# hucsmn/suffix_array

Measured on AMD Instinct MI355X. Metric: input MB/s indexed (SA build), higher is better.
Workload: dtype u8; 1 GPU; c3_english_256m: 268435456 bytes per GPU, seed base + rank, one independent text per GPU; n_bytes=268435456, sigma=57, symbols_per_key=13, refinement_rounds=9, text_rounds=0, radix_passes=25, unresolved_after_initial_sort=199000237

## Files before the change

### include/suffix_array_amd.h

```cpp
#ifndef SUFFIX_ARRAY_AMD_H
#define SUFFIX_ARRAY_AMD_H

#include <stdint.h>

#ifdef __cplusplus
extern "C" {
#endif

#define SA_AMD_OK          0
#define SA_AMD_EINVAL     (-1)
#define SA_AMD_ENOMEM     (-2)
#define SA_AMD_EHIP       (-3)
#define SA_AMD_ENODEVICE  (-4)
#define SA_AMD_EINTERNAL  (-5)
#define SA_AMD_ERANGE     (-6)

#define SA_AMD_MAX_LENGTH 2147483647

int32_t sa_amd_max_length(void);

int32_t sa_amd_divsufsort(const uint8_t *T, int32_t *SA, int32_t n);

int32_t sa_amd_saca_u8(const uint8_t *T, uint32_t *SA, int32_t n);

int32_t sa_amd_saca_batch(const uint8_t *const *T, uint32_t *const *SA, const int32_t *n,
                          const int32_t *device, int32_t count, int32_t *status);


typedef struct sa_amd_stats {
    int32_t sigma;
    int32_t bits_per_symbol;
    int32_t symbols_per_key;
    int32_t rounds;
    int32_t sort_passes;
    int32_t sparse_mode;
    int64_t sorted_elements;
    int64_t unresolved_after_initial;
    int32_t text_rounds;
    int32_t top32_first;
    int64_t locally_sorted;
    int32_t readbacks;
    int32_t reserved;
} sa_amd_stats;

int64_t sa_amd_workspace_bytes(int32_t n);

int32_t sa_amd_saca_device(const uint8_t *dT, uint32_t *dSA, int32_t n, void *dWork,
                           int64_t work_bytes, void *stream, sa_amd_stats *stats);

void sa_amd_release_cache(void);

int32_t sa_amd_last_host_timing(double *ms, int32_t capacity);

void sa_amd_last_stats(sa_amd_stats *out);

int32_t sa_amd_device_count(void);
int32_t sa_amd_device_pci_bus_id(int32_t device, char *buf, int32_t capacity);

const char *sa_amd_strerror(int32_t code);
const char *sa_amd_version(void);

#define SA_AMD_BUCKET_TABLE_LEN 65793
int32_t sa_amd_bucket_table(const uint8_t *T, int32_t n, const uint32_t *SA, uint32_t *bkt);
int32_t sa_amd_saca_u8_buckets(const uint8_t *T, uint32_t *SA, int32_t n, uint32_t *bkt);
int32_t sa_amd_bucket_table_device(const uint8_t *dT, const uint32_t *dSA, int32_t n, uint32_t *dBkt, void *stream);

int64_t sa_amd_check_integrity_work_bytes(int32_t n);
int32_t sa_amd_check_integrity(const uint8_t *T, int32_t n, const uint32_t *SA, int64_t sa_len);
int32_t sa_amd_check_integrity_device(const uint8_t *dT, int32_t n, const uint32_t *dSA, void *dWork,
                                      int64_t work_bytes, void *stream);

typedef struct sa_amd_index sa_amd_index;
int32_t sa_amd_index_create(const uint8_t *T, int32_t n, const uint32_t *SA, sa_amd_index **out);
void sa_amd_index_destroy(sa_amd_index *ix);
int32_t sa_amd_index_sa(const sa_amd_index *ix, uint32_t *SA_out);
int32_t sa_amd_index_buckets(sa_amd_index *ix, uint32_t *bkt);
int32_t sa_amd_index_check_integrity(const sa_amd_index *ix);
int32_t sa_amd_index_search(const sa_amd_index *ix, const uint8_t *pat_data, const int64_t *pat_off, int32_t count,
                            uint8_t *contains, uint32_t *range_lo, uint32_t *range_hi, uint32_t *lcp_start,
                            uint32_t *lcp_len);

int64_t sa_amd_pack_bound(int64_t length);
int32_t sa_amd_pack(const uint32_t *SA, int64_t length, uint8_t *out, int64_t capacity, int64_t *out_len);
int32_t sa_amd_unpack(const uint8_t *bytes, int64_t nbytes, uint32_t *SA, int64_t capacity, int64_t *length);

int64_t sa_amd_lcp_work_bytes(int32_t n);
int32_t sa_amd_lcp_device(const uint8_t *dT, const uint32_t *dSA, int32_t n, uint32_t *dLCP,
                          void *dWork, int64_t work_bytes, void *stream);
int32_t sa_amd_lcp(const uint8_t *T, int32_t n, const uint32_t *SA, uint32_t *LCP);
int32_t sa_amd_saca_u8_lcp(const uint8_t *T, uint32_t *SA, int32_t n, uint32_t *LCP);
int32_t sa_amd_index_lcp(const sa_amd_index *ix, uint32_t *LCP);

int32_t sa_amd_index_enable_lcp(sa_amd_index *ix);

typedef struct sa_amd_search_stats {
    int64_t patterns;
    int64_t compared_bytes;
    int64_t steps;
    int64_t table_steps;
    int32_t route;
    int32_t reserved;
} sa_amd_search_stats;
void sa_amd_last_search_stats(sa_amd_search_stats *out);

typedef struct sa_amd_lcp_stats {
    int64_t irreducible;
    int64_t compared_bytes;
    int64_t long_pairs;
    int32_t readbacks, reserved;
} sa_amd_lcp_stats;
void sa_amd_last_lcp_stats(sa_amd_lcp_stats *out);
int32_t sa_amd_lcp_set_compare_cap(int32_t bytes);

int64_t sa_amd_bwt_work_bytes(int32_t n);
int32_t sa_amd_bwt_device(const uint8_t *dT, const uint32_t *dSA, int32_t n, uint8_t *dBWT, int32_t *primary_out,
                          void *dWork, int64_t work_bytes, void *stream);
int32_t sa_amd_bwt(const uint8_t *T, int32_t n, const uint32_t *SA, uint8_t *BWT, int32_t *primary_out);
int32_t sa_amd_index_bwt(const sa_amd_index *ix, uint8_t *BWT, int32_t *primary_out);

int64_t sa_amd_unbwt_work_bytes(int32_t n);
int32_t sa_amd_unbwt_device(const uint8_t *dBWT, int32_t n, int32_t primary, uint8_t *dT_out, void *dWork,
                            int64_t work_bytes, void *stream);
int32_t sa_amd_unbwt(const uint8_t *BWT, int32_t n, int32_t primary, uint8_t *T_out);

typedef struct sa_amd_unbwt_stats {
    int64_t walkers;
    int64_t steps;
    int64_t longest_walk;
    int32_t splitter_spacing;
    int32_t walk_launches;
    int32_t restarts;
    int32_t readbacks;
} sa_amd_unbwt_stats;
void sa_amd_last_unbwt_stats(sa_amd_unbwt_stats *out);
void sa_amd_unbwt_set_walk_limits(int32_t cap_steps, int32_t max_launches);
int32_t sa_amd_unbwt_set_splitter_spacing(int32_t spacing);

#define SA_AMD_REPEATS_ALL        0
#define SA_AMD_REPEATS_KEEP_FIRST 1
int64_t sa_amd_repeats_work_bytes(int32_t n);
int64_t sa_amd_repeat_spans_bound(int32_t n, int32_t min_len);
int32_t sa_amd_repeat_lengths_device(const uint8_t *dT, const uint32_t *dSA, int32_t n, uint32_t *dLR, void *dWork,
                                     int64_t work_bytes, void *stream);
int32_t sa_amd_repeat_spans_device(const uint8_t *dT, const uint32_t *dSA, int32_t n, int32_t min_len, int32_t mode,
                                   uint32_t *dSpans, int64_t capacity, int64_t *count_out, void *dWork, int64_t work_bytes,
                                   void *stream);
int32_t sa_amd_repeat_lengths(const uint8_t *T, int32_t n, const uint32_t *SA, uint32_t *LR);
int32_t sa_amd_repeat_spans(const uint8_t *T, int32_t n, const uint32_t *SA, int32_t min_len, int32_t mode, uint32_t *spans,
                            int64_t capacity, int64_t *count_out);
int32_t sa_amd_index_repeat_lengths(const sa_amd_index *ix, uint32_t *LR);
int32_t sa_amd_index_repeat_spans(const sa_amd_index *ix, int32_t min_len, int32_t mode, uint32_t *spans, int64_t capacity,
                                  int64_t *count_out);

typedef struct sa_amd_repeat_stats {
    int64_t longest;
    int64_t longest_pos;
    int64_t lcp_sum;
    int64_t distinct_substrings;
    int64_t spans;
    int64_t covered_bytes;
    int64_t flagged;
    int32_t readbacks, reserved;
} sa_amd_repeat_stats;
void sa_amd_last_repeat_stats(sa_amd_repeat_stats *out);

#define SA_AMD_LZ_LITERAL 0xffffffffu
int64_t sa_amd_lz_work_bytes(int32_t n);
int32_t sa_amd_lpf_device(const uint8_t *dT, const uint32_t *dSA, int32_t n, uint32_t *dLPF, uint32_t *dSRC, void *dWork,
                          int64_t work_bytes, void *stream);
int32_t sa_amd_lz77_device(const uint8_t *dT, const uint32_t *dSA, int32_t n, uint32_t *dPhrases, int64_t capacity,
                           int64_t *count_out, void *dWork, int64_t work_bytes, void *stream);
int32_t sa_amd_lpf(const uint8_t *T, int32_t n, const uint32_t *SA, uint32_t *LPF, uint32_t *SRC);
int32_t sa_amd_lz77(const uint8_t *T, int32_t n, const uint32_t *SA, uint32_t *phrases, int64_t capacity, int64_t *count_out);
int32_t sa_amd_index_lpf(const sa_amd_index *ix, uint32_t *LPF, uint32_t *SRC);
int32_t sa_amd_index_lz77(const sa_amd_index *ix, uint32_t *phrases, int64_t capacity, int64_t *count_out);

typedef struct sa_amd_lz_stats {
    int64_t phrases;
    int64_t literals;
    int64_t longest;
    int64_t longest_pos;
    int64_t unresolved;
    int64_t hierarchy_steps;
    int64_t hierarchy_max;
    int64_t walkers;
    int64_t walk_steps;
    int32_t walk_launches;
    int32_t restarts;
    int32_t splitter_spacing;
    int32_t readbacks;
} sa_amd_lz_stats;
void sa_amd_last_lz_stats(sa_amd_lz_stats *out);

#define SA_AMD_MATCH_NONE 0xffffffffu
int64_t sa_amd_match_work_bytes(int32_t m);
int32_t sa_amd_index_match_stats(const sa_amd_index *ix, const uint8_t *Q, int32_t m, int32_t max_len, uint32_t *ML, uint32_t *POS);
int32_t sa_amd_index_match_stats_device(const sa_amd_index *ix, const uint8_t *dQ, int32_t m, int32_t max_len, uint32_t *dML,
                                        uint32_t *dPOS, void *dWork, int64_t work_bytes, void *stream);
int32_t sa_amd_index_match_spans(const sa_amd_index *ix, const uint8_t *Q, int32_t m, int32_t min_len, uint32_t *spans,
                                 int64_t capacity, int64_t *count_out);
int32_t sa_amd_index_match_spans_device(const sa_amd_index *ix, const uint8_t *dQ, int32_t m, int32_t min_len, uint32_t *dSpans,
// ... 35 lines not shown
```

### suffix_array_amd/__init__.py

```python
from __future__ import annotations

import ctypes
import os
from typing import Optional

import numpy as np

__all__ = ["MAX_LENGTH", "saca", "SuffixArray", "SuffixArrayError", "lib", "diag_lib", "library_path", "Stats", "last_host_timing",
           "saca_batch", "workspace_bytes", "device_pci_bus_id", "saca_device_ptr", "bucket_table", "check_integrity", "last_stats", "DeviceIndex", "pack", "unpack",
           "lcp", "saca_lcp", "last_lcp_stats", "lcp_work_bytes", "lcp_device_ptr", "LcpStats",
           "lcp_set_compare_cap", "last_search_stats", "SearchStats",
           "bwt", "unbwt", "bwt_device_ptr", "unbwt_device_ptr", "bwt_work_bytes", "unbwt_work_bytes", "last_unbwt_stats",
           "unbwt_set_walk_limits", "unbwt_set_splitter_spacing", "UnbwtStats",
           "repeat_lengths", "repeat_spans", "last_repeat_stats", "repeats_work_bytes", "repeat_spans_bound",
           "repeat_lengths_device_ptr", "repeat_spans_device_ptr", "RepeatStats", "REPEATS_ALL", "REPEATS_KEEP_FIRST",
           "lpf", "lz77", "lz77_decode", "lz77_literals", "last_lz_stats", "lz_work_bytes", "lpf_device_ptr", "lz77_device_ptr", "LzStats", "LZ_LITERAL",
           "MatchStats", "last_match_stats", "match_work_bytes", "match_set_group_cap", "match_set_group_lanes", "match_stats_device_ptr", "match_spans_device_ptr",
           "MATCH_NONE", "MATCH_TILE"]

MAX_LENGTH = 2**31 - 1

_HERE = os.path.dirname(os.path.abspath(__file__))
_LIB_NAME = "libsuffix_array_amd.so"
_lib: Optional[ctypes.CDLL] = None


class SuffixArrayError(RuntimeError):

    def __init__(self, code: int, what: str):
        super().__init__(f"suffix_array_amd: {what} (status {code})")
        self.code = code


class Stats(ctypes.Structure):
    _fields_ = [("sigma", ctypes.c_int32), ("bits_per_symbol", ctypes.c_int32),
                ("symbols_per_key", ctypes.c_int32), ("rounds", ctypes.c_int32),
                ("sort_passes", ctypes.c_int32), ("sparse_mode", ctypes.c_int32),
                ("sorted_elements", ctypes.c_int64), ("unresolved_after_initial", ctypes.c_int64),
                ("text_rounds", ctypes.c_int32), ("top32_first", ctypes.c_int32), ("locally_sorted", ctypes.c_int64),
                ("readbacks", ctypes.c_int32), ("reserved", ctypes.c_int32)]

    def as_dict(self):
        return {k: getattr(self, k) for k, _ in self._fields_}


class LcpStats(ctypes.Structure):
    _fields_ = [("irreducible", ctypes.c_int64), ("compared_bytes", ctypes.c_int64), ("long_pairs", ctypes.c_int64),
                ("readbacks", ctypes.c_int32), ("reserved", ctypes.c_int32)]

    def as_dict(self):
        return {k: getattr(self, k) for k, _ in self._fields_ if k != "reserved"}


class SearchStats(ctypes.Structure):
    _fields_ = [("patterns", ctypes.c_int64), ("compared_bytes", ctypes.c_int64), ("steps", ctypes.c_int64),
                ("table_steps", ctypes.c_int64), ("route", ctypes.c_int32), ("reserved", ctypes.c_int32)]

    def as_dict(self):
        return {name: getattr(self, name) for name, _ in self._fields_ if name != "reserved"}


class UnbwtStats(ctypes.Structure):
    _fields_ = [("walkers", ctypes.c_int64), ("steps", ctypes.c_int64), ("longest_walk", ctypes.c_int64),
                ("splitter_spacing", ctypes.c_int32), ("walk_launches", ctypes.c_int32), ("restarts", ctypes.c_int32),
                ("readbacks", ctypes.c_int32)]

    def as_dict(self):
        return {name: getattr(self, name) for name, _ in self._fields_}


class RepeatStats(ctypes.Structure):
    _fields_ = [("longest", ctypes.c_int64), ("longest_pos", ctypes.c_int64), ("lcp_sum", ctypes.c_int64),
                ("distinct_substrings", ctypes.c_int64), ("spans", ctypes.c_int64), ("covered_bytes", ctypes.c_int64),
                ("flagged", ctypes.c_int64), ("readbacks", ctypes.c_int32), ("reserved", ctypes.c_int32)]

    def as_dict(self):
        return {name: getattr(self, name) for name, _ in self._fields_ if name != "reserved"}


class LzStats(ctypes.Structure):
    _fields_ = [("phrases", ctypes.c_int64), ("literals", ctypes.c_int64), ("longest", ctypes.c_int64), ("longest_pos", ctypes.c_int64),
                ("unresolved", ctypes.c_int64), ("hierarchy_steps", ctypes.c_int64), ("hierarchy_max", ctypes.c_int64),
                ("walkers", ctypes.c_int64), ("walk_steps", ctypes.c_int64), ("walk_launches", ctypes.c_int32),
                ("restarts", ctypes.c_int32), ("splitter_spacing", ctypes.c_int32), ("readbacks", ctypes.c_int32)]

    def as_dict(self):
        return {name: getattr(self, name) for name, _ in self._fields_}


class MatchStats(ctypes.Structure):
    _fields_ = [("positions", ctypes.c_int64), ("matched", ctypes.c_int64), ("longest", ctypes.c_int64), ("longest_pos", ctypes.c_int64),
                ("ml_sum", ctypes.c_int64), ("long_positions", ctypes.c_int64), ("compared_bytes", ctypes.c_int64), ("steps", ctypes.c_int64),
                ("spans", ctypes.c_int64), ("covered_bytes", ctypes.c_int64), ("flagged", ctypes.c_int64), ("route_long", ctypes.c_int32),
                ("readbacks", ctypes.c_int32), ("group_lanes", ctypes.c_int32), ("group_cap", ctypes.c_int32), ("tile", ctypes.c_int32),
                ("reserved", ctypes.c_int32)]

    def as_dict(self):
        return {name: getattr(self, name) for name, _ in self._fields_ if name != "reserved"}


MATCH_NONE = 0xFFFFFFFF
MATCH_TILE = 256

LZ_LITERAL = 0xFFFFFFFF

REPEATS_ALL = 0
REPEATS_KEEP_FIRST = 1


def library_path() -> str:
    return os.path.join(_HERE, _LIB_NAME)


def lib() -> ctypes.CDLL:
    global _lib
    if _lib is None:
        path = library_path()
        if not os.path.exists(path):
            raise ImportError(f"{path} not found: run `python -c 'import __graft_entry__ as g; g.build()'` "
                              "(there is no CPU fallback)")
        L = ctypes.CDLL(path)
        c_u8p, c_vp = ctypes.c_void_p, ctypes.c_void_p
        L.sa_amd_max_length.restype = ctypes.c_int32
        L.sa_amd_divsufsort.argtypes = [c_u8p, c_vp, ctypes.c_int32]
        L.sa_amd_divsufsort.restype = ctypes.c_int32
        L.sa_amd_saca_u8.argtypes = [c_u8p, c_vp, ctypes.c_int32]
        L.sa_amd_saca_u8.restype = ctypes.c_int32
        L.sa_amd_saca_batch.argtypes = [c_vp, c_vp, c_vp, c_vp, ctypes.c_int32, c_vp]
        L.sa_amd_saca_batch.restype = ctypes.c_int32
        L.sa_amd_workspace_bytes.argtypes = [ctypes.c_int32]
        L.sa_amd_workspace_bytes.restype = ctypes.c_int64
        L.sa_amd_saca_device.argtypes = [c_vp, c_vp, ctypes.c_int32, c_vp, ctypes.c_int64, c_vp, c_vp]
        L.sa_amd_saca_device.restype = ctypes.c_int32
        L.sa_amd_device_count.restype = ctypes.c_int32
        L.sa_amd_device_pci_bus_id.argtypes = [ctypes.c_int32, ctypes.c_char_p, ctypes.c_int32]
        L.sa_amd_device_pci_bus_id.restype = ctypes.c_int32
        L.sa_amd_bucket_table_device.argtypes = [c_vp, c_vp, ctypes.c_int32, c_vp, c_vp]
        L.sa_amd_bucket_table_device.restype = ctypes.c_int32
        L.sa_amd_last_stats.argtypes = [c_vp]
        L.sa_amd_index_create.argtypes = [c_vp, ctypes.c_int32, c_vp, ctypes.POINTER(ctypes.c_void_p)]
        L.sa_amd_index_create.restype = ctypes.c_int32
        L.sa_amd_index_destroy.argtypes = [c_vp]
        L.sa_amd_index_destroy.restype = None
        for fn in ("sa_amd_index_sa", "sa_amd_index_buckets"):
            getattr(L, fn).argtypes = [c_vp, c_vp]
            getattr(L, fn).restype = ctypes.c_int32
        L.sa_amd_index_check_integrity.argtypes = [c_vp]
        L.sa_amd_index_check_integrity.restype = ctypes.c_int32
        L.sa_amd_index_search.argtypes = [c_vp, c_vp, c_vp, ctypes.c_int32, c_vp, c_vp, c_vp, c_vp, c_vp]
        L.sa_amd_index_search.restype = ctypes.c_int32
        L.sa_amd_pack_bound.argtypes = [ctypes.c_int64]
        L.sa_amd_pack_bound.restype = ctypes.c_int64
        L.sa_amd_pack.argtypes = [c_vp, ctypes.c_int64, c_vp, ctypes.c_int64, c_vp]
        L.sa_amd_pack.restype = ctypes.c_int32
        L.sa_amd_unpack.argtypes = [c_vp, ctypes.c_int64, c_vp, ctypes.c_int64, c_vp]
        L.sa_amd_unpack.restype = ctypes.c_int32
        L.sa_amd_bucket_table.argtypes = [c_vp, ctypes.c_int32, c_vp, c_vp]
        L.sa_amd_bucket_table.restype = ctypes.c_int32
        L.sa_amd_saca_u8_buckets.argtypes = [c_vp, c_vp, ctypes.c_int32, c_vp]
        L.sa_amd_saca_u8_buckets.restype = ctypes.c_int32
        L.sa_amd_check_integrity.argtypes = [c_vp, ctypes.c_int32, c_vp, ctypes.c_int64]
        L.sa_amd_check_integrity.restype = ctypes.c_int32
        L.sa_amd_last_stats.restype = None
        L.sa_amd_strerror.argtypes = [ctypes.c_int32]
        L.sa_amd_strerror.restype = ctypes.c_char_p
        L.sa_amd_version.restype = ctypes.c_char_p
        L.sa_amd_profile_begin.restype = None
        L.sa_amd_profile_end.argtypes = [c_vp, c_vp, c_vp, ctypes.c_int32]
        L.sa_amd_profile_end.restype = ctypes.c_int32
        L.sa_amd_profile_kernel_name.argtypes = [ctypes.c_int32]
        L.sa_amd_profile_kernel_name.restype = ctypes.c_char_p
        L.sa_amd_last_host_timing.argtypes = [c_vp, ctypes.c_int32]
        L.sa_amd_last_host_timing.restype = ctypes.c_int32
        L.sa_amd_profile_begin_classes.argtypes = [ctypes.c_uint64]
        L.sa_amd_profile_begin_classes.restype = None
        L.sa_amd_check_integrity_device.argtypes = [c_vp, ctypes.c_int32, c_vp, c_vp, ctypes.c_int64, c_vp]
        L.sa_amd_check_integrity_device.restype = ctypes.c_int32
        L.sa_amd_check_integrity_work_bytes.argtypes = [ctypes.c_int32]
        L.sa_amd_check_integrity_work_bytes.restype = ctypes.c_int64
        L.sa_amd_lcp_work_bytes.argtypes = [ctypes.c_int32]
        L.sa_amd_lcp_work_bytes.restype = ctypes.c_int64
        L.sa_amd_lcp_device.argtypes = [c_vp, c_vp, ctypes.c_int32, c_vp, c_vp, ctypes.c_int64, c_vp]
        L.sa_amd_lcp_device.restype = ctypes.c_int32
        L.sa_amd_lcp.argtypes = [c_vp, ctypes.c_int32, c_vp, c_vp]
        L.sa_amd_lcp.restype = ctypes.c_int32
        L.sa_amd_saca_u8_lcp.argtypes = [c_vp, c_vp, ctypes.c_int32, c_vp]
        L.sa_amd_saca_u8_lcp.restype = ctypes.c_int32
        L.sa_amd_index_lcp.argtypes = [c_vp, c_vp]
        L.sa_amd_index_lcp.restype = ctypes.c_int32
        L.sa_amd_last_lcp_stats.argtypes = [c_vp]
        L.sa_amd_last_lcp_stats.restype = None
        L.sa_amd_lcp_set_compare_cap.argtypes = [ctypes.c_int32]
        L.sa_amd_lcp_set_compare_cap.restype = ctypes.c_int32
        L.sa_amd_index_enable_lcp.argtypes = [c_vp]
        L.sa_amd_index_enable_lcp.restype = ctypes.c_int32
        L.sa_amd_last_search_stats.argtypes = [c_vp]
        L.sa_amd_last_search_stats.restype = None
        L.sa_amd_bwt_work_bytes.argtypes = [ctypes.c_int32]
        L.sa_amd_bwt_work_bytes.restype = ctypes.c_int64
        L.sa_amd_bwt_device.argtypes = [c_vp, c_vp, ctypes.c_int32, c_vp, c_vp, c_vp, ctypes.c_int64, c_vp]
        L.sa_amd_bwt_device.restype = ctypes.c_int32
        L.sa_amd_bwt.argtypes = [c_vp, ctypes.c_int32, c_vp, c_vp, c_vp]
        L.sa_amd_bwt.restype = ctypes.c_int32
        L.sa_amd_index_bwt.argtypes = [c_vp, c_vp, c_vp]
        L.sa_amd_index_bwt.restype = ctypes.c_int32
        L.sa_amd_unbwt_work_bytes.argtypes = [ctypes.c_int32]
        L.sa_amd_unbwt_work_bytes.restype = ctypes.c_int64
        L.sa_amd_unbwt_device.argtypes = [c_vp, ctypes.c_int32, ctypes.c_int32, c_vp, c_vp, ctypes.c_int64, c_vp]
        L.sa_amd_unbwt_device.restype = ctypes.c_int32
        L.sa_amd_unbwt.argtypes = [c_vp, ctypes.c_int32, ctypes.c_int32, c_vp]
        L.sa_amd_unbwt.restype = ctypes.c_int32
        L.sa_amd_last_unbwt_stats.argtypes = [c_vp]
        L.sa_amd_last_unbwt_stats.restype = None
        L.sa_amd_unbwt_set_walk_limits.argtypes = [ctypes.c_int32, ctypes.c_int32]
        L.sa_amd_unbwt_set_walk_limits.restype = None
        L.sa_amd_unbwt_set_splitter_spacing.argtypes = [ctypes.c_int32]
        L.sa_amd_unbwt_set_splitter_spacing.restype = ctypes.c_int32
        L.sa_amd_repeats_work_bytes.argtypes = [ctypes.c_int32]
        L.sa_amd_repeats_work_bytes.restype = ctypes.c_int64
        L.sa_amd_repeat_spans_bound.argtypes = [ctypes.c_int32, ctypes.c_int32]
        L.sa_amd_repeat_spans_bound.restype = ctypes.c_int64
        L.sa_amd_repeat_lengths_device.argtypes = [c_vp, c_vp, ctypes.c_int32, c_vp, c_vp, ctypes.c_int64, c_vp]
        L.sa_amd_repeat_lengths_device.restype = ctypes.c_int32
        L.sa_amd_repeat_spans_device.argtypes = [c_vp, c_vp, ctypes.c_int32, ctypes.c_int32, ctypes.c_int32, c_vp, ctypes.c_int64,
                                                 c_vp, c_vp, ctypes.c_int64, c_vp]
        L.sa_amd_repeat_spans_device.restype = ctypes.c_int32
        L.sa_amd_repeat_lengths.argtypes = [c_vp, ctypes.c_int32, c_vp, c_vp]
        L.sa_amd_repeat_lengths.restype = ctypes.c_int32
        L.sa_amd_repeat_spans.argtypes = [c_vp, ctypes.c_int32, c_vp, ctypes.c_int32, ctypes.c_int32, c_vp, ctypes.c_int64, c_vp]
        L.sa_amd_repeat_spans.restype = ctypes.c_int32
        L.sa_amd_index_repeat_lengths.argtypes = [c_vp, c_vp]
        L.sa_amd_index_repeat_lengths.restype = ctypes.c_int32
        L.sa_amd_index_repeat_spans.argtypes = [c_vp, ctypes.c_int32, ctypes.c_int32, c_vp, ctypes.c_int64, c_vp]
        L.sa_amd_index_repeat_spans.restype = ctypes.c_int32
        L.sa_amd_last_repeat_stats.argtypes = [c_vp]
        L.sa_amd_last_repeat_stats.restype = None
        L.sa_amd_lz_work_bytes.argtypes = [ctypes.c_int32]
        L.sa_amd_lz_work_bytes.restype = ctypes.c_int64
        L.sa_amd_lpf_device.argtypes = [c_vp, c_vp, ctypes.c_int32, c_vp, c_vp, c_vp, ctypes.c_int64, c_vp]
        L.sa_amd_lpf_device.restype = ctypes.c_int32
        L.sa_amd_lz77_device.argtypes = [c_vp, c_vp, ctypes.c_int32, c_vp, ctypes.c_int64, c_vp, c_vp, ctypes.c_int64, c_vp]
        L.sa_amd_lz77_device.restype = ctypes.c_int32
        L.sa_amd_lpf.argtypes = [c_vp, ctypes.c_int32, c_vp, c_vp, c_vp]
        L.sa_amd_lpf.restype = ctypes.c_int32
        L.sa_amd_lz77.argtypes = [c_vp, ctypes.c_int32, c_vp, c_vp, ctypes.c_int64, c_vp]
        L.sa_amd_lz77.restype = ctypes.c_int32
        L.sa_amd_index_lpf.argtypes = [c_vp, c_vp, c_vp]
        L.sa_amd_index_lpf.restype = ctypes.c_int32
        L.sa_amd_index_lz77.argtypes = [c_vp, c_vp, ctypes.c_int64, c_vp]
        L.sa_amd_index_lz77.restype = ctypes.c_int32
        L.sa_amd_last_lz_stats.argtypes = [c_vp]
        L.sa_amd_last_lz_stats.restype = None
        L.sa_amd_match_work_bytes.argtypes = [ctypes.c_int32]
        L.sa_amd_match_work_bytes.restype = ctypes.c_int64
        L.sa_amd_index_match_stats.argtypes = [c_vp, c_vp, ctypes.c_int32, ctypes.c_int32, c_vp, c_vp]
        L.sa_amd_index_match_stats.restype = ctypes.c_int32
        L.sa_amd_index_match_stats_device.argtypes = [c_vp, c_vp, ctypes.c_int32, ctypes.c_int32, c_vp, c_vp, c_vp, ctypes.c_int64, c_vp]
        L.sa_amd_index_match_stats_device.restype = ctypes.c_int32
        L.sa_amd_index_match_spans.argtypes = [c_vp, c_vp, ctypes.c_int32, ctypes.c_int32, c_vp, ctypes.c_int64, c_vp]
        L.sa_amd_index_match_spans.restype = ctypes.c_int32
        L.sa_amd_index_match_spans_device.argtypes = [c_vp, c_vp, ctypes.c_int32, ctypes.c_int32, c_vp, ctypes.c_int64, c_vp, c_vp,
                                                      ctypes.c_int64, c_vp]
        L.sa_amd_index_match_spans_device.restype = ctypes.c_int32
        L.sa_amd_last_match_stats.argtypes = [c_vp]
        L.sa_amd_last_match_stats.restype = None
        L.sa_amd_match_set_group_cap.argtypes = [ctypes.c_int32]
        L.sa_amd_match_set_group_cap.restype = ctypes.c_int32
        L.sa_amd_match_set_group_lanes.argtypes = [ctypes.c_int32]
        L.sa_amd_match_set_group_lanes.restype = ctypes.c_int32
        _lib = L
    return _lib


_diag: Optional[ctypes.CDLL] = None


def diag_lib() -> ctypes.CDLL:
    global _diag
    if _diag is None:
        path = os.path.join(_HERE, "libsuffix_array_amd_diag.so")
        if not os.path.exists(path):
            raise ImportError(f"{path} not found: run __graft_entry__.build()")
        L = ctypes.CDLL(path)
        c_vp = ctypes.c_void_p
        L.sa_amd_test_sort_pairs.argtypes = [c_vp, c_vp, ctypes.c_int64, ctypes.c_int32, ctypes.c_int32]
        L.sa_amd_test_sort_pairs.restype = ctypes.c_int32
        L.sa_amd_test_sort_pairs32.argtypes = [c_vp, c_vp, ctypes.c_int64, ctypes.c_int32, ctypes.c_int32]
        L.sa_amd_test_sort_pairs32.restype = ctypes.c_int32
        L.sa_amd_test_sample_sort64.argtypes = [c_vp, c_vp, ctypes.c_int64, ctypes.c_int32, c_vp]
        L.sa_amd_test_sample_sort64.restype = ctypes.c_int32
        L.sa_amd_test_bucket_sort32.argtypes = [c_vp, c_vp, ctypes.c_int64, ctypes.c_int32, c_vp]
        L.sa_amd_test_bucket_sort32.restype = ctypes.c_int32
        L.sa_amd_test_lz_nsv.argtypes = [c_vp, ctypes.c_int64, c_vp, c_vp, c_vp]
        L.sa_amd_test_lz_nsv.restype = ctypes.c_int32
        L.sa_amd_test_build_keys.argtypes = [c_vp, ctypes.c_int32, c_vp, c_vp, c_vp]
        L.sa_amd_test_build_keys.restype = ctypes.c_int32
        L.sa_amd_debug_phase_cycles.argtypes = [c_vp, ctypes.c_int32]
        L.sa_amd_debug_phase_cycles.restype = ctypes.c_int32
        L.sa_amd_debug_group_sort_stamps.argtypes = [ctypes.c_int32]
        L.sa_amd_debug_group_sort_stamps.restype = ctypes.c_int32
        L.sa_amd_debug_sort_variant_count.restype = ctypes.c_int32
        L.sa_amd_debug_sort_variant_name.argtypes = [ctypes.c_int32]
        L.sa_amd_debug_sort_variant_name.restype = ctypes.c_char_p
        L.sa_amd_saca_u8.argtypes = [c_vp, c_vp, ctypes.c_int32]
        L.sa_amd_saca_u8.restype = ctypes.c_int32
        L.sa_amd_saca_device.argtypes = [c_vp, c_vp, ctypes.c_int32, c_vp, ctypes.c_int64, c_vp, c_vp]
        L.sa_amd_saca_device.restype = ctypes.c_int32
        L.sa_amd_workspace_bytes.argtypes = [ctypes.c_int32]
        L.sa_amd_workspace_bytes.restype = ctypes.c_int64
        L.sa_amd_version.restype = ctypes.c_char_p
        _diag = L
    return _diag


def device_pci_bus_id(device: int = 0) -> str:
    buf = ctypes.create_string_buffer(64)
    _check(lib().sa_amd_device_pci_bus_id(int(device), buf, 64))
    return buf.value.decode()


def _check(code: int) -> None:
    if code != 0:
        raise SuffixArrayError(code, lib().sa_amd_strerror(code).decode())


def _as_u8(s) -> np.ndarray:
    if isinstance(s, np.ndarray):
        if s.dtype != np.uint8 or not s.flags.c_contiguous:
            raise TypeError("text must be a contiguous uint8 array")
        return s
    return np.frombuffer(bytes(s), dtype=np.uint8) if len(s) else np.zeros(0, dtype=np.uint8)


def saca(s, sa: np.ndarray) -> None:
    t = _as_u8(s)
    assert t.size <= MAX_LENGTH
    assert t.size + 1 == sa.size
    if sa.dtype != np.uint32 or not sa.flags.c_contiguous or not sa.flags.writeable:
        raise TypeError("sa must be a writable contiguous uint32 array")
    _check(lib().sa_amd_saca_u8(t.ctypes.data, sa.ctypes.data, t.size))


def divsufsort(s, sa: np.ndarray) -> None:
    t = _as_u8(s)
    assert t.size == sa.size and sa.dtype == np.int32
    _check(lib().sa_amd_divsufsort(t.ctypes.data, sa.ctypes.data, t.size))


def saca_batch(texts, devices=None):
    ts = [_as_u8(t) for t in texts]
    cnt = len(ts)
    if cnt >= 64:
        sizes = np.fromiter((t.size for t in ts), dtype=np.int64, count=cnt)
        offs = np.zeros(cnt + 1, dtype=np.int64)
        np.cumsum(sizes + 1, out=offs[1:])
        buf = np.empty(int(offs[-1]), dtype=np.uint32)
        outs = [buf[a:b] for a, b in zip(offs[:-1].tolist(), offs[1:].tolist())]
        tp = np.fromiter((t.__array_interface__["data"][0] for t in ts), dtype=np.uint64, count=cnt)
        sp = (np.uint64(buf.ctypes.data) + (offs[:-1] * 4).astype(np.uint64)).astype(np.uint64)
        nn = sizes.astype(np.int32)
        dd = np.asarray(devices, dtype=np.int32) if devices is not None else None
        st = np.zeros(cnt, dtype=np.int32)
        rc = lib().sa_amd_saca_batch(tp.ctypes.data, sp.ctypes.data, nn.ctypes.data, dd.ctypes.data if dd is not None else None, cnt,
                                     st.ctypes.data)
        _check(rc)
        return outs
    outs = [np.empty(t.size + 1, dtype=np.uint32) for t in ts]
    T = (ctypes.c_void_p * cnt)(*[t.ctypes.data for t in ts])
    S = (ctypes.c_void_p * cnt)(*[o.ctypes.data for o in outs])
    N = (ctypes.c_int32 * cnt)(*[t.size for t in ts])
    D = (ctypes.c_int32 * cnt)(*devices) if devices is not None else None
    st = (ctypes.c_int32 * cnt)()
    rc = lib().sa_amd_saca_batch(T, S, N, D, cnt, st)
    _check(rc)
    return outs


def last_host_timing() -> dict:
    v = (ctypes.c_double * 9)()
    lib().sa_amd_last_host_timing(v, 9)
    return {"acquire": v[0], "h2d": v[1], "build": v[2], "d2h": v[3], "release": v[4], "total": v[5], "staged_threads": int(v[6]),
            "early_fraction": v[7], "workspace_bytes_in_host_memory": int(v[8])}


def last_stats() -> dict:
    st = Stats()
    lib().sa_amd_last_stats(ctypes.byref(st))
    return st.as_dict()


BUCKET_TABLE_LEN = 256 * 257 + 1


def bucket_table(s, sa: np.ndarray | None = None) -> np.ndarray:
    t = _as_u8(s)
    if sa is not None:
        assert np.asarray(sa).size == t.size + 1
    bkt = np.empty(BUCKET_TABLE_LEN, dtype=np.uint32)
    _check(lib().sa_amd_bucket_table(t.ctypes.data, t.size, None, bkt.ctypes.data))
    return bkt


def check_integrity(s, sa: np.ndarray) -> bool:
    t = _as_u8(s)
    a = np.ascontiguousarray(sa, dtype=np.uint32)
    rc = lib().sa_amd_check_integrity(t.ctypes.data, t.size, a.ctypes.data, a.size)
    if rc == -6:
        raise IndexError("suffix offset out of range (the reference panics here, src/sa.rs:77-78)")
    if rc < 0:
        _check(rc)
    return rc == 1


def pack(sa: np.ndarray) -> bytes:
    a = np.ascontiguousarray(sa, dtype=np.uint32)
    cap = int(lib().sa_amd_pack_bound(a.size))
    out = np.empty(cap, dtype=np.uint8)
    n_out = ctypes.c_int64()
    _check(lib().sa_amd_pack(a.ctypes.data, a.size, out.ctypes.data, cap, ctypes.byref(n_out)))
    return out[:n_out.value].tobytes()


def unpack(blob: bytes) -> np.ndarray:
    b = np.frombuffer(blob, dtype=np.uint8)
    if b.size < 16:
        raise ValueError("packed suffix array: truncated header")
    length = int(np.frombuffer(blob[4:8], dtype="<u4")[0])
    out = np.empty(max(length, 1), dtype=np.uint32)
    got = ctypes.c_int64()
    rc = lib().sa_amd_unpack(b.ctypes.data, b.size, out.ctypes.data, out.size, ctypes.byref(got))
    if rc == -1:
        raise ValueError("packed suffix array: invalid data")
    _check(rc)
    return out[:got.value]


def _lcp_rc(rc: int) -> None:
    if rc == -6:
        raise IndexError("suffix offset out of range")
    _check(rc)


def lcp(s, sa: np.ndarray) -> np.ndarray:
    t = _as_u8(s)
    a = np.ascontiguousarray(sa, dtype=np.uint32)
    assert a.size == t.size + 1
    out = np.empty(t.size + 1, dtype=np.uint32)
    _lcp_rc(lib().sa_amd_lcp(t.ctypes.data, t.size, a.ctypes.data, out.ctypes.data))
    return out


def saca_lcp(s):
    t = _as_u8(s)
    assert t.size <= MAX_LENGTH
    a = np.empty(t.size + 1, dtype=np.uint32)
    out = np.empty(t.size + 1, dtype=np.uint32)
    _check(lib().sa_amd_saca_u8_lcp(t.ctypes.data, a.ctypes.data, t.size, out.ctypes.data))
    return a, out


def last_lcp_stats() -> dict:
    st = LcpStats()
    lib().sa_amd_last_lcp_stats(ctypes.byref(st))
# ... 211 lines not shown
def lz77_device_ptr(text_ptr: int, sa_ptr: int, n: int, phrases_ptr: int, capacity: int, work_ptr: int, work_bytes: int,
                    stream: int = 0) -> int:
    count = ctypes.c_int64(0)
    _bwt_rc(lib().sa_amd_lz77_device(text_ptr, sa_ptr, n, phrases_ptr or None, int(capacity), ctypes.byref(count), work_ptr, work_bytes,
                                     stream))
    return int(count.value)


def last_match_stats() -> dict:
    st = MatchStats()
    lib().sa_amd_last_match_stats(ctypes.byref(st))
    return st.as_dict()


def match_work_bytes(m: int) -> int:
    return int(lib().sa_amd_match_work_bytes(m))


def match_set_group_cap(nbytes: int) -> int:
    return int(lib().sa_amd_match_set_group_cap(int(nbytes)))


def match_set_group_lanes(lanes: int) -> int:
    return int(lib().sa_amd_match_set_group_lanes(int(lanes)))


def _index_handle(index):
    return index._h if isinstance(index, DeviceIndex) else index


def match_stats_device_ptr(index, query_ptr: int, m: int, max_len: int, ml_ptr: int, pos_ptr: int, work_ptr: int, work_bytes: int,
                           stream: int = 0) -> None:
    _check(lib().sa_amd_index_match_stats_device(_index_handle(index), query_ptr or None, int(m), int(max_len), ml_ptr or None,
                                                 pos_ptr or None, work_ptr, work_bytes, stream))


def match_spans_device_ptr(index, query_ptr: int, m: int, min_len: int, spans_ptr: int, capacity: int, work_ptr: int, work_bytes: int,
                           stream: int = 0) -> int:
    count = ctypes.c_int64(0)
    _check(lib().sa_amd_index_match_spans_device(_index_handle(index), query_ptr or None, int(m), int(min_len), spans_ptr or None,
                                                 int(capacity), ctypes.byref(count), work_ptr, work_bytes, stream))
    return int(count.value)


class DeviceIndex:

    def __init__(self, s, sa: Optional[np.ndarray] = None):
        self._s = _as_u8(s)
        h = ctypes.c_void_p()
        a = None if sa is None else np.ascontiguousarray(sa, dtype=np.uint32)
        if a is not None:
            assert a.size == self._s.size + 1
        _check(lib().sa_amd_index_create(self._s.ctypes.data, self._s.size, None if a is None else a.ctypes.data,
                                         ctypes.byref(h)))
        self._h = h

    def close(self):
        if getattr(self, "_h", None):
            lib().sa_amd_index_destroy(self._h)
            self._h = None

    __del__ = close

    def suffix_array(self) -> np.ndarray:
        out = np.empty(self._s.size + 1, dtype=np.uint32)
        _check(lib().sa_amd_index_sa(self._h, out.ctypes.data))
        return out

    def buckets(self) -> np.ndarray:
        bkt = np.empty(BUCKET_TABLE_LEN, dtype=np.uint32)
        _check(lib().sa_amd_index_buckets(self._h, bkt.ctypes.data))
        return bkt

    def check_integrity(self) -> bool:
        rc = lib().sa_amd_index_check_integrity(self._h)
        if rc < 0 and rc != -6:
            _check(rc)
        return rc == 1

    def lcp(self) -> np.ndarray:
        out = np.empty(self._s.size + 1, dtype=np.uint32)
        _lcp_rc(lib().sa_amd_index_lcp(self._h, out.ctypes.data))
        return out

    def bwt(self):
        out = np.empty(self._s.size, dtype=np.uint8)
        primary = ctypes.c_int32(0)
        _bwt_rc(lib().sa_amd_index_bwt(self._h, out.ctypes.data, ctypes.byref(primary)))
        return out, int(primary.value)

    def repeat_lengths(self) -> np.ndarray:
        out = np.empty(self._s.size, dtype=np.uint32)
        _bwt_rc(lib().sa_amd_index_repeat_lengths(self._h, out.ctypes.data))
        return out

    def repeat_spans(self, min_len: int, keep_first: bool = False) -> np.ndarray:
        k = _repeat_min_len(min_len)
        cap = (self._s.size + 1) // (k + 1)
        out = np.empty((cap, 2), dtype=np.uint32)
        count = ctypes.c_int64(0)
        _bwt_rc(lib().sa_amd_index_repeat_spans(self._h, k, REPEATS_KEEP_FIRST if keep_first else REPEATS_ALL, out.ctypes.data, cap,
                                                ctypes.byref(count)))
        return out[:min(int(count.value), cap)].copy()

    def lpf(self):
        out = np.empty((2, self._s.size), dtype=np.uint32)
        _bwt_rc(lib().sa_amd_index_lpf(self._h, out[0].ctypes.data, out[1].ctypes.data))
        return out[0], out[1]

    def lz77(self) -> np.ndarray:
        cap = min(self._s.size, max(1 << 16, self._s.size // 8))
        while True:
            out = np.empty((cap, 2), dtype=np.uint32)
            count = ctypes.c_int64(0)
            _bwt_rc(lib().sa_amd_index_lz77(self._h, out.ctypes.data, cap, ctypes.byref(count)))
            if count.value <= cap:
                return out[:int(count.value)].copy()
            cap = int(count.value)

    def match_stats(self, query, max_len: int):
        q = _as_u8(query)
        assert q.size <= MAX_LENGTH
        cap = min(_repeat_min_len(max_len), 2**31 - 1)
        out = np.empty((2, q.size), dtype=np.uint32)
        _check(lib().sa_amd_index_match_stats(self._h, q.ctypes.data, q.size, cap, out[0].ctypes.data, out[1].ctypes.data))
        return out[0], out[1]

    def match_spans(self, query, min_len: int) -> np.ndarray:
        q = _as_u8(query)
        assert q.size <= MAX_LENGTH
        k = _repeat_min_len(min_len)
        cap = (q.size + 1) // (k + 1)
        out = np.empty((cap, 2), dtype=np.uint32)
        count = ctypes.c_int64(0)
        _check(lib().sa_amd_index_match_spans(self._h, q.ctypes.data, q.size, k, out.ctypes.data, cap, ctypes.byref(count)))
        return out[:min(int(count.value), cap)].copy()

    def enable_lcp(self) -> None:
        _lcp_rc(lib().sa_amd_index_enable_lcp(self._h))

    def search(self, patterns):
        pats = [bytes(p) for p in patterns]
        cnt = len(pats)
        off = np.zeros(cnt + 1, dtype=np.int64)
        off[1:] = np.cumsum([len(p) for p in pats])
        data = np.frombuffer(b"".join(pats), dtype=np.uint8) if off[-1] else np.zeros(1, dtype=np.uint8)
        c = np.zeros(cnt, dtype=np.uint8)
        lo, hi, ls, ll = (np.zeros(cnt, dtype=np.uint32) for _ in range(4))
        _check(lib().sa_amd_index_search(self._h, data.ctypes.data, off.ctypes.data, cnt, c.ctypes.data, lo.ctypes.data,
                                         hi.ctypes.data, ls.ctypes.data, ll.ctypes.data))
        return {"contains": c.astype(bool), "lo": lo, "hi": hi, "lcp_start": ls, "lcp_len": ll}


def workspace_bytes(n: int) -> int:
    return int(lib().sa_amd_workspace_bytes(n))


def saca_device_ptr(text_ptr: int, sa_ptr: int, n: int, work_ptr: int, work_bytes: int, stream: int = 0,
                    stats: Optional[Stats] = None) -> None:
    _check(lib().sa_amd_saca_device(text_ptr, sa_ptr, n, work_ptr, work_bytes, stream,
                                    ctypes.byref(stats) if stats is not None else None))


def _check_integrity(s: np.ndarray, sa: np.ndarray) -> bool:
    n = s.size
    if n + 1 != sa.size:
        return False
    if sa.max() > n:
        raise IndexError("suffix offset out of range (the reference panics here, src/sa.rs:77-78)")
    if n <= 64:
        return _check_integrity_literal(s, sa)
    return _check_integrity_linear(s, sa)


def _check_integrity_literal(s: np.ndarray, sa: np.ndarray) -> bool:
    b = s.tobytes()
    return all(b[int(sa[i - 1]):] < b[int(sa[i]):] for i in range(1, s.size + 1))


def _check_integrity_linear(s: np.ndarray, sa: np.ndarray) -> bool:
    n = s.size
    if int(sa[0]) != n:
        return False
    rank = np.full(n + 1, -1, dtype=np.int64)
    rank[sa] = np.arange(n + 1)
    if (rank < 0).any():
        return False
    a, b = sa[1:-1].astype(np.int64), sa[2:].astype(np.int64)
    ca, cb = s[a], s[b]
    ok = (ca < cb) | ((ca == cb) & (rank[a + 1] < rank[b + 1]))
    return bool(ok.all())


class SuffixArray:

    def __init__(self, s):
        self._s = _as_u8(s)
        self._sa = np.zeros(self._s.size + 1, dtype=np.uint32)
        saca(self._s, self._sa)
        self._bkt = None
        self._esa = False
        self._ix = None

    @classmethod
    def new(cls, s) -> "SuffixArray":
        return cls(s)

    def set(self, s) -> None:
        t = _as_u8(s)
        self._sa = np.resize(self._sa, t.size + 1)
        saca(t, self._sa)
        self._ix = None

    def fit(self) -> None:
        self._sa = np.ascontiguousarray(self._sa)

    def as_ref(self) -> np.ndarray:
        return self._s

    def len(self) -> int:
        return int(self._s.size)

    def is_empty(self) -> bool:
        return self.len() == 0

    def into_parts(self):
        return self._s, self._sa

    @classmethod
    def from_parts(cls, s, sa) -> Optional["SuffixArray"]:
        obj = cls.unchecked_from_parts(s, sa)
        if lib().sa_amd_device_count() > 0:
            ok = check_integrity(obj._s, obj._sa)
        else:
            ok = _check_integrity(obj._s, obj._sa)
        return obj if ok else None

    @classmethod
    def unchecked_from_parts(cls, s, sa) -> "SuffixArray":
        obj = cls.__new__(cls)
        obj._s = _as_u8(s)
        obj._sa = np.ascontiguousarray(sa, dtype=np.uint32)
        obj._bkt = None
        obj._esa = False
        obj._ix = None
        return obj

    def dump_bytes(self) -> bytes:
        return pack(self._sa)

    def dump(self, file) -> None:
        file.write(self.dump_bytes())

    @classmethod
    def load_bytes(cls, s, blob: bytes) -> "SuffixArray":
        obj = cls.from_parts(s, unpack(blob))
        if obj is None:
            raise ValueError("inconsistent suffix array")
        return obj

    @classmethod
    def load(cls, s, file) -> "SuffixArray":
        return cls.load_bytes(s, file.read())

    def enable_buckets(self) -> None:
        if self._bkt is None:
            self._bkt = bucket_table(self._s, self._sa)
            if getattr(self, "_ix", None) is not None:
                self._ix.buckets()

    def buckets(self) -> Optional[np.ndarray]:
        return self._bkt

    def _index(self) -> "DeviceIndex":
        if getattr(self, "_ix", None) is None:
            self._ix = DeviceIndex(self._s, self._sa)
            if self._bkt is not None:
                self._ix.buckets()
            if getattr(self, "_esa", False):
                self._ix.enable_lcp()
        return self._ix

    def contains(self, pat) -> bool:
        return bool(self._index().search([pat])["contains"][0])

    def search_all(self, pat) -> np.ndarray:
        r = self._index().search([pat])
        return self._sa[int(r["lo"][0]):int(r["hi"][0])]

    def search_lcp(self, pat) -> range:
        r = self._index().search([pat])
        return range(int(r["lcp_start"][0]), int(r["lcp_start"][0]) + int(r["lcp_len"][0]))

    def lcp_array(self) -> np.ndarray:
        return lcp(self._s, self._sa)

    def bwt(self):
        return bwt(self._s, self._sa)

    def repeat_lengths(self) -> np.ndarray:
        return repeat_lengths(self._s, self._sa)

    def repeat_spans(self, min_len: int, keep_first: bool = False) -> np.ndarray:
        return repeat_spans(self._s, min_len, keep_first, self._sa)

    def lpf(self):
# ... 18 lines not shown
```

### suffix_array_amd/csrc/host/pipeline.hpp

```cpp
#pragma once
#include "support.hpp"
#include "tuning.hpp"
#include "pool.hpp"

#include <functional>

namespace sa {

constexpr int SORT_MAX_WG = 1024;
constexpr int BK_TOP_BITS_MAX = 18;
constexpr uint32_t BK_BUCKETS_MAX = 1u << BK_TOP_BITS_MAX;
static_assert(32 - 16 <= BK_MAX_LBITS, "two 8-bit passes inside a bucket");
constexpr size_t GRAM_MAX_ENTRIES = (size_t)1 << 24;
static_assert(GROUP_CAP_MAX == GS_CAP, "Tuning clamps SA_AMD_GROUP_CAP to the kernel's cap");

#ifdef SA_AMD_DIAG
typedef void (*DownsweepFn)(const uint64_t *, const uint32_t *, uint64_t *, uint32_t *, uint32_t *,
                            const uint32_t *, int64_t, int, uint32_t, int64_t, int);
struct SortVariant { int threads, items, wg_per_cu; DownsweepFn fn; const char *name; };
static const SortVariant sort_variants[] = {
    { 1024, 8, 2, k_radix_downsweep_wcl<1024, 8, 16, 1, false, uint64_t, 4>, "carry-completed lines 1024x8 + LDS prefetch of half of the next tile's keys (default)" },
    { 1024, 8, 2, k_radix_downsweep_wcl<1024, 8>, "carry-completed lines 1024x8" },
    { 512, 16, 1, k_radix_downsweep_wcl<512, 16>, "carry-completed lines 512x16" },
    { 1024, 8, 2, k_radix_downsweep_wcl<1024, 8, 8>, "carry 1024x8, granule 8" },
#ifdef SA_AMD_DIAG
    { 1024, 8, 2, k_radix_downsweep<1024, 8, 4>, "plain tile scatter 1024x8 (first generation)" },
    { 1024, 8, 2, k_radix_downsweep<1024, 8, 4, 1>, "plain 1024x8 ABLATION sequential stores (wrong results)" },
    { 1024, 8, 2, k_radix_downsweep<1024, 8, 4, 33>, "plain 1024x8 ABLATION no ranking + sequential stores (wrong results)" },
    { 1024, 8, 2, k_radix_downsweep<1024, 8, 4, 16>, "plain 1024x8 ABLATION no stores (wrong results)" },
    { 1024, 8, 2, k_radix_downsweep<1024, 8, 4, 49>, "plain 1024x8 ABLATION no ranking, no stores (wrong results)" },
    { 1024, 8, 2, k_radix_downsweep_wcl<1024, 8, 16, 1, true>, "carry 1024x8 DIAGNOSTIC phase stamps (tools/phase_stamps.py)" },
#endif
};
constexpr int N_SORT_VARIANTS = (int)(sizeof(sort_variants) / sizeof(sort_variants[0]));

struct SortGrid { int G; int64_t tiles_per_wg; int tile; };
static SortGrid sort_grid(int64_t count, const SortVariant &sv)
{
    SortGrid g;
    g.tile = sv.threads * sv.items;
    const int64_t tiles = ceil_div(count, g.tile);
    int max_wg = 256 * sv.wg_per_cu;
    if (max_wg > SORT_MAX_WG) max_wg = SORT_MAX_WG;
    g.tiles_per_wg = ceil_div(tiles, max_wg);
    if (g.tiles_per_wg < 1) g.tiles_per_wg = 1;
    g.G = (int)ceil_div(tiles, g.tiles_per_wg);
    if (g.G < 1) g.G = 1;
    return g;
}

#else
constexpr int N_SORT_VARIANTS = 1;
#endif

struct SortScratch {
    uint32_t *spine;
    uint32_t *digit_tot;
    unsigned long long *status;
    uint32_t *err;
};

struct Workspace {
    uint64_t *keysA, *keysB, *keysC;
    uint32_t *valsA, *valsB, *isa, *U0, *U1, *G0, *G1;
    uint32_t *spine, *digit_tot, *tcnt, *thead, *tnext, *hist, *total, *chg, *has_isa;
    uint8_t *packed;
    uint8_t *gram_flags;
    uint4 *gram_table;
    uint32_t *surv_bits, *surv_cnt, *todo_bits, *ft_cnt, *ft_head;
    unsigned long long *os_status;
    uint32_t *os_err;
    uint32_t *bk_start;
    uint32_t *early_bits, *early_cnt;
    SortScratch ss;
    size_t bytes, bytes2;
};

static Workspace carve(void *base, int64_t n, size_t cap = ~(size_t)0, void *base2 = nullptr)
{
    Workspace w;
    const size_t N = (size_t)(n > 0 ? n : 1);
    size_t off = 0, off2 = 0;
    auto take = [&](size_t b) {
        if (off + b <= cap) { size_t o = off; off = align_up(off + b, 256); return (char *)base + o; }
        size_t o = off2; off2 = align_up(off2 + b, 256); return (char *)base2 + o;
    };
    const size_t rr_tiles = (size_t)ceil_div((int64_t)N, RR_TILE);
    const size_t ft_tiles = (size_t)ceil_div((int64_t)N, FT_TILE) + 1;
    const size_t gram_entries = N < GRAM_MAX_ENTRIES ? N : GRAM_MAX_ENTRIES;
    w.spine = (uint32_t *)take((size_t)RADIX * SORT_MAX_WG * 4);
    w.digit_tot = (uint32_t *)take(RADIX * 4);
    w.os_status = (unsigned long long *)take(((size_t)ceil_div((int64_t)N, OS_MIN_TILE) + 1) * RADIX * 8);
    w.os_err = (uint32_t *)take(256);
    w.hist = (uint32_t *)take(256 * 4);
    w.total = (uint32_t *)take(256);
    w.chg = (uint32_t *)take((size_t)RR_CHG_COUNTERS * 32 * 4);
    w.tcnt = (uint32_t *)take(rr_tiles * 4);
    w.thead = (uint32_t *)take(rr_tiles * 4);
    w.tnext = (uint32_t *)take(rr_tiles * 4);
    w.surv_cnt = (uint32_t *)take(rr_tiles * 4);
    w.ft_cnt = (uint32_t *)take(ft_tiles * 4);
    w.ft_head = (uint32_t *)take(ft_tiles * 4);
    w.bk_start = (uint32_t *)take(((size_t)BK_BUCKETS_MAX + 1) * 4);
    w.early_cnt = (uint32_t *)take(((N + 1 + EARLY_TILE - 1) / EARLY_TILE + 8) * 4);
    w.gram_table = (uint4 *)take((gram_entries / 64 + 1) * 16);
    w.has_isa = (uint32_t *)take((N + 31) / 32 * 4);
    w.surv_bits = (uint32_t *)take((N + 31) / 32 * 4);
    w.todo_bits = (uint32_t *)take((N + 31) / 32 * 4);
    w.early_bits = (uint32_t *)take(((N + 1 + 31) / 32 + EARLY_THREADS) * 4);
    w.gram_flags = (uint8_t *)take(gram_entries + 64);
    w.packed = (uint8_t *)take(N / 2 + 64);
    w.keysA = (uint64_t *)take((N + 64) * 8);
    w.keysB = (uint64_t *)take((N + 64) * 8);
    w.valsA = (uint32_t *)take(N * 4);
    w.valsB = (uint32_t *)take(N * 4);
    w.isa = (uint32_t *)take(N * 4);
    w.U0 = (uint32_t *)take(N * 4);
    w.G0 = (uint32_t *)take(N * 4);
    w.U1 = (uint32_t *)take(N * 4);
    w.G1 = (uint32_t *)take(N * 4);
    w.keysC = (uint64_t *)take((N + 64) * 8);
    w.ss.spine = w.spine; w.ss.digit_tot = w.digit_tot; w.ss.status = w.os_status; w.ss.err = w.os_err;
    w.bytes = off;
    w.bytes2 = off2;
    return w;
}


struct OsShape { int threads, items; bool seq; int wg_per_cu; };
static const OsShape os_shapes64[] = { { 1024, 8, false, 1 }, { 512, 16, true, 2 }, { 512, 8, false, 2 } };
static const OsShape os_shapes32[] = { { 1024, 12, false, 1 }, { 512, 16, true, 2 }, { 512, 12, false, 2 }, { 1024, 8, false, 1 } };
constexpr int N_OS_SHAPES64 = (int)(sizeof(os_shapes64) / sizeof(os_shapes64[0]));
constexpr int N_OS_SHAPES32 = (int)(sizeof(os_shapes32) / sizeof(os_shapes32[0]));
constexpr int OS_TICKETS = 64;
constexpr int OS_MAX_RADIX = 512;
constexpr int OS_ZONE = OS_TICKETS + OS_MAX_RADIX * OS_NSEG;
static_assert(OS_NSEG <= OS_TICKETS, "one ticket word per segment");
constexpr int OS_MAX_ZONES = 2 * 8 + 2;
static_assert(OS_MAX_ZONES * OS_ZONE <= RADIX * SORT_MAX_WG, "the zones live in the spine slab");

#ifdef SA_AMD_DIAG
static bool onesweep_on(const SortScratch &ss, const Tuning &tn) { return ss.status != nullptr && !tn.no_onesweep; }
#else
static bool onesweep_on(const SortScratch &ss, const Tuning &) { return ss.status != nullptr; }
#endif

struct OnesweepGeom { int tiles, nseg, tiles_per_seg; int64_t seg_elems; };
static OnesweepGeom onesweep_geom(int64_t count, int tile)
{
    OnesweepGeom g;
    g.tiles = (int)ceil_div(count, tile);
    if (g.tiles < 1) g.tiles = 1;
    int nseg = g.tiles < OS_NSEG ? g.tiles : OS_NSEG;
    g.tiles_per_seg = (int)ceil_div(g.tiles, nseg);
    g.nseg = (int)ceil_div(g.tiles, g.tiles_per_seg);
    g.seg_elems = (int64_t)g.tiles_per_seg * tile;
    return g;
}

struct FirstCounts { uint32_t *counts; int64_t chunk_elems; int G; void *zero_ptr; size_t zero_bytes; };
static FirstCounts sort_first_counts(const SortScratch &ss, const Tuning &tn, int64_t count, bool keys32);

static int cu_count()
{
    static int cus = 0;
    if (cus > 0) return cus;
    int dev = 0;
    hipDeviceProp_t prop;
    if (hipGetDevice(&dev) == hipSuccess && hipGetDeviceProperties(&prop, dev) == hipSuccess && prop.multiProcessorCount > 0) cus = prop.multiProcessorCount;
    else { (void)hipGetLastError(); cus = 256; }
    return cus;
}

static int read_words(void *dst, const void *dsrc, size_t bytes, hipStream_t st);

__global__ __launch_bounds__(RADIX) void k_os_digit_totals(const uint32_t *__restrict__ hist, int nseg, uint32_t *__restrict__ digit_tot)
{
    uint32_t s = 0;
    for (int q = 0; q < nseg; ++q) s += hist[threadIdx.x * nseg + q];
    digit_tot[threadIdx.x] = s;
}

constexpr int HA_THREADS = 256;
template <typename KeyT>
__global__ __launch_bounds__(HA_THREADS) void k_radix_hist_all(const KeyT *__restrict__ keys, int64_t count, int begin_bit, int end_bit,
                                                               uint32_t *__restrict__ zone0, int zone_words, int ticket_words)
{
    __shared__ uint32_t h[8][RADIX];
    for (int i = threadIdx.x; i < 8 * RADIX; i += HA_THREADS) (&h[0][0])[i] = 0;
    __syncthreads();
    const int np = (end_bit - begin_bit + RADIX_BITS - 1) / RADIX_BITS;
    for (int64_t i = (int64_t)blockIdx.x * HA_THREADS + threadIdx.x; i < count; i += (int64_t)gridDim.x * HA_THREADS) {
        const uint64_t k = (uint64_t)keys[i];
        for (int p = 0; p < np; ++p) {
            const int sh = begin_bit + p * RADIX_BITS, nb = end_bit - sh < RADIX_BITS ? end_bit - sh : RADIX_BITS;
            atomicAdd(&h[p][(k >> sh) & ((1u << nb) - 1u)], 1u);
        }
    }
    __syncthreads();
    for (int i = threadIdx.x; i < np * RADIX; i += HA_THREADS) {
        const uint32_t c = (&h[0][0])[i];
        if (c) atomicAdd(&zone0[(size_t)(i / RADIX) * zone_words + ticket_words + (i % RADIX)], c);
    }
}

template <typename KeyT, int THREADS, int ITEMS, bool SEQ, int RBITS = RADIX_BITS>
static int sort_pairs_onesweep(KeyT *keys_in, uint32_t *vals_in, KeyT *keys_alt, uint32_t *vals_alt, int64_t count, int begin_bit, int end_bit,
                               const SortScratch &ss, uint32_t *final_vals, hipStream_t st, KeyT **keys_res, uint32_t **vals_res, int *passes,
                               int *skipped, const Tuning &tn, bool iota, bool may_skip, bool first_counted,
                               const uint8_t *text = nullptr, int64_t text_n = 0,
                               int text_bits = 8,
                               int val_extra = 0,
                               KeyT *keys_out2 = nullptr)
{
    constexpr int TILE = THREADS * ITEMS;
    constexpr int R = 1 << RBITS;
    static_assert(R <= OS_MAX_RADIX && (RBITS == RADIX_BITS || TILE >= 2 * OS_MIN_TILE), "zones and granule slab are sized for 8-bit digits of 4 Ki-element tiles");
    static_assert(TILE >= OS_MIN_TILE, "the granule slab is sized for tiles of at least OS_MIN_TILE elements");
    constexpr bool K64 = sizeof(KeyT) == 8;
    OnesweepGeom g = onesweep_geom(count, TILE);
    auto zone = [&](int i) { return ss.spine + (size_t)i * OS_ZONE; };
    int z = 0;
    bool have_counts = first_counted;
    const int npass = (int)ceil_div(end_bit - begin_bit, RBITS);
    const bool upfront = RBITS == RADIX_BITS && !tn.no_upfront_counts && count < tn.count_next_min_n && !may_skip && !text && npass <= 8 && npass >= 2;
    if (upfront) { g.nseg = 1; g.tiles_per_seg = g.tiles; g.seg_elems = (int64_t)g.tiles * TILE; }
    HIP_TRY(hipMemsetAsync(ss.status, 0, (size_t)g.tiles * R * 8, st));
    {
        int zones = (may_skip ? 2 * npass : npass) + 1;
        if (zones > OS_MAX_ZONES) return SA_AMD_EINTERNAL;
        const int z0 = (first_counted && !upfront) ? 1 : 0;
        HIP_TRY(hipMemsetAsync(zone(z0), 0, (size_t)(zones - z0) * OS_ZONE * 4, st));
    }
    if (upfront) {
        int blocks = (int)ceil_div(count, (int64_t)HA_THREADS * 16);
        if (blocks > 512) blocks = 512;
        if (blocks < 1) blocks = 1;
        PROF(K64 ? KC_UPSWEEP : KC_UPSWEEP32, count, st, hipLaunchKernelGGL((k_radix_hist_all<KeyT>), dim3((unsigned)blocks), dim3(HA_THREADS), 0, st, (const KeyT *)keys_in, count,
                                                                        begin_bit, end_bit, zone(0), (int)OS_ZONE, (int)OS_TICKETS));
        have_counts = true;
    }
    KeyT *kin = keys_in, *kout = keys_alt;
    uint32_t *vin = vals_in, *vout = vals_alt;
    constexpr int WG_PER_CU = THREADS <= 512 ? 2 : 1;
    int grid = cu_count() * WG_PER_CU;
    if (grid > g.tiles) grid = g.tiles;
    uint32_t epoch = 0;
    for (int shift = begin_bit; shift < end_bit; shift += RBITS) {
        const int nb = (end_bit - shift) < RBITS ? (end_bit - shift) : RBITS;
        const uint32_t dmask = (1u << nb) - 1u;
        const bool last = shift + RBITS >= end_bit;
        uint32_t *vdst = (last && final_vals) ? final_vals : vout;
        if (!have_counts) {
            if (RBITS != RADIX_BITS) return SA_AMD_EINTERNAL;
            int split = 2048 / g.nseg;
            while (split > 1 && g.seg_elems / split < 8192) split /= 2;
            const int64_t sub = K64 ? ((ceil_div(g.seg_elems, split) + 1) & ~(int64_t)1) : ((ceil_div(g.seg_elems, split) + 3) & ~(int64_t)3);
            if (K64)
// ... 239 lines not shown
        f.counts = ss.spine + OS_TICKETS; f.chunk_elems = g.seg_elems; f.G = g.nseg;
        f.zero_ptr = ss.spine; f.zero_bytes = (size_t)OS_ZONE * 4;
        return f;
    }
#ifdef SA_AMD_DIAG
    f.counts = ss.spine; f.zero_ptr = ss.spine;
    if (keys32) {
        const SortGrid32 g32 = sort_grid32(count, sort32_variants[tn.sort32_variant]);
        f.chunk_elems = g32.tiles_per_wg * g32.tile; f.G = g32.G;
    } else {
        const SortGrid g64 = sort_grid(count, sort_variants[tn.sort_variant]);
        f.chunk_elems = g64.tiles_per_wg * g64.tile; f.G = g64.G;
    }
    f.zero_bytes = (size_t)RADIX * f.G * 4;
    return f;
#else
    f.counts = ss.spine; f.zero_ptr = ss.spine; f.chunk_elems = count; f.G = 1; f.zero_bytes = (size_t)RADIX * 4;
    return f;
#endif
}

struct BkShape { int threads, items, minw; };
static const BkShape bk_shapes[] = { { 256, 10, 6 }, { 512, 10, 8 }, { 1024, 10, 8 }, { 1024, 20, 1 }, { 256, 20, 1 } };
constexpr int N_BK_SHAPES = (int)(sizeof(bk_shapes) / sizeof(bk_shapes[0]));
constexpr int N_BK_DEFAULT = 4;
static int64_t bucket_cap(int shape) { return (int64_t)bk_shapes[shape].threads * bk_shapes[shape].items; }
static int64_t bucket_cap_max() { return bucket_cap(N_BK_DEFAULT - 1); }

static int bucket_sort32(const uint32_t *keys_in, const uint32_t *vals_in, uint32_t *keys_out, uint32_t *vals_out, int64_t count, int top_bits,
                         uint32_t *start, uint32_t *words, hipStream_t st, const Tuning &tn, bool *done, uint32_t *largest,
                         const BucketFinish *fin = nullptr, const KeyParams *P = nullptr, const KeySrc *K = nullptr, bool *fused = nullptr,
                         int val_extra = 0)
{
    *done = false; *largest = 0;
    if (fused) *fused = false;
    if (top_bits < 32 - BK_MAX_LBITS || top_bits > BK_TOP_BITS_MAX) return SA_AMD_EINTERNAL;
    const int lbits = 32 - top_bits;
    if (val_extra < 0 || lbits + val_extra > BK_MAX_LBITS) return SA_AMD_EINTERNAL;
    const uint32_t nb = 1u << top_bits;
    HIP_TRY(hipMemsetAsync(words, 0, 8, st));
    PROF(KC_MISC, nb, st, hipLaunchKernelGGL((k_bucket_starts), dim3((unsigned)ceil_div((int64_t)nb + 1, BK_STARTS_THREADS)), dim3(BK_STARTS_THREADS),
                                              0, st, keys_in, count, lbits, nb, start));
    PROF(KC_MISC, nb, st, hipLaunchKernelGGL((k_bucket_max), dim3((unsigned)ceil_div((int64_t)nb, BK_STARTS_THREADS)), dim3(BK_STARTS_THREADS), 0, st,
                                              (const uint32_t *)start, nb, words));
    uint32_t maxb = 0;
    { const int rcw = read_words(&maxb, words, 4, st); if (rcw) return rcw; }
    *largest = maxb;
    int shape = -1;
    if (tn.bucket_shape >= 0 && tn.bucket_shape < N_BK_SHAPES && bucket_cap(tn.bucket_shape) >= (int64_t)maxb) shape = tn.bucket_shape;
    for (int c = 0; shape < 0 && c < N_BK_DEFAULT; ++c)
        if (bucket_cap(c) >= (int64_t)maxb) shape = c;
    if (shape < 0) return SA_AMD_OK;
    const bool fuse = fin != nullptr && (bk_shapes[shape].items <= 10 || tn.bucket_finish_always);
    const BucketFinish F0 = BucketFinish();
    const KeyParams P0 = KeyParams();
    const KeySrc K0 = KeySrc();
#define BK_LAUNCH(T, I, W)                                                                                                               \
    do {                                                                                                                                 \
        if (fuse) PROF(KC_BUCKET, count, st, hipLaunchKernelGGL((k_bucket_sort<T, I, W, true>), dim3(nb), dim3(T), 0, st, keys_in, vals_in,         \
                                                                (const uint32_t *)start, lbits, keys_out, vals_out, words + 1, *fin, *P, *K, val_extra)); \
        else PROF(KC_BUCKET, count, st, hipLaunchKernelGGL((k_bucket_sort<T, I, W, false>), dim3(nb), dim3(T), 0, st, keys_in, vals_in,             \
                                                            (const uint32_t *)start, lbits, keys_out, vals_out, words + 1, F0, P0, K0, val_extra)); \
    } while (0)
    switch (shape) {
    case 0: BK_LAUNCH(256, 10, 6); break;
    case 1: BK_LAUNCH(512, 10, 8); break;
    case 2: BK_LAUNCH(1024, 10, 8); break;
    case 3: BK_LAUNCH(1024, 20, 1); break;
    default: BK_LAUNCH(256, 20, 1); break;
    }
#undef BK_LAUNCH
    *done = true;
    if (fused) *fused = fuse;
    return SA_AMD_OK;
}

#ifdef SA_AMD_DIAG
static int64_t sample_count(int64_t n, const Tuning &tn)
{
    int lg = tn.sample_log ? tn.sample_log : (n >= ((int64_t)1 << 28) ? 22 : (n >= ((int64_t)1 << 27) ? 21 : 20));
    while (lg > 16 && ((int64_t)1 << lg) * 4 > n) --lg;
    return (int64_t)1 << lg;
}

static int sample_sort64(uint64_t *keys_a, uint64_t *keys_b, uint64_t *keys_c, uint32_t *vals_a, uint32_t *vals_b, uint32_t *u0, uint32_t *u1,
                         uint32_t *big, uint32_t *small, uint32_t *words, uint32_t *final_vals, int64_t n, int key_bits, const SortScratch &ss,
                         hipStream_t st, sa_amd_stats *local, const Tuning &tn, bool *done, bool trace)
{
    *done = false;
    const int64_t S = sample_count(n, tn);
    if (S < 65536 || n < 4 * S || n >= ((int64_t)1 << 32)) return SA_AMD_OK;
    uint64_t *samp = keys_c, *samp_alt = keys_c + S;
    PROF(KC_MISC, S, st, hipLaunchKernelGGL((k_ss_sample), dim3((unsigned)ceil_div(S, 256)), dim3(256), 0, st, (const uint64_t *)keys_a, n, S, samp));
    SortResult sr;
    int rc = sort_pairs(samp, u0, samp_alt, u1, S, 0, key_bits, ss, nullptr, st, &sr, tn, true);
    if (rc) return rc;
    local->sort_passes += sr.passes; local->sorted_elements += (int64_t)sr.passes * S;
    const uint64_t *sample = sr.keys;
    const int64_t tiles1 = ceil_div(n, SS_TILE), max_tiles2 = tiles1 + SS_WAYS;
    const int64_t per = ceil_div(tiles1, SS_CHUNKS);
    const int chunks = (int)ceil_div(tiles1, per);
    uint32_t *counts = big;
    uint32_t *tot1 = small, *base1 = tot1 + SS_CHUNKS * SS_WAYS, *seg_start = base1 + SS_CHUNKS * SS_WAYS, *seg_first = seg_start + 320;
    uint32_t *tot2 = seg_first + 320, *bstart = tot2 + SS_WAYS * SS_IDS2;
    uint32_t *tile_seg = bstart + SS_BUCKETS + 64, *tile_base = tile_seg + ((max_tiles2 + 63) & ~(int64_t)63);
    PROF(KC_SS_COUNT, n, st, hipLaunchKernelGGL((k_ss_count<1>), dim3((unsigned)tiles1), dim3(SS_THREADS), 0, st, (const uint64_t *)keys_a, n, sample, S,
                                                (const uint32_t *)nullptr, (const uint32_t *)nullptr, (const uint32_t *)nullptr, counts));
    PROF(KC_RR_SCAN, tiles1, st, hipLaunchKernelGGL((k_ss_scan_tiles<SS_WAYS>), dim3((unsigned)chunks), dim3(SS_WAYS), 0, st, counts, tiles1, per,
                                                    (const uint32_t *)nullptr, tot1));
    PROF(KC_RR_SCAN, chunks, st, hipLaunchKernelGGL((k_ss_bases1), dim3(1), dim3(SS_WAYS), 0, st, (const uint32_t *)tot1, chunks, base1, seg_start, seg_first));
    PROF(KC_RR_SCAN, max_tiles2, st, hipLaunchKernelGGL((k_ss_tiles), dim3(SS_WAYS + 1), dim3(256), 0, st, (const uint32_t *)seg_start, (const uint32_t *)seg_first,
                                                        max_tiles2, tile_seg, tile_base));
    PROF(KC_SS_SCATTER, n, st, hipLaunchKernelGGL((k_ss_scatter<1>), dim3((unsigned)tiles1), dim3(SS_THREADS), 0, st, (const uint64_t *)keys_a, (const uint32_t *)nullptr, n,
                                                  sample, S, (const uint32_t *)nullptr, (const uint32_t *)nullptr, (const uint32_t *)nullptr,
                                                  (const uint32_t *)counts, (const uint32_t *)base1, per, keys_b, vals_a));
    PROF(KC_SS_COUNT, n, st, hipLaunchKernelGGL((k_ss_count<2>), dim3((unsigned)max_tiles2), dim3(SS_THREADS), 0, st, (const uint64_t *)keys_b, n, sample, S,
                                                (const uint32_t *)tile_seg, (const uint32_t *)tile_base, (const uint32_t *)seg_start, counts));
    PROF(KC_RR_SCAN, max_tiles2, st, hipLaunchKernelGGL((k_ss_scan_tiles<SS_IDS2>), dim3(SS_WAYS), dim3(SS_IDS2), 0, st, counts, max_tiles2, (int64_t)0,
                                                        (const uint32_t *)seg_first, tot2));
    PROF(KC_RR_SCAN, SS_WAYS, st, hipLaunchKernelGGL((k_ss_bases2), dim3(SS_WAYS), dim3(SS_IDS2), 0, st, (const uint32_t *)tot2, (const uint32_t *)seg_start, bstart, (uint32_t)n));
    PROF(KC_SS_SCATTER, n, st, hipLaunchKernelGGL((k_ss_scatter<2>), dim3((unsigned)max_tiles2), dim3(SS_THREADS), 0, st, (const uint64_t *)keys_b, (const uint32_t *)vals_a, n,
                                                  sample, S, (const uint32_t *)tile_seg, (const uint32_t *)tile_base, (const uint32_t *)seg_start,
                                                  (const uint32_t *)counts, (const uint32_t *)bstart, (int64_t)1, keys_a, vals_b));
    HIP_TRY(hipMemsetAsync(words, 0, 16, st));
    if (!tn.sample_merge)
    PROF(KC_SS_BUCKET, n, st, hipLaunchKernelGGL((k_ss_bucket_sort<SB_SMALL_THREADS, SB_SMALL_ITEMS, 9, 0, false>), dim3((unsigned)SS_BUCKETS), dim3(SB_SMALL_THREADS), 0, st,
                                                 (const uint64_t *)keys_a, (const uint32_t *)vals_b, (const uint32_t *)bstart, keys_b, final_vals, words, words + 4));
    else
    PROF(KC_SS_BUCKET, n, st, hipLaunchKernelGGL((k_ss_bucket_merge<SB_SMALL_THREADS, SB_SMALL_ITEMS>), dim3((unsigned)SS_BUCKETS), dim3(SB_SMALL_THREADS), 0, st,
                                                 (const uint64_t *)keys_a, (const uint32_t *)vals_b, (const uint32_t *)bstart, keys_b, final_vals, words));
    PROF(KC_SS_BUCKET, 0, st, hipLaunchKernelGGL((k_ss_bucket_sort<SB_THREADS, SB_ITEMS, 10, SB_SMALL_CAP, true>), dim3((unsigned)SS_BUCKETS), dim3(SB_THREADS), 0, st,
                                                 (const uint64_t *)keys_a, (const uint32_t *)vals_b, (const uint32_t *)bstart, keys_b, final_vals, words, words + 4));
    uint32_t res[2] = { 0, 0 };
    { const int rcw = read_words(res, words, 8, st); if (rcw) return rcw; }
    local->sort_passes += 3; local->sorted_elements += 3 * n;
    if (trace) fprintf(stderr, "suffix_array_amd: sample sort: %lld samples, largest bucket %u (a workgroup holds %d), %u oversize buckets that are no equality buckets\n",
                       (long long)S, res[1], SB_CAP, res[0]);
    *done = res[0] == 0;
    return SA_AMD_OK;
}

#endif

static int make_key_params(const uint32_t *hist, KeyParams *P, int *sigma_out, int kb_max = 64)
{
    int sigma = 0;
    for (int c = 0; c < 256; ++c) {
        if (hist[c]) P->code[c] = (uint8_t)sigma++;
        else P->code[c] = 0;
    }
    *sigma_out = sigma;
    P->packed = nullptr;
    P->gram = 0; P->gram_m = 0; P->gram_tail = 0; P->gram_top = 0; P->gram_D = 0; P->gram_table = nullptr;
    const uint64_t se = sigma > 2 ? (uint64_t)sigma : 2u;
    P->sigma = se;
    if ((se & (se - 1)) == 0) {
        const int bits = bit_length(se - 1);
        P->bits = bits;
        P->k = kb_max / bits;
        const int used = P->k * bits;
        P->mask = used >= 64 ? ~0ull : ((1ull << used) - 1ull);
        P->top = 0;
        return used;
    }
    unsigned __int128 pw = 1;
    int k = 0;
    while (pw * se <= ((unsigned __int128)1 << kb_max)) { pw *= se; ++k; }
    P->bits = 0;
    P->k = k;
    P->mask = ~0ull;
    uint64_t top = 1;
    for (int i = 0; i + 1 < k; ++i) top *= se;
    P->top = top;
    const unsigned __int128 maxkey = pw - 1;
    return bit_length((uint64_t)maxkey);
}

struct PinnedWords {
    PinBlock b;
    bool failed = false;
    ~PinnedWords() { if (b.p) pool().release_pinned(b); }
};
static thread_local PinnedWords g_pinned;
static thread_local int g_readbacks = 0;
static thread_local bool g_posted_off = false;
static std::atomic<uint32_t> g_post_seq{0};

constexpr int POST_LINE = 16;
__global__ __launch_bounds__(256) void k_post_words(const uint32_t *__restrict__ src, uint32_t *__restrict__ dst, int words, uint32_t seq)
{
    const int lines = (words + POST_LINE - 2) / (POST_LINE - 1);
    for (int i = threadIdx.x; i < lines * POST_LINE; i += 256) {
        const int q = i / POST_LINE, j = i % POST_LINE;
        if (j) { const int k = q * (POST_LINE - 1) + j - 1; dst[i] = k < words ? src[k] : 0u; }
    }
    __threadfence_system();
    __syncthreads();
    for (int q = threadIdx.x; q < lines; q += 256) __hip_atomic_store(dst + q * POST_LINE, seq, __ATOMIC_RELEASE, __HIP_MEMORY_SCOPE_SYSTEM);
}

static int read_words(void *dst, const void *dsrc, size_t bytes, hipStream_t st)
{
    ++g_readbacks;
    if (!g_pinned.b.p && !g_pinned.failed) {
        if (pool().pinned(8192, -1, -1, &g_pinned.b) == SA_AMD_OK) memset(g_pinned.b.p, 0, 8192);
        else g_pinned.failed = true;
    }
    if (!g_pinned.b.p) {
        HIP_TRY(hipMemcpyAsync(dst, dsrc, bytes, hipMemcpyDeviceToHost, st));
        HIP_TRY(hipStreamSynchronize(st));
        return SA_AMD_OK;
    }
    const int words = (int)(bytes / 4);
    const int lines = (words + POST_LINE - 2) / (POST_LINE - 1);
    if (!g_posted_off && (bytes & 3) == 0 && words > 0 && (size_t)lines * POST_LINE * 4 <= 4096) {
        uint32_t *host = (uint32_t *)g_pinned.b.p;
        uint32_t seq = g_post_seq.fetch_add(1, std::memory_order_relaxed) + 1;
        if (seq == 0) seq = g_post_seq.fetch_add(1, std::memory_order_relaxed) + 1;
        hipLaunchKernelGGL(k_post_words, dim3(1), dim3(256), 0, st, (const uint32_t *)dsrc, host, words, seq);
        if (hipGetLastError() == hipSuccess) {
            const auto t0 = std::chrono::steady_clock::now();
            bool done = false, finished = false;
            for (unsigned spin = 0; !done; ++spin) {
                done = true;
                for (int q = lines - 1; q >= 0 && done; --q)
                    done = __atomic_load_n((volatile uint32_t *)(host + q * POST_LINE), __ATOMIC_ACQUIRE) == seq;
                if (done) break;
                if ((spin & 1023u) == 1023u) {
                    const double us = std::chrono::duration<double, std::micro>(std::chrono::steady_clock::now() - t0).count();
                    if (us > 200.0) {
                        if (finished) break;
                        const hipError_t q = hipStreamQuery(st);
                        if (q == hipSuccess) finished = true;
                        else if (q != hipErrorNotReady) { (void)hipGetLastError(); break; }
                    }
                }
            }
            if (done) {
                uint32_t *out = (uint32_t *)dst;
                for (int k = 0; k < words; ++k) out[k] = host[(k / (POST_LINE - 1)) * POST_LINE + 1 + k % (POST_LINE - 1)];
                return SA_AMD_OK;
            }
        }
    }
    char *copy = (char *)g_pinned.b.p + 4096;
    HIP_TRY(hipMemcpyAsync(copy, dsrc, bytes, hipMemcpyDeviceToHost, st));
    HIP_TRY(hipStreamSynchronize(st));
    memcpy(dst, copy, bytes);
    return SA_AMD_OK;
}

static bool binned(int64_t n, int64_t count, const Tuning &tn)
{
    if (tn.no_binned_isa) return false;
    if (tn.binned_isa_always) return count > 0;
    return n >= ((int64_t)1 << 25) && (count >= n || count >= tn.binned_min);
}

static int scatter_binned(uint32_t *pk, uint32_t *pv, uint32_t *altk, uint32_t *altv, int64_t count, int64_t n,
                          const Workspace &w, hipStream_t st, sa_amd_stats *local, const Tuning &tn, bool iota = false,
                          uint32_t *altk2 = nullptr, uint32_t *altv2 = nullptr)
{
    const int nb = bit_length((uint64_t)(n > 1 ? n : 1));
    int wlog = nb - 16;
    if (wlog < 10) wlog = 10;
    if (wlog > 15) wlog = 15;
    const bool two = nb > wlog && (tn.scatter_levels == 2 || (tn.scatter_levels == 0 && count >= ((int64_t)1 << 25)));
    SortResult32 pr;
    if (two) {
        int rc;
        if (iota) {
            const int mid = wlog + RADIX_BITS < nb ? wlog + RADIX_BITS : nb;
            rc = sort_pairs32(pk, nullptr, altk, altv, count, wlog, mid, w.ss, nullptr, st, &pr, tn, true);
            if (rc) return rc;
            if (pr.passes != 1) return SA_AMD_EINTERNAL;
            local->sort_passes += 1; local->sorted_elements += count;
            if (mid < nb) {
                rc = sort_pairs32(altk, altv, altk2, altv2, count, mid, nb, w.ss, nullptr, st, &pr, tn);
                if (rc) return rc;
                local->sort_passes += pr.passes; local->sorted_elements += (int64_t)pr.passes * count;
            }
        } else {
            rc = sort_pairs32(pk, pv, altk, altv, count, wlog, nb, w.ss, nullptr, st, &pr, tn, false, false, RADIX_BITS, nullptr, 0, 8, 0, altk2);
            if (rc) return rc;
            local->sort_passes += pr.passes; local->sorted_elements += (int64_t)pr.passes * count;
        }
        const unsigned grid = (unsigned)ceil_div(count, SW_CHUNK);
        if (wlog <= 13)
            PROF(KC_SCATTER, count, st, hipLaunchKernelGGL((k_scatter_windows<13>), dim3(grid), dim3(SW_THREADS), 0, st, (const uint32_t *)pr.keys,
                                                           (const uint32_t *)pr.vals, w.isa, count, (uint32_t)n, wlog));
        else
            PROF(KC_SCATTER, count, st, hipLaunchKernelGGL((k_scatter_windows<15>), dim3(grid), dim3(SW_THREADS), 0, st, (const uint32_t *)pr.keys,
                                                           (const uint32_t *)pr.vals, w.isa, count, (uint32_t)n, wlog));
        return SA_AMD_OK;
    }
    const int shift = nb > RADIX_BITS ? nb - RADIX_BITS : 0;
    int rc = sort_pairs32(pk, pv, altk, altv, count, shift, shift + RADIX_BITS, w.ss, nullptr, st, &pr, tn, iota);
    if (rc) return rc;
    local->sort_passes += pr.passes; local->sorted_elements += (int64_t)pr.passes * count;
    PROF(KC_SCATTER, count, st, hipLaunchKernelGGL((k_scatter_pairs<uint32_t>), dim3((unsigned)ceil_div(count, 1024)), dim3(256), 0, st,
                                                   (const uint32_t *)pr.keys, (const uint32_t *)pr.vals, w.isa, count, (uint32_t)n));
    return SA_AMD_OK;
}

struct Refined { const uint64_t *keys; const uint32_t *vals; uint32_t *vnext; int64_t m_global; };

// ... 78 lines not shown
    const int64_t tiles = ceil_div(m, RR_TILE);
    const int kb = K.kb;
    SortResult sr;
    int rc;
    bool counted = false;
    uint32_t groups = 0;
    if (!*local_ok && retry_local && !tn.no_local_sort && m < tn.dense_rekey_min) *local_ok = true;
    if (!*local_ok && retry_local && !tn.no_local_sort && m >= tn.dense_rekey_min) {
        PROF(KC_RR_COUNT, m, st, hipLaunchKernelGGL((k_flag_count), dim3((unsigned)tiles), dim3(RR_THREADS), 0, st,
                                                    (const uint8_t *)nullptr, Ucur, Gcur, m, w.tcnt, w.ft_cnt));
        PROF(KC_RR_SCAN, tiles, st, hipLaunchKernelGGL((k_rr_scan), dim3(1), dim3(SPINE_THREADS), 0, st, w.ft_cnt, w.thead, tiles, w.total + 8));
        { const int rcw = read_words(&groups, w.total + 8, 4, st); if (rcw) return rcw; }
        counted = true;
        if ((int64_t)groups * 2 * tn.group_cap >= m) *local_ok = true;
    }
    const bool had_local_pass = *local_ok;
    if (*local_ok) {
        uint8_t *flags = (uint8_t *)scratchG;
        const unsigned gs_blocks = (unsigned)ceil_div(m, GS_TILE);
        const int cap = tn.group_cap;
        const bool big_local = !tn.no_big_group_sort && kb <= 32 && m > GS_CAP && !(ctl && ctl->skip_big);
        uint32_t *bheads = big_local ? scratchU : (uint32_t *)nullptr, *bcount = big_local ? w.total + RC_BIG_LISTED : (uint32_t *)nullptr;
        if (!resume) {
        if (!(ctl && ctl->counters_clear))
            HIP_TRY(hipMemsetAsync(w.total + RC_BIG_LISTED, 0, 8, st));
        if (K.mode == KS_TEXT)
            PROF(KC_LOCAL, m, st, hipLaunchKernelGGL((k_group_sort<KS_TEXT>), dim3(gs_blocks), dim3(GS_THREADS), 0, st, (const uint32_t *)Vcur,
                                                     Gcur, Ucur, dT, P, m, n, K, rkA, Vcur, flags, cap, bheads, bcount));
        else if (K.mode == KS_LOWKEY)
            PROF(KC_LOCAL, m, st, hipLaunchKernelGGL((k_group_sort<KS_LOWKEY>), dim3(gs_blocks), dim3(GS_THREADS), 0, st, (const uint32_t *)Vcur,
                                                     Gcur, Ucur, dT, P, m, n, K, rkA, Vcur, flags, cap, bheads, bcount));
        else if (K.mode == KS_RANK)
            PROF(KC_LOCAL, m, st, hipLaunchKernelGGL((k_group_sort<KS_RANK>), dim3(gs_blocks), dim3(GS_THREADS), 0, st, (const uint32_t *)Vcur,
                                                     Gcur, Ucur, dT, P, m, n, K, rkA, Vcur, flags, cap, bheads, bcount));
        else if (K.mode == KS_CHASE)
            PROF(KC_LOCAL, m, st, hipLaunchKernelGGL((k_group_sort<KS_CHASE>), dim3(gs_blocks), dim3(GS_THREADS), 0, st, (const uint32_t *)Vcur,
                                                     Gcur, Ucur, dT, P, m, n, K, rkA, Vcur, flags, cap, bheads, bcount));
        else {
            int64_t gblocks = ceil_div(m, GK_THREADS);
            if (gblocks > 8192) gblocks = 8192;
            PROF(KC_GATHER, m, st, hipLaunchKernelGGL((k_gather_textkey<KS_SPARSE>), dim3((unsigned)gblocks), dim3(GK_THREADS), 0, st,
                                                      (const uint32_t *)Vcur, Gcur, dT, P, m, n, K, rkA));
            PROF(KC_LOCAL, m, st, hipLaunchKernelGGL((k_group_sort<KS_PRE>), dim3(gs_blocks), dim3(GS_THREADS), 0, st, (const uint32_t *)Vcur,
                                                     Gcur, Ucur, dT, P, m, n, K, rkA, Vcur, flags, cap, bheads, bcount));
        }
        if (gs_blocks > 1)
            PROF(KC_LOCAL, 0, st, hipLaunchKernelGGL((k_group_sort_straddle), dim3(gs_blocks - 1), dim3(GX_THREADS), 0, st, rkA, Vcur, Gcur,
                                                     Ucur, m, flags, cap, K, n));
        if (big_local) {
            const int lo = cap > GS_CAP ? cap : GS_CAP;
            PROF(KC_LOCAL, 0, st, hipLaunchKernelGGL((k_group_sort_big<256>), dim3((unsigned)(8 * cu_count())), dim3(256), 0, st, rkA, Vcur, Gcur, m, kb, lo,
                                                     (const uint32_t *)bheads, (const uint32_t *)bcount, flags, w.total + 13));
            PROF(KC_LOCAL, 0, st, hipLaunchKernelGGL((k_group_sort_big<512>), dim3((unsigned)(4 * cu_count())), dim3(512), 0, st, rkA, Vcur, Gcur, m, kb,
                                                     lo > GB_CAP_SMALL ? lo : GB_CAP_SMALL, (const uint32_t *)bheads, (const uint32_t *)bcount, flags, w.total + 13));
        }
        PROF(KC_RR_COUNT, m, st, hipLaunchKernelGGL((k_flag_count), dim3((unsigned)tiles), dim3(RR_THREADS), 0, st,
                                                    (const uint8_t *)flags, Ucur, Gcur, m, w.tcnt, w.ft_cnt));
        PROF(KC_RR_SCAN, tiles, st, hipLaunchKernelGGL((k_rr_scan_pair), dim3(2), dim3(SPINE_THREADS), 0, st, w.tcnt, w.thead, w.total + RC_FLAGGED,
                                                       w.ft_cnt, (uint32_t *)nullptr, w.total + RC_GROUPS, tiles));
        }
        if (ctl && ctl->defer && !resume) {
            ctl->deferred = true;
            out->keys = rkA; out->vals = Vcur; out->vnext = Valt; out->m_global = 0;
            return SA_AMD_OK;
        }
        uint32_t tot9[RC_WORDS] = { 0 };
        if (resume) memcpy(tot9, ctl->resume_tot, sizeof(tot9));
        else {
            const int rcw = read_words(tot9, w.total, sizeof(tot9), st); if (rcw) return rcw;
            }
        const int64_t m_big = tot9[RC_FLAGGED], m_big_local = tot9[RC_BIG_ORDERED];
        if (ctl) { ctl->m_flagged = m_big; ctl->big_listed = big_local ? (int64_t)tot9[RC_BIG_LISTED] : -1; }
        const size_t half = ((size_t)n / 2) & ~(size_t)1;
        if ((size_t)m_big <= half && half + (size_t)m_big <= (size_t)n) {
            if (m_big > 0) {
                const int idx_bits = bit_length((uint64_t)(tot9[RC_GROUPS] > 0 ? tot9[RC_GROUPS] - 1 : 0));
                PROF(KC_RR_APPLY, m, st, hipLaunchKernelGGL((k_flag_gather), dim3((unsigned)tiles), dim3(RR_THREADS), 0, st,
                                                            (const uint8_t *)flags, (const uint64_t *)rkA, (const uint32_t *)Vcur, Ucur, Gcur, m,
                                                            (const uint32_t *)w.tcnt, (const uint32_t *)w.ft_cnt, kb, rkB, Valt, scratchU));
                rc = sort_pairs(rkB, Valt, rkB + half, Valt + half, m_big, 0, kb + idx_bits, w.ss, nullptr, st, &sr, tn, false, true);
                if (rc) return rc;
                local->sort_passes += sr.passes; local->sorted_elements += (int64_t)sr.passes * m_big;
                PROF(KC_SCATTER, m_big, st, hipLaunchKernelGGL((k_scatter_back), dim3((unsigned)ceil_div(m_big, 256)), dim3(256), 0, st,
                                                               (const uint64_t *)sr.keys, (const uint32_t *)sr.vals,
                                                               (const uint32_t *)scratchU, Gcur, kb, m_big, rkA, Vcur));
            }
            out->keys = rkA; out->vals = Vcur; out->vnext = Valt; out->m_global = m_big + m_big_local;
            local->locally_sorted += m - m_big;
            if (m_big * 2 > m) *local_ok = false;
            return SA_AMD_OK;
        }
        if (m_big * 10 >= m * 9) *local_ok = false;
    }
    int sort_bits = kb + g_bits;
    bool rekeyed = false;
    if (m >= tn.dense_rekey_min) {
        if (!counted || had_local_pass) {
            PROF(KC_RR_COUNT, m, st, hipLaunchKernelGGL((k_flag_count), dim3((unsigned)tiles), dim3(RR_THREADS), 0, st,
                                                        (const uint8_t *)nullptr, Ucur, Gcur, m, w.tcnt, w.ft_cnt));
            PROF(KC_RR_SCAN, tiles, st, hipLaunchKernelGGL((k_rr_scan), dim3(1), dim3(SPINE_THREADS), 0, st, w.ft_cnt, w.thead, tiles, w.total + 8));
            { const int rcw = read_words(&groups, w.total + 8, 4, st); if (rcw) return rcw; }
            }
        const int idx_bits = bit_length((uint64_t)(groups > 0 ? groups - 1 : 0));
        if (ceil_div(kb + idx_bits, RADIX_BITS) < ceil_div(kb + g_bits, RADIX_BITS)) {
            sort_bits = kb + idx_bits;
            rekeyed = true;
        }
    }
    const bool split_wanted = rekeyed && !tn.no_split && m >= tn.split_min && groups > 0 && (int64_t)groups * tn.split_group_min <= m &&
                              !(split_rest && *split_rest > 0);
    bool starts_ready = false;
    if (had_local_pass) {
        if (rekeyed)
            PROF(KC_RR_APPLY, m, st, hipLaunchKernelGGL((k_rekey_dense), dim3((unsigned)tiles), dim3(RR_THREADS), 0, st, rkA, Ucur, Gcur, m,
                                                        (const uint32_t *)w.ft_cnt, kb));
    } else if (K.mode == KS_SPARSE) {
        int64_t gblocks = ceil_div(m, GK_THREADS);
        if (gblocks > 8192) gblocks = 8192;
        PROF(KC_GATHER, m, st, hipLaunchKernelGGL((k_gather_textkey<KS_SPARSE>), dim3((unsigned)gblocks), dim3(GK_THREADS), 0, st,
                                                  (const uint32_t *)Vcur, Gcur, dT, P, m, n, K, rkA));
        if (rekeyed)
            PROF(KC_RR_APPLY, m, st, hipLaunchKernelGGL((k_rekey_dense), dim3((unsigned)tiles), dim3(RR_THREADS), 0, st, rkA, Ucur, Gcur, m,
                                                        (const uint32_t *)w.ft_cnt, kb));
    } else {
        const uint32_t *th = rekeyed ? (const uint32_t *)w.ft_cnt : (const uint32_t *)nullptr;
        uint32_t *gs = split_wanted ? scratchG : (uint32_t *)nullptr;
        starts_ready = gs != nullptr;
        if (K.mode == KS_TEXT)
            PROF(KC_GATHER, m, st, hipLaunchKernelGGL((k_gather_keyed<KS_TEXT>), dim3((unsigned)tiles), dim3(RR_THREADS), 0, st,
                                                      (const uint32_t *)Vcur, Ucur, Gcur, dT, P, m, n, K, th, rkA, gs, groups));
        else if (K.mode == KS_LOWKEY)
            PROF(KC_GATHER, m, st, hipLaunchKernelGGL((k_gather_keyed<KS_LOWKEY>), dim3((unsigned)tiles), dim3(RR_THREADS), 0, st,
                                                      (const uint32_t *)Vcur, Ucur, Gcur, dT, P, m, n, K, th, rkA, gs, groups));
        else
            PROF(KC_GATHER, m, st, hipLaunchKernelGGL((k_gather_keyed<KS_RANK>), dim3((unsigned)tiles), dim3(RR_THREADS), 0, st,
                                                      (const uint32_t *)Vcur, Ucur, Gcur, dT, P, m, n, K, th, rkA, gs, groups));
    }
    if (split_rest && *split_rest > 0) --*split_rest;
    else if (split_wanted) {
        bool taken = false;
        rc = split_giant_groups(rkA, rkB, Vcur, Valt, Ucur, Gcur, scratchU, scratchG, m, n, groups, kb, sort_bits, w, st, local, out, tn, &taken,
                                starts_ready);
        if (rc || taken) return rc;
        if (split_rest) *split_rest = 3;
    }
    rc = sort_pairs(rkA, Vcur, rkB, Valt, m, 0, sort_bits, w.ss, nullptr, st, &sr, tn, false, true);
    if (rc) return rc;
    local->sort_passes += sr.passes; local->sorted_elements += (int64_t)sr.passes * m;
    out->keys = sr.keys; out->vals = sr.vals; out->m_global = m;
    out->vnext = (sr.vals == Vcur) ? Valt : Vcur;
    return SA_AMD_OK;
}

static int choose_gram_keys(const uint8_t *dT, int64_t n, KeyParams *Pp, int *key_bits, const Workspace &w, hipStream_t st,
                            const Tuning &tn, bool trace)
{
    KeyParams &P = *Pp;
    const uint64_t se = P.sigma;
    const uint64_t cap = (uint64_t)((size_t)n < GRAM_MAX_ENTRIES ? (size_t)n : GRAM_MAX_ENTRIES);
    int g = 0;
    uint64_t S = 1;
    for (int t = 1; t <= 8; ++t) {
        if (S * se > cap) break;
        S *= se; g = t;
        if (tn.gram_g >= 2 && g == tn.gram_g) break;
    }
    if (g < 2) return SA_AMD_OK;
    uint64_t top = 1;
    for (int t = 0; t + 1 < g; ++t) top *= se;
    const int64_t gtiles = ceil_div((int64_t)S, GT_TILE);
    HIP_TRY(hipMemsetAsync(w.gram_flags, 0, (size_t)S, st));
    PROF(KC_MISC, n, st, hipLaunchKernelGGL((k_gram_mark), dim3((unsigned)ceil_div(ceil_div(n, KB_TILE), GM_TPW)), dim3(KB_THREADS), 0, st, dT, n, P, g,
                                            (uint32_t)top, w.gram_flags));
    PROF(KC_MISC, (int64_t)S, st, hipLaunchKernelGGL((k_gram_count), dim3((unsigned)gtiles), dim3(GT_THREADS), 0, st,
                                            (const uint8_t *)w.gram_flags, (int64_t)S, w.tcnt));
    PROF(KC_RR_SCAN, gtiles, st, hipLaunchKernelGGL((k_rr_scan), dim3(1), dim3(SPINE_THREADS), 0, st, w.tcnt, w.thead, gtiles, w.total));
    uint32_t D = 0;
    { const int rcw = read_words(&D, w.total, 4, st); if (rcw) return rcw; }
    int m = 0;
    unsigned __int128 pw = 1;
    while (D >= 2 && (m + 1) * g <= 64 && pw * D <= ((unsigned __int128)1 << 64)) { pw *= D; ++m; }
    int tail = 0;
    while (m > 0 && tail < tn.gram_tail_max && m * g + tail + 1 <= 64 && pw * se <= ((unsigned __int128)1 << 64)) { pw *= se; ++tail; }
    const int gram_bits = m > 0 ? bit_length((uint64_t)(pw - 1)) : 0;
    const int plain_passes = (int)ceil_div(*key_bits, RADIX_BITS), gram_passes = (int)ceil_div(gram_bits, RADIX_BITS);
    const int syms = m * g + tail;
    const bool better = m > 0 && (syms > P.k || (syms == P.k && gram_passes < plain_passes));
    if (trace) fprintf(stderr, "suffix_array_amd: gram keys: %u of %llu %d-grams occur -> %d symbols (%d grams + %d plain) in %d bits (plain: %d in %d) -> %s\n",
                       D, (unsigned long long)S, g, syms, m, tail, gram_bits, P.k, *key_bits, better ? "gram keys" : "plain keys");
    if (!better) return SA_AMD_OK;
    PROF(KC_MISC, (int64_t)S, st, hipLaunchKernelGGL((k_gram_table), dim3((unsigned)gtiles), dim3(GT_THREADS), 0, st,
                                            (const uint8_t *)w.gram_flags, (int64_t)S, (const uint32_t *)w.tcnt, w.gram_table));
    P.gram = g; P.gram_m = m; P.gram_tail = tail; P.gram_top = (uint32_t)top; P.gram_D = D; P.gram_table = w.gram_table;
    P.bits = 0; P.k = syms; P.mask = ~0ull;
    *key_bits = gram_bits;
    return SA_AMD_OK;
}

struct EarlyDownload {
    int off = 0;
    int64_t threshold = 0;
    std::function<void(hipEvent_t)> start;
    std::function<int64_t()> stop;
    bool started = false;
    int64_t m_snap = 0;
    int64_t covered = 0;
    int64_t holes = 0;
    const uint32_t *d_bits = nullptr, *d_tile_off = nullptr, *d_holes = nullptr;
    hipEvent_t ev = nullptr;
};

struct DeviceBuild {
    const uint8_t *dT;
    uint32_t *dSA, *SA;
    int64_t n;
    hipStream_t st;
    Tuning tn;
    Workspace w;
    sa_amd_stats local;
    EarlyDownload *early = nullptr;
    bool trace = false;
    double trace_t = 0;
    double lap() { const double t = now_ms(), d = t - trace_t; trace_t = t; return d; }
    bool timing_only() const
    {
#ifdef SA_AMD_DIAG
        return tn.timing_only_initial_sort;
#else
        return false;
#endif
    }
    KeyParams P, Ptext;
    int sigma = 0, key_bits = 0, g_bits = 0, top_shift = 0;
    bool force_dense = false, text_ok = false, local_ok = false, probe_dense = false;
    SortResult sr;
    const uint32_t *sorted32 = nullptr;
    int bucket_top_bits = 0;
    bool flat_text = false;
    bool bucket_finished = false;
    uint64_t *sorted0 = nullptr;
    uint32_t *Ucur = nullptr, *Unext = nullptr, *Gcur = nullptr, *Gnext = nullptr, *Vcur = nullptr;
    uint64_t *rkA = nullptr, *rkB = nullptr;
    int64_t tiles = 0, m = 0, depth = 0;
    uint32_t m32 = 0;
    bool lists_ready = false, finished32 = false, fused64 = false, sparse = false;
    bool isa_tail_ranks = false;
    int s_sym = 0, tkb = 0, key2_bits = 0;
    bool unary_done = false;
    bool prev_clean = true;
    int deferred_misses = 0;


    int early_maybe_start()
    {
        if (!early || early->started || m <= 0 || m > early->threshold || !early->start) return SA_AMD_OK;
        if (!early->ev && hipEventCreateWithFlags(&early->ev, hipEventDisableTiming) != hipSuccess) { (void)hipGetLastError(); return SA_AMD_OK; }
        hipLaunchKernelGGL(k_set_u32, dim3(1), dim3(1), 0, st, dSA, (uint32_t)n);
        LAUNCH_CHECK(st);
        HIP_TRY(hipMemsetAsync(w.early_bits, 0, (((size_t)n + 1 + 31) / 32 + EARLY_THREADS) * 4, st));
        int64_t blocks = ceil_div(m, 256 * 8);
        if (blocks > 65536) blocks = 65536;
        if ((((uintptr_t)Ucur) & 15) != 0) return SA_AMD_OK;
        PROF(KC_MISC, m, st, hipLaunchKernelGGL((k_early_mark), dim3((unsigned)blocks), dim3(256), 0, st, (const uint32_t *)Ucur, m, (uint32_t)early->off, w.early_bits));
        HIP_TRY(hipEventRecord(early->ev, st));
        early->started = true;
        early->m_snap = m;
        if (trace) fprintf(stderr, "suffix_array_amd: early download starts with %lld suffixes still tied\n", (long long)m);
        early->start(early->ev);
        return SA_AMD_OK;
    }
    int early_finish()
    {
        if (!early || !early->started) return SA_AMD_OK;
        early->covered = early->stop ? early->stop() : 0;
        if (early->covered > n + early->off) early->covered = n + early->off;
        early->holes = 0;
        if (early->covered <= 0) return SA_AMD_OK;
        const int64_t tiles_e = ceil_div(early->covered, EARLY_TILE);
        const int64_t words = ceil_div(early->covered, 32);
        PROF(KC_MISC, early->covered, st, hipLaunchKernelGGL((k_early_count), dim3((unsigned)tiles_e), dim3(EARLY_THREADS), 0, st,
                                                             (const uint32_t *)w.early_bits, words, w.early_cnt));
        PROF(KC_RR_SCAN, tiles_e, st, hipLaunchKernelGGL((k_rr_scan), dim3(1), dim3(SPINE_THREADS), 0, st, w.early_cnt, (uint32_t *)nullptr, tiles_e, w.early_cnt + tiles_e));
        uint32_t *holes = (uint32_t *)w.keysC;
        PROF(KC_MISC, early->covered, st, hipLaunchKernelGGL((k_early_gather), dim3((unsigned)tiles_e), dim3(EARLY_THREADS), 0, st,
                                                             (const uint32_t *)w.early_bits, words, (const uint32_t *)w.early_cnt,
                                                             (const uint32_t *)(dSA + 1 - early->off), holes));
        uint32_t total = 0;
        { const int rcw = read_words(&total, w.early_cnt + tiles_e, 4, st); if (rcw) return rcw; }
        early->holes = total;
        early->d_bits = w.early_bits; early->d_tile_off = w.early_cnt; early->d_holes = holes;
        return SA_AMD_OK;
    }

    int choose_bucket_bits() const
    {
        if (tn.no_bucket_sort || n < tn.bucket_min_n || n <= 1) return 0;
        const bool wide_ok = onesweep_on(w.ss, tn) && tn.onesweep32_shape == 0;
        if (tn.bucket_bits == 18 && wide_ok) return 18;
        if (tn.bucket_bits == 16) return 16;
        const bool value_bits = wide_ok && !tn.no_value_bits && !tn.no_text_keys && g_bits <= 30 &&
                                ((sigma == 256 && P.bits == 8) || (sigma == 4 && P.bits == 2 && !tn.no_packed_text));
        if (value_bits && (n >> 16) > 7500 && (n >> 18) * 10 <= bucket_cap_max() * 9) return 18;
        if ((n >> 16) * 10 <= bucket_cap(2) * 9) return 16;
        if (wide_ok && (n >> 18) * 10 <= bucket_cap_max() * 9) return 18;
        if ((n >> 16) * 10 <= bucket_cap_max() * 9) return 16;
        return 0;
    }

    bool flat_rule_applies() const { return n >= 2 && n < tn.top32_probe_min_n && n < ((int64_t)1 << 24) && !tn.no_flat_rule; }

    int geometry_and_probes()
    {
        int rc = SA_AMD_OK; (void)rc;
        HIP_TRY(hipMemsetAsync(w.hist, 0, 256 * 4, st));
        {
            int64_t blocks = ceil_div(ceil_div(n, 16), BH_THREADS);
            if (blocks > 2048) blocks = 2048;
            if (blocks < 1) blocks = 1;
            const bool counts = flat_rule_applies();
            if (counts) PROF(KC_BYTE_HIST, n, st, hipLaunchKernelGGL((k_byte_hist_counts), dim3((unsigned)(blocks > 256 ? 256 : blocks)), dim3(BH_THREADS), 0, st, dT, n, w.hist));
            else PROF(KC_BYTE_HIST, n, st, hipLaunchKernelGGL((k_byte_hist), dim3((unsigned)blocks), dim3(BH_THREADS), 0, st, dT, n, w.hist));
        }
        uint32_t hist[256];
        { const int rcw = read_words(hist, w.hist, sizeof(hist), st); if (rcw) return rcw; }
        int kb_max = tn.key_bits_max;
        if (flat_rule_applies()) {
            double h0 = 0.0; int used = 0;
            for (int c = 0; c < 256; ++c)
                if (hist[c]) { const double pc = (double)hist[c] / (double)n; h0 -= pc * std::log2(pc); ++used; }
            if (used >= 2 && h0 > std::log2((double)used) - 0.01) {
                int kb = (bit_length((uint64_t)(n - 1)) + 20 + 7) / 8 * 8;
                if (kb < 32) kb = 32;
                if (kb < kb_max) kb_max = kb;
                flat_text = true;
            }
        }
        key_bits = make_key_params(hist, &P, &sigma, kb_max);
        local.sigma = sigma; local.bits_per_symbol = P.bits; local.symbols_per_key = P.k;
        if (sigma == 1 && !tn.no_unary_shortcut) {
            int64_t blocks = ceil_div(n, 256 * 16);
            if (blocks > 16384) blocks = 16384;
            PROF(KC_MISC, n, st, hipLaunchKernelGGL((k_fill_descending), dim3((unsigned)blocks), dim3(256), 0, st, SA, n));
            unary_done = true;
            return SA_AMD_OK;
        }

        g_bits = bit_length((uint64_t)(n - 1 > 0 ? n - 1 : 1));
        bucket_top_bits = choose_bucket_bits();
        force_dense = tn.force_dense;
        text_ok = !force_dense && !tn.no_text_rounds;
        local_ok = !tn.no_local_sort;

        top_shift = 0;
        if (text_ok && local_ok && key_bits > 32 && !tn.no_top32) {
            bool use = tn.force_top32;
            if (!use && n >= tn.top32_probe_min_n) {
                int64_t S = (int64_t)1 << 20;
                while (S > 1024 && S * 8 > n) S >>= 1;
                PROF(KC_MISC, S, st, hipLaunchKernelGGL((k_sample_keys), dim3((unsigned)ceil_div(S, GK_THREADS)), dim3(GK_THREADS), 0, st, dT, P, n, S,
                                                        key_bits - 32, w.keysA));
                const uint32_t H = (uint32_t)S * 4u;
                HIP_TRY(hipMemsetAsync(w.keysB, 0xff, (size_t)H * 8, st));
                HIP_TRY(hipMemsetAsync(w.total, 0, 8, st));
                PROF(KC_MISC, S, st, hipLaunchKernelGGL((k_count_sample_dups), dim3((unsigned)(ceil_div(S, 256) < 4096 ? ceil_div(S, 256) : 4096)), dim3(256), 0, st, (const uint64_t *)w.keysA, S,
                                                        (unsigned long long *)w.keysB, H - 1u, w.total));
                const int tb = choose_bucket_bits();
                if (tb) {
                    HIP_TRY(hipMemsetAsync(w.keysC, 0, ((size_t)1 << tb) * 4, st));
                    PROF(KC_MISC, S / 4, st, hipLaunchKernelGGL((k_sample_bucket_hist), dim3((unsigned)ceil_div(S / 4, BK_STARTS_THREADS)), dim3(BK_STARTS_THREADS), 0, st,
                                                            (const uint64_t *)w.keysA, S / 4, tb, (uint32_t *)w.keysC));
                    PROF(KC_MISC, S, st, hipLaunchKernelGGL((k_u32_max), dim3((unsigned)(((size_t)1 << tb) / BK_STARTS_THREADS)), dim3(BK_STARTS_THREADS), 0, st,
                                                            (const uint32_t *)w.keysC, 1u << tb, w.total + 1));
                }
                uint32_t dups = 0;
                {
                    uint32_t two[2] = { 0, 0 };
                    const int rcw = read_words(two, w.total, 8, st); if (rcw) return rcw;
                    dups = two[0];
                    const double est = (double)two[1] * (double)n / (double)(S / 4);
                    if (tb && est > 3.0 * (double)bucket_cap_max()) {
                        bucket_top_bits = 0;
                        if (trace) fprintf(stderr, "suffix_array_amd: bucket sort of the 32-bit first stage: largest bucket estimated at %.0f suffixes -> four global passes\n", est);
                    }
                }
                const double p32 = (double)n * 2.0 * (double)dups / ((double)S * (double)S);
                use = p32 < (double)tn.top32_partners_x100 / 100.0;
                double p64 = -1.0;
                if (!use && p32 < 4.0 * (double)tn.top32_collisions_x100 / 100.0) {
                    PROF(KC_MISC, S, st, hipLaunchKernelGGL((k_sample_keys), dim3((unsigned)ceil_div(S, GK_THREADS)), dim3(GK_THREADS), 0, st, dT, P, n, S,
                                                            -1, w.keysA));
                    HIP_TRY(hipMemsetAsync(w.keysB, 0xff, (size_t)H * 8, st));
                    HIP_TRY(hipMemsetAsync(w.total, 0, 4, st));
                    PROF(KC_MISC, S, st, hipLaunchKernelGGL((k_count_sample_dups), dim3((unsigned)(ceil_div(S, 256) < 4096 ? ceil_div(S, 256) : 4096)), dim3(256), 0, st, (const uint64_t *)w.keysA, S,
                                                            (unsigned long long *)w.keysB, H - 1u, w.total));
                    uint32_t dups64 = 0;
                    { const int rcw = read_words(&dups64, w.total, 4, st); if (rcw) return rcw; }
                    const double chance = (double)S * (double)S / 8589934592.0;
                    const double d64 = (double)dups64 > chance ? (double)dups64 - chance : 0.0;
                    p64 = (double)n * 2.0 * d64 / ((double)S * (double)S);
                    use = p64 < 0.8 * (double)tn.top32_partners_x100 / 100.0 && p32 - p64 < (double)tn.top32_collisions_x100 / 100.0;
                }
                if (trace) fprintf(stderr, "suffix_array_amd: entropy probe: %u duplicates of the top 32 key bits among %lld samples -> %.3f expected partners per suffix "
                                           "(on all key bits: %.3f) -> %s\n", dups, (long long)S, p32, p64, use ? "32-bit first stage" : "full keys");
            }
            if (use) top_shift = key_bits - 32;
        }
        local.top32_first = top_shift ? 1 : 0;
        probe_dense = false;
        if (text_ok && local_ok && !top_shift && !force_dense && !tn.no_repeat_probe && n >= ((int64_t)1 << 24)) {
            const int64_t S = (int64_t)1 << 20;
            PROF(KC_MISC, S, st, hipLaunchKernelGGL((k_sample_repeat_keys), dim3((unsigned)ceil_div(S, GK_THREADS)), dim3(GK_THREADS), 0, st, dT, P, n, S,
                                                    w.keysA));
            const uint32_t H = (uint32_t)S * 4u;
            HIP_TRY(hipMemsetAsync(w.keysB, 0xff, (size_t)H * 8, st));
            HIP_TRY(hipMemsetAsync(w.total, 0, 4, st));
            PROF(KC_MISC, S, st, hipLaunchKernelGGL((k_count_sample_dups), dim3((unsigned)(ceil_div(S, 256) < 4096 ? ceil_div(S, 256) : 4096)), dim3(256), 0, st, (const uint64_t *)w.keysA, S,
                                                    (unsigned long long *)w.keysB, H - 1u, w.total));
            uint32_t dups = 0;
            { const int rcw = read_words(&dups, w.total, 4, st); if (rcw) return rcw; }
            const double chance = (double)S * (double)S / 8589934592.0;
            const double frac = ((double)dups - chance) * (double)n / ((double)S * (double)S);
            probe_dense = frac > 0.04;
            if (trace) fprintf(stderr, "suffix_array_amd: repeat probe: %u duplicates among %lld samples (repeat index %.3f, threshold 0.04) -> %s\n",
                               dups, (long long)S, frac, probe_dense ? "rank doubling from the start" : "text-keyed rounds");
        }

        if (!top_shift && !tn.no_gram_keys && n >= tn.gram_min_n && n >= 2 && sigma >= 2 && tn.key_bits_max == 64) {
            const int rcg = choose_gram_keys(dT, n, &P, &key_bits, w, st, tn, trace);
            if (rcg) return rcg;
            local.bits_per_symbol = P.bits; local.symbols_per_key = P.k;
        }

        return SA_AMD_OK;
    }

    int initial_sort_top32(uint32_t *vals0, uint8_t *packed_out, bool iota)
    {
        int rc = SA_AMD_OK; (void)rc;
        uint32_t *k32a = (uint32_t *)w.keysA, *k32b = (uint32_t *)w.keysB;
        int top_bits = bucket_top_bits;
        for (;;) {
            const FirstCounts fc = sort_first_counts(w.ss, tn, n, true);
            const bool counted = n > 1;
            const int rbits = top_bits == 18 ? 9 : RADIX_BITS;
            const bool text_route = top_bits != 0 && counted && iota && top_shift == 32 && onesweep_on(w.ss, tn) && tn.onesweep32_shape == 0 && !tn.no_text_keys;
            const bool text_keys = text_route && sigma == 256 && P.bits == 8 && packed_out == nullptr;
            const bool packed_keys = text_route && sigma == 4 && P.bits == 2 && packed_out != nullptr;
            int val_extra = 0;
            if ((text_keys || packed_keys) && !tn.no_value_bits) {
                val_extra = 32 - g_bits;
                if (val_extra > BK_MAX_LBITS - (32 - top_bits)) val_extra = BK_MAX_LBITS - (32 - top_bits);
                if (val_extra > 2) val_extra = 2;
                if (val_extra < 0) val_extra = 0;
            }
            if (counted) HIP_TRY(hipMemsetAsync(fc.zero_ptr, 0, fc.zero_bytes, st));
            if (text_keys || packed_keys) {
                int split = 2048 / fc.G;
                while (split > 1 && fc.chunk_elems / split < 16384) split /= 2;
                const int64_t sub = (ceil_div(fc.chunk_elems, split) + 15) & ~(int64_t)15;
                if (packed_keys) {
                    int64_t pblocks = ceil_div(ceil_div(n, 16), 256);
                    if (pblocks > 16384) pblocks = 16384;
                    PROF(KC_BUILD_KEYS, n, st, hipLaunchKernelGGL((k_pack_text2), dim3((unsigned)pblocks), dim3(256), 0, st, dT, n, P, packed_out));
                    PROF(KC_BUILD_KEYS, n, st, hipLaunchKernelGGL((k_packed2_upsweep32), dim3((unsigned)(fc.G * split)), dim3(SORT_THREADS), 0, st, (const uint8_t *)packed_out, n,
                                                                  fc.counts, 32 - top_bits, (1u << rbits) - 1u, fc.chunk_elems, fc.G, split, sub));
                } else
                PROF(KC_BUILD_KEYS, n, st, hipLaunchKernelGGL((k_text_upsweep32), dim3((unsigned)(fc.G * split)), dim3(SORT_THREADS), 0, st, dT, n, fc.counts,
                                                              32 - top_bits, (1u << rbits) - 1u, fc.chunk_elems, fc.G, split, sub));
            } else
            PROF(KC_BUILD_KEYS, n, st, hipLaunchKernelGGL((k_build_keys<true>), dim3((unsigned)ceil_div(ceil_div(n, KB_TILE), KB_TPW)), dim3(KB_THREADS), 0, st, dT, n, P,
                                                          (uint64_t *)nullptr, vals0, k32a, top_shift, packed_out,
                                                          counted ? fc.counts : (uint32_t *)nullptr, fc.chunk_elems, fc.G, (1u << rbits) - 1u, top_bits ? 32 - top_bits : 0));
            SortResult32 s32;
            if (top_bits) {
                rc = sort_pairs32(k32a, w.valsA, k32b, w.valsB, n, 32 - top_bits, 32, w.ss, nullptr, st, &s32, tn, iota, counted, rbits,
                                  text_keys ? dT : (packed_keys ? (const uint8_t *)packed_out : (const uint8_t *)nullptr), n, packed_keys ? 2 : 8, val_extra);
                if (rc) return rc;
                local.sort_passes += s32.passes; local.sorted_elements += (int64_t)s32.passes * n;
                uint32_t *kout = (s32.keys == k32a) ? k32b : k32a;
                bool done = false, fused = false;
                uint32_t largest = 0;
                const bool fuse = local_ok && !tn.no_fused_finish && !tn.no_bucket_finish && !timing_only();
                BucketFinish F = BucketFinish();
                KeySrc K = KeySrc();
                if (fuse) {
                    const int64_t rr_tiles = ceil_div(n, RR_TILE);
                    HIP_TRY(hipMemsetAsync(w.surv_bits, 0, ((size_t)n + 31) / 32 * 4, st));
                    HIP_TRY(hipMemsetAsync(w.tcnt, 0, (size_t)rr_tiles * 4, st));
                    HIP_TRY(hipMemsetAsync(w.thead, 0, (size_t)rr_tiles * 4, st));
                    HIP_TRY(hipMemsetAsync(w.total, 0, 16, st));
                    HIP_TRY(hipMemsetAsync(w.chg, 0, (size_t)RR_CHG_COUNTERS * 32 * 4, st));
                    F.T = dT; F.n = n; F.cap = tn.group_cap; F.surv_bits = w.surv_bits; F.surv_head = w.isa; F.tile_cnt = w.tcnt; F.counters = w.total;
                    K.mode = KS_LOWKEY; K.kb = top_shift;
                }
                KeyParams Pf = P;
                Pf.packed = packed_out;
                rc = bucket_sort32(s32.keys, s32.vals, kout, SA, n, top_bits, w.bk_start, w.os_err + 2, st, tn, &done, &largest,
                                   fuse ? &F : nullptr, &Pf, &K, &fused, val_extra);
                if (rc) return rc;
                bucket_finished = done && fused;
                if (trace) fprintf(stderr, "suffix_array_amd: 32-bit first stage: %d global passes over the top %d key bits, largest bucket %u -> %s\n", s32.passes, top_bits, largest,
                                   done ? (fused ? "low bits and ties on all 32 ordered bucket by bucket in LDS" : "low bits ordered bucket by bucket in LDS")
                                        : "too large: keys rebuilt, four global passes");
                if (!done) { top_bits = 0; continue; }
                local.sort_passes += 1; local.sorted_elements += n;
                sorted32 = kout;
                sr.vals = SA; sr.passes = s32.passes + 1;
                sr.keys = (kout == k32a) ? w.keysA : w.keysB;
                break;
            }
            rc = sort_pairs32(k32a, w.valsA, k32b, w.valsB, n, 0, 32, w.ss, SA, st, &s32, tn, iota, counted);
            if (rc) return rc;
            local.sort_passes += s32.passes; local.sorted_elements += (int64_t)s32.passes * n;
            sorted32 = s32.keys;
            sr.vals = s32.vals; sr.passes = s32.passes;
            sr.keys = (s32.keys == k32a) ? w.keysA : w.keysB;
            break;
        }
        return SA_AMD_OK;
    }

    int initial_sort()
    {
        int rc = SA_AMD_OK; (void)rc;
        sr.keys = w.keysA; sr.vals = w.valsA; sr.passes = 0;
        sorted32 = nullptr;
        bucket_finished = false;
        const bool iota = n >= 2 && key_bits > 0;
        uint32_t *vals0 = iota ? (uint32_t *)nullptr : w.valsA;
        uint8_t *packed_out = nullptr;
        if ((P.bits == 1 || P.bits == 2 || P.bits == 4) && n >= 64 && !tn.no_packed_text) {
            packed_out = w.packed;
            HIP_TRY(hipMemsetAsync(packed_out + (size_t)(n >> 3) * P.bits, 0, 64, st));
        }
        if (top_shift) {
            rc = initial_sort_top32(vals0, packed_out, iota);
            if (rc) return rc;
        } else {
            const FirstCounts fc = sort_first_counts(w.ss, tn, n, false);
            const bool counted = n > 1 && key_bits > 0;
            const int nb0 = key_bits < RADIX_BITS ? key_bits : RADIX_BITS;
            if (counted) HIP_TRY(hipMemsetAsync(fc.zero_ptr, 0, fc.zero_bytes, st));
            if (P.gram > 0)
                PROF(KC_BUILD_KEYS, n, st, hipLaunchKernelGGL((k_build_keys<false, true>), dim3((unsigned)ceil_div(ceil_div(n, KB_TILE), KB_TPW)), dim3(KB_THREADS), 0, st, dT, n, P,
                                                              w.keysA, vals0, (uint32_t *)nullptr, 0, packed_out,
                                                              counted ? fc.counts : (uint32_t *)nullptr, fc.chunk_elems, fc.G, (1u << nb0) - 1u));
            else
                PROF(KC_BUILD_KEYS, n, st, hipLaunchKernelGGL((k_build_keys<false>), dim3((unsigned)ceil_div(ceil_div(n, KB_TILE), KB_TPW)), dim3(KB_THREADS), 0, st, dT, n, P,
                                                              w.keysA, vals0, (uint32_t *)nullptr, 0, packed_out,
                                                              counted ? fc.counts : (uint32_t *)nullptr, fc.chunk_elems, fc.G, (1u << nb0) - 1u));
            bool ss_done = false;
#ifdef SA_AMD_DIAG
            if (iota && counted && tn.sample_sort && n >= tn.sample_sort_min_n && key_bits > 32 && onesweep_on(w.ss, tn) && !timing_only()) {
                const size_t need_big = ((size_t)ceil_div(n, SS_TILE) + SS_WAYS) * SS_IDS2 * 4;
                if (need_big <= (size_t)n * 4 && (size_t)n * 4 >= ((size_t)4 << 20)) {
                    rc = sample_sort64(w.keysA, w.keysB, w.keysC, w.valsA, w.valsB, w.U0, w.U1, w.isa, w.G0, w.bk_start, SA, n, key_bits, w.ss, st, &local, tn,
                                       &ss_done, trace);
                    if (rc) return rc;
                    if (ss_done) { sr.keys = w.keysB; sr.vals = SA; sr.passes = 3; sr.skipped = 0; }
                    else {
                        HIP_TRY(hipMemsetAsync(fc.zero_ptr, 0, fc.zero_bytes, st));
                        if (P.gram > 0)
                            PROF(KC_BUILD_KEYS, n, st, hipLaunchKernelGGL((k_build_keys<false, true>), dim3((unsigned)ceil_div(ceil_div(n, KB_TILE), KB_TPW)), dim3(KB_THREADS), 0, st, dT, n, P,
                                                                          w.keysA, vals0, (uint32_t *)nullptr, 0, packed_out, fc.counts, fc.chunk_elems, fc.G, (1u << nb0) - 1u));
                        else
                            PROF(KC_BUILD_KEYS, n, st, hipLaunchKernelGGL((k_build_keys<false>), dim3((unsigned)ceil_div(ceil_div(n, KB_TILE), KB_TPW)), dim3(KB_THREADS), 0, st, dT, n, P,
                                                                          w.keysA, vals0, (uint32_t *)nullptr, 0, packed_out, fc.counts, fc.chunk_elems, fc.G, (1u << nb0) - 1u));
                    }
                }
            }
#endif
            if (!ss_done) {
            rc = sort_pairs(w.keysA, w.valsA, w.keysB, w.valsB, n, 0, key_bits, w.ss, SA, st, &sr, tn, iota, sigma == 1, counted);
            if (rc) return rc;
            local.sort_passes += sr.passes; local.sorted_elements += (int64_t)sr.passes * n;
            }
        }
        P.packed = packed_out;
        if (sr.vals != SA) {
            PROF(KC_MISC, n, st, hipLaunchKernelGGL((k_copy_u32), dim3(1), dim3(256), 0, st, sr.vals, SA, n));
        }

        return SA_AMD_OK;
    }

    int first_round_from_sorted_keys()
    {
        int rc = SA_AMD_OK; (void)rc;
        Ucur = w.U0; Unext = w.U1; Gcur = w.G0; Gnext = w.G1;
        Vcur = w.valsA;
        tiles = ceil_div(n, RR_TILE);
        m32 = 0;
        m = 0;
        rkA = w.keysA; rkB = w.keysB;
        sorted0 = sr.keys;
        lists_ready = false;
        depth = P.k;
        Ptext = P;
        if (P.bits == 0) Ptext.bits = bit_length(P.sigma - 1);
        Ptext.gram = 0;
        s_sym = 0; tkb = 0;
        {
            const int room = 64 - g_bits;
            s_sym = room / Ptext.bits;
            if (s_sym > 64) s_sym = 64;
            tkb = s_sym * Ptext.bits;
        }
        finished32 = false; fused64 = false;
        if (top_shift && local_ok && !tn.no_fused_finish && !timing_only()) {
            const int cap = tn.group_cap;
            uint32_t *surv_bits = w.surv_bits, *surv_head = w.isa;
            if (!bucket_finished) {
            HIP_TRY(hipMemsetAsync(surv_bits, 0, ((size_t)n + 31) / 32 * 4, st));
            HIP_TRY(hipMemsetAsync(w.tcnt, 0, (size_t)tiles * 4, st));
            HIP_TRY(hipMemsetAsync(w.thead, 0, (size_t)tiles * 4, st));
            HIP_TRY(hipMemsetAsync(w.total, 0, 16, st));
            HIP_TRY(hipMemsetAsync(w.chg, 0, (size_t)RR_CHG_COUNTERS * 32 * 4, st));
            KeySrc K = KeySrc(); K.mode = KS_LOWKEY; K.kb = top_shift;
            PROF(KC_FINISH, n, st, hipLaunchKernelGGL((k_finish_sorted<uint32_t, KS_LOWKEY, false>), dim3((unsigned)ceil_div(n, FT_TILE)), dim3(FT_THREADS),
                                                     0, st, sorted32, SA, dT, P, n, K, cap, surv_bits, surv_head, w.tcnt, w.total, (uint32_t *)nullptr,
                                                     (uint32_t *)nullptr, (uint32_t *)nullptr));
            }
            if (!bucket_finished) PROF(KC_RR_SCAN, tiles, st, hipLaunchKernelGGL((k_rr_scan), dim3(1), dim3(SPINE_THREADS), 0, st, w.tcnt, w.thead, tiles, w.total));
            uint32_t cnt3[3] = { 0, 0, 0 };
            {
                uint32_t words[64 + RR_CHG_COUNTERS * 32];
                const int rcw = read_words(words, w.total, sizeof(words), st); if (rcw) return rcw;
                cnt3[0] = words[0]; cnt3[1] = words[1];
                for (int c = 0; c < RR_CHG_COUNTERS; ++c) cnt3[2] += words[64 + c * 32];
                if (bucket_finished) {
                    cnt3[0] = 0;
                    for (int c = 0; c < RR_CHG_COUNTERS; ++c) cnt3[0] += words[64 + c * 32 + 1];
                    if (cnt3[0] != 0 && cnt3[1] == 0)
                        PROF(KC_RR_SCAN, tiles, st, hipLaunchKernelGGL((k_rr_scan), dim3(1), dim3(SPINE_THREADS), 0, st, w.tcnt, w.thead, tiles, w.total));
                }
            }
            if (cnt3[1] == 0) {
                finished32 = true;
                m = cnt3[0];
                local.locally_sorted += cnt3[2];
                local.unresolved_after_initial = m;
                if (m > 0) {
                    PROF(KC_RR_APPLY, n, st, hipLaunchKernelGGL((k_surv_compact), dim3((unsigned)tiles), dim3(256), 0, st, (const uint32_t *)surv_bits,
                                                                (const uint32_t *)surv_head, (const uint32_t *)SA, n, (const uint32_t *)w.tcnt,
                                                                (const uint32_t *)w.total, Ucur, Gcur, Vcur));
                    rkA = (sr.keys == w.keysA) ? w.keysB : w.keysA;
                    rkB = w.keysC;
                    lists_ready = true;
                }
            }
        }
        if (!top_shift && text_ok && local_ok && s_sym > 0 && tn.fused64 && !tn.no_fused_finish && !tn.sparse_div_set && !timing_only()) {
            const int cap = tn.group_cap;
            const int64_t ft_tiles = ceil_div(n, FT_TILE);
            uint32_t *surv_head = w.isa;
            HIP_TRY(hipMemsetAsync(w.surv_bits, 0, ((size_t)n + 31) / 32 * 4, st));
            HIP_TRY(hipMemsetAsync(w.todo_bits, 0, ((size_t)n + 31) / 32 * 4, st));
            HIP_TRY(hipMemsetAsync(w.ft_cnt, 0, (size_t)(ft_tiles + 1) * 4, st));
            HIP_TRY(hipMemsetAsync(w.ft_head, 0, (size_t)(ft_tiles + 1) * 4, st));
            HIP_TRY(hipMemsetAsync(w.surv_cnt, 0, (size_t)tiles * 4, st));
            HIP_TRY(hipMemsetAsync(w.thead, 0, (size_t)tiles * 4, st));
            HIP_TRY(hipMemsetAsync(w.total, 0, 32, st));
            HIP_TRY(hipMemsetAsync(w.chg, 0, (size_t)RR_CHG_COUNTERS * 32 * 4, st));
            KeySrc K = KeySrc(); K.mode = KS_TEXT; K.h = depth; K.s = s_sym; K.kb = tkb;
            PROF(KC_FINISH, n, st, hipLaunchKernelGGL((k_finish_sorted<uint64_t, KS_TEXT, true>), dim3((unsigned)ft_tiles), dim3(FT_THREADS), 0, st,
                                                     (const uint64_t *)sorted0, SA, dT, Ptext, n, K, cap, w.surv_bits, surv_head, w.surv_cnt, w.total,
                                                     w.todo_bits, w.ft_cnt, w.ft_head));
            PROF(KC_RR_SCAN, ft_tiles, st, hipLaunchKernelGGL((k_rr_scan), dim3(1), dim3(SPINE_THREADS), 0, st, w.ft_cnt, w.ft_head, ft_tiles, w.total + 3));
            uint32_t cnt4[4] = { 0, 0, 0, 0 };
            {
                uint32_t words[64 + RR_CHG_COUNTERS * 32];
                const int rcw = read_words(words, w.total, sizeof(words), st); if (rcw) return rcw;
                cnt4[0] = words[0]; cnt4[1] = words[1]; cnt4[3] = words[3];
                for (int c = 0; c < RR_CHG_COUNTERS; ++c) cnt4[2] += words[64 + c * 32];
            }
            local.unresolved_after_initial = cnt4[2];
            const int64_t m_todo = cnt4[3];
            local.locally_sorted += (int64_t)cnt4[2] - m_todo;
            rkA = (sr.keys == w.keysA) ? w.keysB : w.keysA;
            rkB = w.keysC;
            if (m_todo > 0) {
                PROF(KC_RR_APPLY, n, st, hipLaunchKernelGGL((k_todo_compact<uint64_t>), dim3((unsigned)ft_tiles), dim3(FT_THREADS), 0, st,
                                                            (const uint64_t *)sorted0, (const uint32_t *)SA, n, (const uint32_t *)w.todo_bits,
                                                            (const uint32_t *)w.ft_cnt, (const uint32_t *)w.ft_head, (const uint32_t *)(w.total + 3),
                                                            Ucur, Gcur, Vcur));
                uint32_t *Valt = (Vcur == w.valsA) ? w.valsB : w.valsA;
                Refined rf;
                bool big_local = true;
                rc = refine_list(rkA, rkB, Vcur, Valt, Ucur, Gcur, Unext, Gnext, m_todo, n, dT, Ptext, K, g_bits, &big_local, w, st, &local, &rf, tn);
                if (rc) return rc;
                const int64_t tt = ceil_div(m_todo, RR_TILE);
                PROF(KC_RR_COUNT, m_todo, st, hipLaunchKernelGGL((k_rr_count<false>), dim3((unsigned)tt), dim3(RR_THREADS), 0, st, rf.keys,
                                                            (const uint32_t *)Ucur, m_todo, w.ft_cnt, w.ft_head, 0, (uint32_t *)nullptr, 0));
                PROF(KC_RR_SCAN, tt, st, hipLaunchKernelGGL((k_rr_scan), dim3(1), dim3(SPINE_THREADS), 0, st, w.ft_cnt, w.ft_head, tt, w.total + 4));
                PROF(KC_RR_APPLY, m_todo, st, hipLaunchKernelGGL((k_rr_apply<false, true, 4>), dim3((unsigned)tt), dim3(RR_THREADS), 0, st,
                                                            rf.keys, rf.vals, (const uint32_t *)Ucur, m_todo, (const uint32_t *)w.ft_cnt,
                                                            (const uint32_t *)w.ft_head, SA, surv_head, Unext, Gnext, rf.vnext, (uint32_t)n,
                                                            w.surv_bits, 0, (uint64_t *)nullptr, w.surv_cnt, (const uint32_t *)(w.total + 4), 0, (const uint32_t *)nullptr, 0, (uint32_t *)nullptr));
            }
            PROF(KC_RR_SCAN, tiles, st, hipLaunchKernelGGL((k_rr_scan), dim3(1), dim3(SPINE_THREADS), 0, st, w.surv_cnt, w.thead, tiles, w.total));
            { const int rcw = read_words(&m32, w.total, 4, st); if (rcw) return rcw; }
            m = m32;
            Ucur = w.U0; Gcur = w.G0; Vcur = w.valsA; Unext = w.U1; Gnext = w.G1;
            if (m > 0)
                PROF(KC_RR_APPLY, n, st, hipLaunchKernelGGL((k_surv_compact), dim3((unsigned)tiles), dim3(256), 0, st, (const uint32_t *)w.surv_bits,
                                                            (const uint32_t *)surv_head, (const uint32_t *)SA, n, (const uint32_t *)w.surv_cnt,
                                                            (const uint32_t *)w.total, Ucur, Gcur, Vcur));
            fused64 = true;
            lists_ready = true;
            depth += s_sym;
            local.text_rounds++;
            local.rounds++;
        }
        return SA_AMD_OK;
    }

// ... 376 lines not shown
```

### suffix_array_amd/csrc/host/tuning.hpp

```cpp
#pragma once
#include <cstdlib>
#include <cstdint>
#include <atomic>

namespace sa {

constexpr int64_t SPARSE_DIV_DEFAULT = 64;
constexpr int GROUP_CAP_MAX = 1024;

constexpr int UNBWT_SPACING_DEFAULT = 256;
constexpr int UNBWT_SPACING_MAX = 65536;
constexpr int UNBWT_SPACING_MIN = 4;
constexpr int UNBWT_CAP_DEFAULT = 4096;
constexpr int UNBWT_CAP_MAX = 1 << 24;
constexpr int UNBWT_RESTART_WALKS = 64;

inline bool env_flag(const char *name)
{
    const char *e = getenv(name);
    return e && *e && !(e[0] == '0' && e[1] == 0);
}

inline int64_t env_int(const char *name, int64_t def, int64_t lo, int64_t hi)
{
    const char *e = getenv(name);
    if (!e || !*e) return def;
    char *end = nullptr;
    const long long v = strtoll(e, &end, 10);
    if (end == e) return def;
    return v < lo ? lo : (v > hi ? hi : (int64_t)v);
}

inline int env_small_max() { return (int)env_int("SA_AMD_SMALL_MAX", 8192, 0, 8192); }

#ifdef SA_AMD_DIAG
inline std::atomic<int> g_rerank_routes{0};
#endif

struct Tuning {
    int sort_variant = 0;
    int sort32_variant = 0;
    int key_bits_max = 64;
    int group_cap = GROUP_CAP_MAX;
    int64_t sparse_div = SPARSE_DIV_DEFAULT;
    bool sparse_div_set = false;
    bool force_dense = false;
    bool no_text_rounds = false;
    bool no_local_sort = false;
    bool no_top32 = false;
    bool force_top32 = false;
    bool no_fused_finish = false;
    bool fused64 = false;
    bool no_packed_text = false;
    bool no_binned_isa = false;
    bool binned_isa_always = false;
    bool no_run_skip = false;
    int64_t run_skip_min = (int64_t)1 << 25;
    int64_t dense_rekey_min = (int64_t)1 << 22;
    bool no_first_tail = false;
    bool sa_every_round = false;
    bool setup_key_copy = false;
    bool no_repeat_probe = false;
    int64_t binned_min = (int64_t)1 << 26;
    int chase = 7;
    int chase_big = 3;
    int64_t chase_big_min = (int64_t)1 << 23;
    int scatter_levels = 0;
    int max_text_rounds = 4;
    bool no_split = false;
    int64_t split_min = (int64_t)1 << 22;
    int64_t split_group_min = (int64_t)1 << 15;
    bool no_gram_keys = false;
    int64_t gram_min_n = (int64_t)1 << 22;
    int gram_g = 0;
    int gram_tail_max = 8;
    int top32_partners_x100 = 50;
    int top32_collisions_x100 = 400;
    int64_t top32_probe_min_n = (int64_t)1 << 21;
    int small_max = 8192;
    bool no_onesweep = false;
    int onesweep_flags = 0;
    int onesweep64_shape = 0;
    int onesweep32_shape = 0;
    bool no_unary_shortcut = false;
    int64_t count_next_min_n = 20000000;
    int64_t count_next_below_n = 393216;
    int network_min = 256;
    bool no_upfront_counts = false;
    bool no_flat_rule = false;
    bool no_posted_readback = false;
    bool no_defer = false;
    bool no_big_group_sort = false;
    bool no_text_keys = false;
    bool no_value_bits = false;
    bool no_bucket_sort = false;
    int64_t bucket_min_n = (int64_t)1 << 25;
    bool no_bucket_finish = false;
    bool bucket_finish_always = false;
    int bucket_bits = 0;
    int bucket_shape = -1;
#ifdef SA_AMD_DIAG
    bool sample_sort = false;
    int64_t sample_sort_min_n = (int64_t)1 << 26;
    bool sample_merge = false;
    int sample_log = 0;
    bool timing_only_initial_sort = false;
#endif

    static Tuning from_env(int n_sort_variants, int n_sort32_variants, int n_os64 = 1, int n_os32 = 1)
    {
        Tuning t;
        t.sort_variant = (int)env_int("SA_AMD_SORT_VARIANT", 0, 0, 1 << 20);
        if (t.sort_variant >= n_sort_variants) t.sort_variant = 0;
        t.sort32_variant = (int)env_int("SA_AMD_SORT32_VARIANT", 0, 0, 1 << 20);
        if (t.sort32_variant >= n_sort32_variants) t.sort32_variant = 0;
        t.key_bits_max = (int)env_int("SA_AMD_KEY_BITS", 64, 16, 64);
        t.group_cap = (int)env_int("SA_AMD_GROUP_CAP", GROUP_CAP_MAX, 2, GROUP_CAP_MAX);
        t.sparse_div_set = getenv("SA_AMD_SPARSE_DIV") != nullptr;
        t.sparse_div = env_int("SA_AMD_SPARSE_DIV", SPARSE_DIV_DEFAULT, 1, (int64_t)1 << 40);
        t.force_dense = env_flag("SA_AMD_FORCE_DENSE");
        t.no_text_rounds = env_flag("SA_AMD_NO_TEXT_ROUNDS");
        t.no_local_sort = env_flag("SA_AMD_NO_LOCAL_SORT");
        t.no_top32 = env_flag("SA_AMD_NO_TOP32");
        t.force_top32 = env_flag("SA_AMD_FORCE_TOP32");
        t.no_fused_finish = env_flag("SA_AMD_NO_FUSED_FINISH");
        t.fused64 = env_flag("SA_AMD_FUSED64");
        t.no_packed_text = env_flag("SA_AMD_NO_PACKED_TEXT");
        t.no_binned_isa = env_flag("SA_AMD_NO_BINNED_ISA");
        t.binned_isa_always = env_flag("SA_AMD_BINNED_ISA_ALWAYS");
        t.no_run_skip = env_flag("SA_AMD_NO_RUN_SKIP");
        t.run_skip_min = env_int("SA_AMD_RUN_SKIP_MIN", (int64_t)1 << 25, 1, (int64_t)1 << 40);
        t.no_first_tail = env_flag("SA_AMD_NO_FIRST_TAIL");
        t.no_repeat_probe = env_flag("SA_AMD_NO_REPEAT_PROBE");
        t.dense_rekey_min = env_int("SA_AMD_DENSE_REKEY_MIN", (int64_t)1 << 22, 1, (int64_t)1 << 40);
        t.max_text_rounds = (int)env_int("SA_AMD_MAX_TEXT_ROUNDS", 4, 0, 8);
        t.chase = (int)env_int("SA_AMD_CHASE", 7, 1, 15);
        t.chase_big = (int)env_int("SA_AMD_CHASE_BIG", 3, 1, 15);
        t.chase_big_min = env_int("SA_AMD_CHASE_BIG_MIN", (int64_t)1 << 23, 1, (int64_t)1 << 40);
        t.scatter_levels = (int)env_int("SA_AMD_SCATTER_LEVELS", 0, 0, 2);
        t.binned_min = env_int("SA_AMD_BINNED_MIN", (int64_t)1 << 26, 1, (int64_t)1 << 40);
        t.no_split = env_flag("SA_AMD_NO_SPLIT");
        t.split_min = env_int("SA_AMD_SPLIT_MIN", (int64_t)1 << 22, 1, (int64_t)1 << 40);
        t.split_group_min = env_int("SA_AMD_SPLIT_GROUP_MIN", (int64_t)1 << 15, 1, (int64_t)1 << 40);
        t.no_gram_keys = env_flag("SA_AMD_NO_GRAM_KEYS");
        t.gram_min_n = env_int("SA_AMD_GRAM_MIN_N", (int64_t)1 << 22, 1, (int64_t)1 << 40);
        t.gram_g = (int)env_int("SA_AMD_GRAM_G", 0, 0, 8);
        t.gram_tail_max = (int)env_int("SA_AMD_GRAM_TAIL", 8, 0, 8);
        t.top32_partners_x100 = (int)env_int("SA_AMD_TOP32_PARTNERS_X100", 50, 0, 1000000);
        t.top32_collisions_x100 = (int)env_int("SA_AMD_TOP32_COLLISIONS_X100", 400, 0, 1000000);
        t.top32_probe_min_n = env_int("SA_AMD_TOP32_PROBE_MIN_N", (int64_t)1 << 21, 8192, (int64_t)1 << 40);
        t.small_max = env_small_max();
        t.no_onesweep = env_flag("SA_AMD_NO_ONESWEEP");
        t.onesweep_flags = (int)env_int("SA_AMD_ONESWEEP_FLAGS", 0, 0, 255);
        t.onesweep64_shape = (int)env_int("SA_AMD_ONESWEEP64_SHAPE", 0, 0, 1 << 20);
        if (t.onesweep64_shape >= n_os64) t.onesweep64_shape = 0;
        t.onesweep32_shape = (int)env_int("SA_AMD_ONESWEEP32_SHAPE", 0, 0, 1 << 20);
        if (t.onesweep32_shape >= n_os32) t.onesweep32_shape = 0;
        t.no_big_group_sort = env_flag("SA_AMD_NO_BIG_GROUP_SORT");
        t.no_defer = env_flag("SA_AMD_NO_DEFER");
        t.no_posted_readback = env_flag("SA_AMD_NO_POSTED_READBACK");
        t.no_flat_rule = env_flag("SA_AMD_NO_FLAT_RULE");
        t.no_upfront_counts = env_flag("SA_AMD_NO_UPFRONT_COUNTS");
        t.network_min = (int)env_int("SA_AMD_NETWORK_MIN", 256, 0, 1 << 20);
        t.count_next_min_n = env_int("SA_AMD_COUNT_NEXT_MIN_N", 20000000, 0, (int64_t)1 << 40);
        t.count_next_below_n = env_int("SA_AMD_COUNT_NEXT_BELOW_N", 393216, 0, (int64_t)1 << 40);
        t.no_unary_shortcut = env_flag("SA_AMD_NO_UNARY_SHORTCUT");

        t.no_text_keys = env_flag("SA_AMD_NO_TEXT_KEYS");
        t.no_value_bits = env_flag("SA_AMD_NO_VALUE_BITS");
        t.no_bucket_sort = env_flag("SA_AMD_NO_BUCKET_SORT");
        t.bucket_min_n = env_int("SA_AMD_BUCKET_MIN_N", (int64_t)1 << 25, 1, (int64_t)1 << 40);
        t.no_bucket_finish = env_flag("SA_AMD_NO_BUCKET_FINISH");
        t.bucket_finish_always = env_flag("SA_AMD_BUCKET_FINISH_ALWAYS");
        t.bucket_bits = (int)env_int("SA_AMD_BUCKET_BITS", 0, 0, 18);
        if (t.bucket_bits != 16 && t.bucket_bits != 18) t.bucket_bits = 0;
        t.bucket_shape = (int)env_int("SA_AMD_BUCKET_SHAPE", -1, -1, 64);
#ifdef SA_AMD_DIAG
        t.sample_sort = env_flag("SA_AMD_SAMPLE_SORT");
        t.sample_merge = env_flag("SA_AMD_SAMPLE_MERGE");
        t.sample_sort_min_n = env_int("SA_AMD_SAMPLE_SORT_MIN_N", (int64_t)1 << 26, (int64_t)1 << 17, (int64_t)1 << 40);
        t.sample_log = (int)env_int("SA_AMD_SAMPLE_LOG", 0, 0, 24);
        if (t.sample_log != 0 && t.sample_log < 16) t.sample_log = 16;
        t.timing_only_initial_sort = env_flag("SA_AMD_TIMING_ONLY_INITIAL_SORT");
        {
            const int r = g_rerank_routes.load(std::memory_order_relaxed);
            t.sa_every_round = (r & 1) != 0;
            t.setup_key_copy = (r & 2) != 0;
        }
#endif
        return t;
    }
};

constexpr size_t STAGE_BYTES = (size_t)16 << 20;

struct HostTuning {
    int small_max;
    int copy_threads;
    size_t staged_min;
    bool prefault;
    int prefault_keep;
    bool prefault_wait;
    int64_t early_div;
    size_t early_min;
    size_t early_chunk;
    int64_t early_wait;
    bool reduced;
    bool lanes;
    int64_t lanes_min_n;
    bool kernel_d2h;
    bool kernel_d2h_always;
    int verbose;

    static HostTuning from_env()
    {
        HostTuning h;
        h.small_max = env_small_max();
        h.copy_threads = (int)env_int("SA_AMD_COPY_THREADS", 12, 0, 32);
        h.staged_min = (size_t)env_int("SA_AMD_STAGED_MIN_BYTES", (int64_t)64 << 20, 0, (int64_t)1 << 40);
        h.prefault = env_int("SA_AMD_NO_PREFAULT", 0, 0, 1) == 0;
        h.prefault_keep = (int)env_int("SA_AMD_PREFAULT_KEEP", 3, 0, 32);
        h.prefault_wait = env_int("SA_AMD_PREFAULT_WAIT", 0, 0, 1) != 0;
        h.early_div = env_int("SA_AMD_EARLY_DIV", 4, 0, 1 << 20);
        h.early_min = (size_t)env_int("SA_AMD_EARLY_MIN_BYTES", (int64_t)128 << 20, 0, (int64_t)1 << 40);
        h.early_chunk = (size_t)env_int("SA_AMD_EARLY_CHUNK_BYTES", (int64_t)STAGE_BYTES, 65536, (int64_t)STAGE_BYTES) & ~(size_t)4095;
        h.early_wait = env_int("SA_AMD_EARLY_WAIT_CHUNKS", 0, 0, 1 << 20);
        h.reduced = env_int("SA_AMD_NO_REDUCED", 0, 0, 1) == 0;
        h.lanes = env_int("SA_AMD_NO_LANES", 0, 0, 1) == 0;
        h.lanes_min_n = env_int("SA_AMD_LANES_MIN_N", (int64_t)32 << 20, 0, (int64_t)1 << 40);
        h.kernel_d2h = env_int("SA_AMD_NO_KERNEL_D2H", 0, 0, 1) == 0;
        h.kernel_d2h_always = env_int("SA_AMD_KERNEL_D2H_ALWAYS", 0, 0, 1) != 0;
        h.verbose = (int)env_int("SA_AMD_VERBOSE", 0, 0, 9);
        return h;
    }
};

}
```

### suffix_array_amd/csrc/kernels/keys.hpp

```cpp
#pragma once
#include "common.hpp"

namespace sa {

constexpr int BH_THREADS = 256;

__global__ __launch_bounds__(BH_THREADS) void k_byte_hist(const uint8_t *__restrict__ T, int64_t n,
                                                           uint32_t *__restrict__ hist)
{
    __shared__ uint32_t h[256];
    h[threadIdx.x] = 0;
    __syncthreads();
    const uintptr_t addr = (uintptr_t)T;
    int64_t head = (int64_t)((16 - (addr & 15)) & 15);
    if (head > n) head = n;
    const int64_t nvec = (n - head) / 16;
    const uint4 *V = (const uint4 *)(T + head);
    const int64_t gtid = (int64_t)blockIdx.x * BH_THREADS + threadIdx.x;
    const int64_t gstride = (int64_t)gridDim.x * BH_THREADS;
    for (int64_t i = gtid; i < nvec; i += gstride) {
        uint4 q = V[i];
        uint32_t w4[4] = { q.x, q.y, q.z, q.w };
#pragma unroll
        for (int a = 0; a < 4; ++a) {
#pragma unroll
            for (int b = 0; b < 4; ++b) h[(w4[a] >> (8 * b)) & 255u] = 1u;
        }
    }
    if (blockIdx.x == 0) {
        for (int64_t i = threadIdx.x; i < head; i += BH_THREADS) h[T[i]] = 1u;
        for (int64_t i = head + nvec * 16 + threadIdx.x; i < n; i += BH_THREADS) h[T[i]] = 1u;
    }
    __syncthreads();
    if (h[threadIdx.x]) hist[threadIdx.x] = 1u;
}

__global__ __launch_bounds__(BH_THREADS) void k_byte_hist_counts(const uint8_t *__restrict__ T, int64_t n, uint32_t *__restrict__ hist)
{
    __shared__ uint32_t h[BH_THREADS / WAVE][256];
    for (int i = threadIdx.x; i < (BH_THREADS / WAVE) * 256; i += BH_THREADS) (&h[0][0])[i] = 0;
    __syncthreads();
    uint32_t *mine = h[wave_id()];
    const uintptr_t addr = (uintptr_t)T;
    int64_t head = (int64_t)((16 - (addr & 15)) & 15);
    if (head > n) head = n;
    const int64_t nvec = (n - head) / 16;
    const uint4 *V = (const uint4 *)(T + head);
    const int64_t gtid = (int64_t)blockIdx.x * BH_THREADS + threadIdx.x;
    const int64_t gstride = (int64_t)gridDim.x * BH_THREADS;
    for (int64_t i = gtid; i < nvec; i += gstride) {
        const uint4 q = V[i];
        const uint32_t w4[4] = { q.x, q.y, q.z, q.w };
#pragma unroll
        for (int a = 0; a < 4; ++a) {
#pragma unroll
            for (int b = 0; b < 4; ++b) atomicAdd(&mine[(w4[a] >> (8 * b)) & 255u], 1u);
        }
    }
    if (blockIdx.x == 0) {
        for (int64_t i = threadIdx.x; i < head; i += BH_THREADS) atomicAdd(&mine[T[i]], 1u);
        for (int64_t i = head + nvec * 16 + threadIdx.x; i < n; i += BH_THREADS) atomicAdd(&mine[T[i]], 1u);
    }
    __syncthreads();
    uint32_t c = 0;
#pragma unroll
    for (int w = 0; w < BH_THREADS / WAVE; ++w) c += h[w][threadIdx.x];
    if (c) atomicAdd(&hist[threadIdx.x], c);
}

constexpr int KB_THREADS = 256;
constexpr int KB_ITEMS = 8;
constexpr int KB_TILE = KB_THREADS * KB_ITEMS;
constexpr int KB_HALO = 64 + 8;

struct KeyParams {
    uint8_t code[256];
    int32_t bits;
    int32_t k;
    uint64_t mask;
    uint64_t sigma;
    uint64_t top;
    const uint8_t *packed;
    int32_t gram, gram_m, gram_tail;
    uint32_t gram_top;
    uint64_t gram_D;
    const uint4 *gram_table;
};

__device__ __forceinline__ uint32_t gram_rank(const uint4 *__restrict__ table, uint32_t idx)
{
    const uint4 rec = table[idx >> 6];
    const uint64_t bits = ((uint64_t)rec.y << 32) | rec.x;
    return rec.z + (uint32_t)__popcll(bits & ((1ull << (idx & 63u)) - 1ull));
}

__device__ __forceinline__ void kb_stage_codes(const uint8_t *__restrict__ T, int64_t n, int64_t base, const uint8_t *lcode, uint8_t *c, int tid);

constexpr int KB_TPW = 8;
constexpr int GM_LOG = 13;
constexpr int GRAM_CACHE = 1 << GM_LOG;
constexpr int GM_TPW = 64;
__device__ __forceinline__ uint32_t gram_slot(uint32_t idx) { return (idx * 2654435761u) >> (32 - GM_LOG); }

template <bool TOP32, bool GRAM = false>
__global__ __launch_bounds__(KB_THREADS) void k_build_keys(const uint8_t *__restrict__ T, int64_t n,
                                                            KeyParams P, uint64_t *__restrict__ keys,
                                                            uint32_t *__restrict__ vals, uint32_t *__restrict__ keys32,
                                                            int top_shift, uint8_t *__restrict__ packed_out,
                                                            uint32_t *__restrict__ counts, int64_t chunk_elems, int G, uint32_t dmask, int dshift = 0)
{
    __shared__ uint8_t lcode[256];
    __shared__ __attribute__((aligned(16))) uint8_t c[KB_TILE + KB_HALO];
    __shared__ uint32_t dhist[512];
    __shared__ uint32_t gc[GRAM ? KB_TILE + KB_HALO : 1];
    const int tid = threadIdx.x;
    lcode[tid] = P.code[tid];
    for (int d = tid; d < 512; d += KB_THREADS) dhist[d] = 0;

    __syncthreads();
    const int64_t tiles = (n + KB_TILE - 1) / KB_TILE;
    const int64_t tile0 = (int64_t)blockIdx.x * KB_TPW;
    const int64_t tile1 = tile0 + KB_TPW < tiles ? tile0 + KB_TPW : tiles;
  for (int64_t tile = tile0; tile < tile1; ++tile) {
    const int64_t base = tile * KB_TILE;
    kb_stage_codes(T, n, base, lcode, c, tid);
    __syncthreads();
    const int p0 = tid * KB_ITEMS;
    const int k = P.k, bits = P.bits;
    uint64_t kk[KB_ITEMS];
    if (GRAM) {
        const int g = P.gram, m = P.gram_m;
        const uint32_t sg = (uint32_t)P.sigma;
        for (int o = tid; o + g <= KB_TILE + KB_HALO; o += KB_THREADS) {
            uint32_t idx = 0;
            for (int t = 0; t < g; ++t) idx = idx * sg + (uint32_t)c[o + t];
            gc[o] = gram_rank(P.gram_table, idx);
        }
        __syncthreads();
        const uint64_t D = P.gram_D;
        const int tail = P.gram_tail;
#pragma unroll
        for (int r = 0; r < KB_ITEMS; ++r) {
            uint64_t key = 0;
            for (int j = 0; j < m; ++j) key = key * D + (uint64_t)gc[p0 + r + g * j];
            for (int t = 0; t < tail; ++t) key = key * (uint64_t)sg + (uint64_t)c[p0 + r + g * m + t];
            kk[r] = key;
        }
    } else if (bits > 0) {
        const uint64_t mask = P.mask;
        uint64_t key = 0;
        for (int j = 0; j < k; ++j) key = (key << bits) | (uint64_t)c[p0 + j];
        kk[0] = key;
#pragma unroll
        for (int r = 1; r < KB_ITEMS; ++r) {
            key = ((key << bits) | (uint64_t)c[p0 + k - 1 + r]) & mask;
            kk[r] = key;
        }
    } else {
        const uint64_t sigma = P.sigma, top = P.top;
        uint64_t key = 0;
        for (int j = 0; j < k; ++j) key = key * sigma + (uint64_t)c[p0 + j];
        kk[0] = key;
#pragma unroll
        for (int r = 1; r < KB_ITEMS; ++r) {
            key = (key - (uint64_t)c[p0 + r - 1] * top) * sigma + (uint64_t)c[p0 + k - 1 + r];
            kk[r] = key;
        }
    }
    const int64_t g0 = base + p0;
    if (packed_out && g0 < n) {
        uint32_t val = 0;
#pragma unroll
        for (int r = 0; r < KB_ITEMS; ++r) val = (val << bits) | (uint32_t)c[p0 + r];
        uint8_t *po = packed_out + (g0 >> 3) * bits;
        for (int b = 0; b < bits; ++b) po[b] = (uint8_t)(val >> (8 * (bits - 1 - b)));
    }
    if (g0 + KB_ITEMS <= n) {
        if (TOP32) {
            uint4 *ko = (uint4 *)(keys32 + g0);
            ko[0] = make_uint4((uint32_t)(kk[0] >> top_shift), (uint32_t)(kk[1] >> top_shift), (uint32_t)(kk[2] >> top_shift),
                               (uint32_t)(kk[3] >> top_shift));
            ko[1] = make_uint4((uint32_t)(kk[4] >> top_shift), (uint32_t)(kk[5] >> top_shift), (uint32_t)(kk[6] >> top_shift),
                               (uint32_t)(kk[7] >> top_shift));
        } else {
            ulonglong2 *ko = (ulonglong2 *)(keys + g0);
#pragma unroll
            for (int r = 0; r < KB_ITEMS / 2; ++r) ko[r] = make_ulonglong2(kk[2 * r], kk[2 * r + 1]);
        }
        if (vals) {
            uint4 *vo = (uint4 *)(vals + g0);
            const uint32_t v0 = (uint32_t)g0;
            vo[0] = make_uint4(v0, v0 + 1, v0 + 2, v0 + 3);
            vo[1] = make_uint4(v0 + 4, v0 + 5, v0 + 6, v0 + 7);
        }
    } else {
#pragma unroll
        for (int r = 0; r < KB_ITEMS; ++r)
            if (g0 + r < n) {
                if (TOP32) keys32[g0 + r] = (uint32_t)(kk[r] >> top_shift); else keys[g0 + r] = kk[r];
                if (vals) vals[g0 + r] = (uint32_t)(g0 + r);
            }
    }
    if (counts) {
#pragma unroll
        for (int r = 0; r < KB_ITEMS; ++r) {
            const bool in = g0 + r < n;
            const uint32_t d = (uint32_t)((TOP32 ? (kk[r] >> top_shift) : kk[r]) >> dshift) & dmask;
            const uint64_t act = __ballot(in);
            const uint32_t f = (uint32_t)__builtin_amdgcn_readfirstlane((int)d);
            if (__all(!in || d == f)) {
                if (act && lane_id() == __ffsll((unsigned long long)act) - 1) atomicAdd(&dhist[d], (uint32_t)__popcll(act));
            } else if (in) atomicAdd(&dhist[d], 1u);
        }
    }
    __syncthreads();
    if (counts) {
        const int64_t chunk = base / chunk_elems;
        const bool flush = tile + 1 == tile1 || (base + KB_TILE) / chunk_elems != chunk;
        if (flush) {
            for (int d = tid; d <= (int)dmask; d += KB_THREADS) {
                const uint32_t cnt = dhist[d];
                if (cnt) atomicAdd(&counts[(int64_t)d * G + chunk], cnt);
                dhist[d] = 0;
            }
            __syncthreads();
        }
    }
  }
}

__device__ __forceinline__ void kb_stage_codes(const uint8_t *__restrict__ T, int64_t n, int64_t base, const uint8_t *lcode, uint8_t *c, int tid)
{
    for (int o = tid * 8; o < KB_TILE + KB_HALO; o += KB_THREADS * 8) {
        const int64_t p = base + o;
        uint8_t b[8];
        if (p + 8 <= n && (((uintptr_t)(T + p)) & 7) == 0) {
            uint2 q = *(const uint2 *)(T + p);
            uint32_t w2[2] = { q.x, q.y };
#pragma unroll
            for (int j = 0; j < 8; ++j) b[j] = lcode[(w2[j >> 2] >> (8 * (j & 3))) & 255u];
        } else {
#pragma unroll
            for (int j = 0; j < 8; ++j) b[j] = (p + j < n) ? lcode[T[p + j]] : (uint8_t)0;
        }
        uint2 o2;
        o2.x = (uint32_t)b[0] | ((uint32_t)b[1] << 8) | ((uint32_t)b[2] << 16) | ((uint32_t)b[3] << 24);
        o2.y = (uint32_t)b[4] | ((uint32_t)b[5] << 8) | ((uint32_t)b[6] << 16) | ((uint32_t)b[7] << 24);
        *(uint2 *)(c + o) = o2;
    }
}

__global__ __launch_bounds__(KB_THREADS) void k_gram_mark(const uint8_t *__restrict__ T, int64_t n, KeyParams P, int g, uint32_t top,
                                                           uint8_t *__restrict__ F)
{
    __shared__ uint8_t lcode[256];
    __shared__ __attribute__((aligned(16))) uint8_t c[KB_TILE + KB_HALO];
    __shared__ uint32_t s_tag[GRAM_CACHE];
    const int tid = threadIdx.x;
    lcode[tid] = P.code[tid];
    for (int i = tid; i < GRAM_CACHE; i += KB_THREADS) s_tag[i] = 0xffffffffu;
    __syncthreads();
    const int64_t tiles = (n + KB_TILE - 1) / KB_TILE;
    const int64_t tile0 = (int64_t)blockIdx.x * GM_TPW;
    const int64_t tile1 = tile0 + GM_TPW < tiles ? tile0 + GM_TPW : tiles;
    const uint32_t sg = (uint32_t)P.sigma;
    for (int64_t tile = tile0; tile < tile1; ++tile) {
        const int64_t base = tile * KB_TILE;
        kb_stage_codes(T, n, base, lcode, c, tid);
        __syncthreads();
        const int p0 = tid * KB_ITEMS;
        uint32_t idx = 0;
        for (int t = 0; t < g; ++t) idx = idx * sg + (uint32_t)c[p0 + t];
        uint32_t ix[KB_ITEMS];
        bool miss[KB_ITEMS];
#pragma unroll
        for (int r = 0; r < KB_ITEMS; ++r) {
            ix[r] = idx;
            const uint32_t sl = gram_slot(idx);
            miss[r] = base + p0 + r < n && s_tag[sl] != idx;
            if (miss[r]) s_tag[sl] = idx;
            idx = (idx - (uint32_t)c[p0 + r] * top) * sg + (uint32_t)c[p0 + r + g];
        }
        uint8_t f[KB_ITEMS];
#pragma unroll
        for (int r = 0; r < KB_ITEMS; ++r) f[r] = miss[r] ? F[ix[r]] : (uint8_t)1;
#pragma unroll
        for (int r = 0; r < KB_ITEMS; ++r) if (miss[r] && f[r] == 0) F[ix[r]] = 1;
        __syncthreads();
    }
    if (blockIdx.x == 0 && tid == 0) F[0] = 1;
}

constexpr int GT_THREADS = 1024;
constexpr int GT_TILE = GT_THREADS * 64;
__device__ __forceinline__ uint64_t gram_word(const uint8_t *__restrict__ F, int64_t S, int64_t i0)
{
    uint64_t w = 0;
    if (i0 + 64 <= S) {
        const uint4 *q = (const uint4 *)(F + i0);
#pragma unroll
        for (int a = 0; a < 4; ++a) {
            const uint4 v = q[a];
            const uint32_t ww[4] = { v.x, v.y, v.z, v.w };
#pragma unroll
            for (int b = 0; b < 16; ++b) w |= (uint64_t)((ww[b >> 2] >> (8 * (b & 3))) & 1u) << (16 * a + b);
        }
    } else {
        for (int j = 0; j < 64; ++j) if (i0 + j < S && F[i0 + j]) w |= 1ull << j;
    }
    return w;
}

__global__ __launch_bounds__(GT_THREADS) void k_gram_count(const uint8_t *__restrict__ F, int64_t S, uint32_t *__restrict__ tile_cnt)
{
    __shared__ uint32_t lds[GT_THREADS / WAVE];
    const int64_t i0 = (int64_t)blockIdx.x * GT_TILE + (int64_t)threadIdx.x * 64;
    const uint32_t c = i0 < S ? (uint32_t)__popcll(gram_word(F, S, i0)) : 0u;
    uint32_t tot;
    (void)block_excl_sum<GT_THREADS>(c, lds, &tot);
    if (threadIdx.x == 0) tile_cnt[blockIdx.x] = tot;
}

__global__ __launch_bounds__(GT_THREADS) void k_gram_table(const uint8_t *__restrict__ F, int64_t S, const uint32_t *__restrict__ tile_off,
                                                            uint4 *__restrict__ table)
{
    __shared__ uint32_t lds[GT_THREADS / WAVE];
    const int64_t i0 = (int64_t)blockIdx.x * GT_TILE + (int64_t)threadIdx.x * 64;
    const uint64_t w = i0 < S ? gram_word(F, S, i0) : 0ull;
    uint32_t tot;
    const uint32_t off = tile_off[blockIdx.x] + block_excl_sum<GT_THREADS>((uint32_t)__popcll(w), lds, &tot);
    if (i0 < S) table[i0 >> 6] = make_uint4((uint32_t)w, (uint32_t)(w >> 32), off, 0u);
}

constexpr int GK_THREADS = 256;

__device__ __forceinline__ uint64_t code_at(const uint8_t *__restrict__ T, const uint8_t *lcode, int64_t n, int64_t pos)
{
    return pos < n ? (uint64_t)lcode[T[pos]] : 0ull;
}

__device__ __forceinline__ uint64_t text_key(const uint8_t *__restrict__ T, const uint8_t *lcode, const KeyParams &P, int64_t n,
                                             int64_t p, int nsym, bool aligned8)
{
    uint64_t tk = 0;
    if (P.gram > 0 && nsym == P.k) {
        const uint32_t sg = (uint32_t)P.sigma;
        for (int j = 0; j < P.gram_m; ++j) {
            uint32_t idx = 0;
            for (int t = 0; t < P.gram; ++t) idx = idx * sg + (uint32_t)code_at(T, lcode, n, p + (int64_t)P.gram * j + t);
            tk = tk * P.gram_D + (uint64_t)gram_rank(P.gram_table, idx);
        }
        for (int t = 0; t < P.gram_tail; ++t) tk = tk * P.sigma + code_at(T, lcode, n, p + (int64_t)P.gram * P.gram_m + t);
        return tk;
    }
    if (P.packed) {
        const int64_t bo = p * P.bits;
        const int nb = nsym * P.bits;
        if (nb == 0 || p >= n) return 0;
        const uint64_t *W = (const uint64_t *)P.packed + (bo >> 6);
        const uint64_t w0 = __builtin_bswap64(W[0]), w1 = __builtin_bswap64(W[1]);
        const int sh = (int)(bo & 63);
        const uint64_t val = sh ? ((w0 << sh) | (w1 >> (64 - sh))) : w0;
        return val >> (64 - nb);
    }
    if (aligned8 && p + nsym + 16 <= n) {
        const uint64_t *W = (const uint64_t *)(T + (p & ~(int64_t)7));
        const int sh = (int)(p & 7) * 8;
        uint64_t w0 = W[0];
        for (int done = 0, wi = 1; done < nsym; done += 8, ++wi) {
            const uint64_t w1 = W[wi];
            const uint64_t bytes = sh ? ((w0 >> sh) | (w1 << (64 - sh))) : w0;
            const int cnt = nsym - done < 8 ? nsym - done : 8;
            for (int i = 0; i < cnt; ++i) {
                const uint64_t cs = (uint64_t)lcode[(bytes >> (8 * i)) & 255u];
                tk = P.bits > 0 ? ((tk << P.bits) | cs) : (tk * P.sigma + cs);
            }
            w0 = w1;
        }
    } else {
        for (int i = 0; i < nsym; ++i) {
            const uint64_t cs = code_at(T, lcode, n, p + i);
            tk = P.bits > 0 ? ((tk << P.bits) | cs) : (tk * P.sigma + cs);
        }
    }
    return tk;
}

__global__ __launch_bounds__(GK_THREADS) void k_sample_keys(const uint8_t *__restrict__ T, KeyParams P, int64_t n, int64_t samples,
                                                             int top_shift, uint64_t *__restrict__ out)
{
    __shared__ uint8_t lcode[256];
    lcode[threadIdx.x] = P.code[threadIdx.x];
    __syncthreads();
    const int64_t i = (int64_t)blockIdx.x * GK_THREADS + threadIdx.x;
    if (i >= samples) return;
    const uint64_t r = ((uint64_t)i + 1u) * 0x9E3779B97F4A7C15ull;
    const int64_t p = (int64_t)((r >> 11) % (uint64_t)n);
    const uint64_t kq = text_key(T, lcode, P, n, p, P.k, (((uintptr_t)T) & 7) == 0);
    uint64_t part = kq >> (top_shift < 0 ? 0 : top_shift);
    if (top_shift < 0) {
        part ^= part >> 33; part *= 0xff51afd7ed558ccdull; part ^= part >> 33; part *= 0xc4ceb9fe1a85ec53ull; part ^= part >> 33;
    }
    out[i] = (part << 32) | (uint64_t)(uint32_t)p;
}

__global__ __launch_bounds__(GK_THREADS) void k_sample_repeat_keys(const uint8_t *__restrict__ T, KeyParams P, int64_t n, int64_t samples,
                                                                    uint64_t *__restrict__ out)
{
    __shared__ uint8_t lcode[256];
    lcode[threadIdx.x] = P.code[threadIdx.x];
    __syncthreads();
    const int64_t i = (int64_t)blockIdx.x * GK_THREADS + threadIdx.x;
    if (i >= samples) return;
    const uint64_t r = ((uint64_t)i + 1u) * 0xD1B54A32D192ED03ull;
    const int64_t p = (int64_t)((r >> 11) % (uint64_t)n);
    const bool al = (((uintptr_t)T) & 7) == 0;
    uint64_t h = text_key(T, lcode, P, n, p, P.k, al) * 0x9E3779B97F4A7C15ull;
    h ^= h >> 29;
    h += text_key(T, lcode, P, n, p + P.k, P.k, al) * 0xBF58476D1CE4E5B9ull;
    h ^= h >> 32;
    h *= 0x94D049BB133111EBull;
    out[i] = (h & 0xffffffff00000000ull) | (uint64_t)(uint32_t)p;
}

__global__ __launch_bounds__(256) void k_count_sample_dups(const uint64_t *__restrict__ samples, int64_t count, unsigned long long *table,
                                                            uint32_t table_mask, uint32_t *__restrict__ dups)
{
    __shared__ uint32_t wsum[256 / WAVE];
    uint32_t c = 0;
    for (int64_t i = (int64_t)blockIdx.x * 256 + threadIdx.x; i < count; i += (int64_t)gridDim.x * 256) {
        const unsigned long long e = samples[i];
        const uint32_t k = (uint32_t)(e >> 32);
        uint32_t h = (k * 2654435761u) >> 7;
        for (;;) {
            h &= table_mask;
            unsigned long long old = __atomic_load_n(&table[h], __ATOMIC_RELAXED);
            if (old == ~0ull) old = atomicCAS(&table[h], ~0ull, e);
            if (old == ~0ull) break;
            if ((uint32_t)(old >> 32) == k) { c += old != e ? 1u : 0u; break; }
            ++h;
        }
    }
#pragma unroll
    for (int o = 32; o > 0; o >>= 1) c += __shfl_xor(c, o, WAVE);
    if (lane_id() == 0) wsum[wave_id()] = c;
    __syncthreads();
    if (threadIdx.x == 0) {
        uint32_t t = 0;
        for (int w = 0; w < 256 / WAVE; ++w) t += wsum[w];
        if (t) atomicAdd(dups, t);
    }
}

}
```

### suffix_array_amd/csrc/sa_api.hip

```cpp
#include "host/support.hpp"
#include "host/tuning.hpp"
#include "host/pipeline.hpp"
#include "host/host_path.hpp"
#include "host/lcp.hpp"
#include "host/esa.hpp"
#include "host/bwt.hpp"
#include "host/repeats.hpp"
#include "host/lz.hpp"
#include "host/match.hpp"

extern "C" {

#define SA_EXPORT __attribute__((visibility("default")))

SA_EXPORT int32_t sa_amd_max_length(void) { return SA_AMD_MAX_LENGTH; }

SA_EXPORT int32_t sa_amd_divsufsort(const uint8_t *T, int32_t *SA, int32_t n)
{
    SA_ABI_GUARD_BEGIN
    return sa::build_host(T, (uint32_t *)SA, n, false, sa::pick_device());
    SA_ABI_GUARD_END(0)
}

SA_EXPORT int32_t sa_amd_saca_u8(const uint8_t *T, uint32_t *SA, int32_t n)
{
    SA_ABI_GUARD_BEGIN
    return sa::build_host(T, SA, n, true, sa::pick_device());
    SA_ABI_GUARD_END(0)
}

SA_EXPORT int32_t sa_amd_saca_batch(const uint8_t *const *T, uint32_t *const *SA, const int32_t *n, const int32_t *device,
                                    int32_t count, int32_t *status)
{
    if (count < 0 || (count > 0 && (!T || !SA || !n))) return SA_AMD_EINVAL;
    int ndev = 0;
    if (hipGetDeviceCount(&ndev) != hipSuccess || ndev <= 0) return SA_AMD_ENODEVICE;
    SA_ABI_GUARD_BEGIN
    std::vector<int32_t> st((size_t)count, SA_AMD_OK);
    std::vector<std::vector<int>> per_dev((size_t)ndev), small_dev((size_t)ndev);
    const sa::HostTuning ht = sa::HostTuning::from_env();
    for (int i = 0; i < count; ++i) {
        const int d = device ? device[i] : i % ndev;
        if (d < 0 || d >= ndev) { st[(size_t)i] = SA_AMD_EINVAL; continue; }
        if (n[i] > 0 && n[i] <= ht.small_max && T[i] && SA[i]) small_dev[(size_t)d].push_back(i);
        else per_dev[(size_t)d].push_back(i);
    }
    for (int d = 0; d < ndev; ++d)
        if (small_dev[(size_t)d].size() == 1) { per_dev[(size_t)d].push_back(small_dev[(size_t)d][0]); small_dev[(size_t)d].clear(); }
    std::vector<std::atomic<int>> small_taken((size_t)ndev);
    for (auto &a : small_taken) a.store(0);
    const int per_env = (int)sa::env_int("SA_AMD_BATCH_THREADS", 0, 0, 16);
    const int64_t lanes_min = ht.lanes_min_n;
    std::vector<int> per_of((size_t)ndev, 2);
    for (int d = 0; d < ndev; ++d) {
        int64_t largest = 0;
        for (int i : per_dev[(size_t)d]) largest = n[i] > largest ? n[i] : largest;
        per_of[(size_t)d] = per_env > 0 ? per_env : (largest < lanes_min ? (largest < ((int64_t)8 << 20) ? 12 : 6) : 2);
    }
    std::vector<std::atomic<size_t>> next((size_t)ndev);
    for (auto &a : next) a.store(0);
    auto work = [&](int d) {
        if (!small_dev[(size_t)d].empty() && small_taken[(size_t)d].exchange(1) == 0) {
            try { (void)sa::build_host_small_batch(T, SA, n, small_dev[(size_t)d].data(), small_dev[(size_t)d].size(), d, st.data()); }
            catch (const std::bad_alloc &) { for (int i : small_dev[(size_t)d]) st[(size_t)i] = SA_AMD_ENOMEM; }
            catch (...) { for (int i : small_dev[(size_t)d]) st[(size_t)i] = SA_AMD_EINTERNAL; }
        }
        for (;;) {
            const size_t q = next[(size_t)d].fetch_add(1);
            if (q >= per_dev[(size_t)d].size()) break;
            const int i = per_dev[(size_t)d][q];
            int32_t rc;
            try { rc = sa::build_host(T[i], SA[i], n[i], true, d); }
            catch (const std::bad_alloc &) { rc = SA_AMD_ENOMEM; }
            catch (...) { rc = SA_AMD_EINTERNAL; }
            st[(size_t)i] = rc;
        }
    };
    std::vector<std::thread> workers;
    bool spawn_failed = false;
    for (int d = 0; d < ndev && !spawn_failed; ++d) {
        const size_t items = per_dev[(size_t)d].size() + (small_dev[(size_t)d].empty() ? 0 : 1);
        for (int k = 0; k < per_of[(size_t)d] && (size_t)k < items; ++k) {
            try { workers.emplace_back(work, d); }
            catch (...) { spawn_failed = true; break; }
        }
    }
    for (auto &t : workers) t.join();
    if (spawn_failed)
        for (int d = 0; d < ndev; ++d) work(d);
    int32_t first = SA_AMD_OK;
    for (int i = 0; i < count; ++i) {
        if (status) status[i] = st[(size_t)i];
        if (first == SA_AMD_OK && st[(size_t)i] != SA_AMD_OK) first = st[(size_t)i];
    }
    return first;
    SA_ABI_GUARD_END(0)
}

SA_EXPORT int64_t sa_amd_workspace_bytes(int32_t n)
{
    if (n < 0) return -1;
    return (int64_t)sa::carve(nullptr, n).bytes;
}

SA_EXPORT int32_t sa_amd_saca_device(const uint8_t *dT, uint32_t *dSA, int32_t n, void *dWork, int64_t work_bytes,
                                     void *stream, sa_amd_stats *stats)
{
    if (n < 0 || !dSA || (n > 0 && (!dT || !dWork))) return SA_AMD_EINVAL;
    if (n > 0 && (((uintptr_t)dWork) & 255u)) return SA_AMD_EINVAL;
    SA_ABI_GUARD_BEGIN
    return sa::build_device(dT, dSA, n, dWork, work_bytes, (hipStream_t)stream, stats);
    SA_ABI_GUARD_END(0)
}


SA_EXPORT int32_t sa_amd_bucket_table_device(const uint8_t *dT, const uint32_t *dSA, int32_t n, uint32_t *dBkt, void *stream)
{
    SA_ABI_GUARD_BEGIN
    if (n < 0 || !dBkt || (n > 0 && !dT)) return SA_AMD_EINVAL;
    hipStream_t st = (hipStream_t)stream;
    if (dSA) {
        hipLaunchKernelGGL(sa::k_bucket_table, dim3((sa::BKT_LEN + 255) / 256), dim3(256), 0, st, dT, dSA, (int64_t)n, dBkt);
    } else {
        if (hipMemsetAsync(dBkt, 0, (size_t)65536 * 4, st) != hipSuccess) return SA_AMD_EHIP;
        int64_t pairs = sa::ceil_div((int64_t)n, sa::BG_MIN_CHUNK);
        if (pairs > sa::BG_MAX_PAIRS) pairs = sa::BG_MAX_PAIRS;
        if (n >= 2)
            hipLaunchKernelGGL(sa::k_bigram_hist, dim3((unsigned)(2 * pairs)), dim3(sa::BG_THREADS), 0, st, dT, (int64_t)n, (int)pairs, dBkt);
        hipLaunchKernelGGL(sa::k_bigram_scan, dim3(1), dim3(sa::BGS_THREADS), 0, st, (const uint32_t *)dBkt, dT, (int64_t)n, dBkt);
    }
    if (hipGetLastError() != hipSuccess) return SA_AMD_EHIP;
    return hipStreamSynchronize(st) == hipSuccess ? SA_AMD_OK : SA_AMD_EHIP;
    SA_ABI_GUARD_END(0)
}

struct CiLayout { size_t flags, rank, alt, alt_elems, spine, status, err, starts, bitmap, bitmap_bytes, bytes; };
static CiLayout ci_layout(int32_t n)
{
    CiLayout L;
    const size_t N1 = (size_t)n + 1;
    size_t off = 0;
    auto take = [&](size_t b) { const size_t o = off; off = sa::align_up(off + b, 256); return o; };
    L.flags = take(256);
    L.rank = take(N1 * 4);
    L.alt_elems = (N1 + 67) & ~(size_t)3;
    L.alt = take(4 * L.alt_elems * 4);
    L.spine = take(((size_t)sa::RADIX * sa::SORT_MAX_WG + sa::RADIX) * 4);
    L.status = take(((size_t)sa::ceil_div((int64_t)N1, sa::OS_MIN_TILE) + 1) * sa::RADIX * 8);
    L.err = take(256);
    L.starts = take(257 * 4);
    L.bitmap_bytes = ((N1 + 31) / 32 + 1) * 4;
    L.bitmap = take(L.bitmap_bytes);
    L.bytes = off;
    return L;
}

SA_EXPORT int64_t sa_amd_check_integrity_work_bytes(int32_t n)
{
    if (n < 0) return -1;
    return (int64_t)ci_layout(n).bytes;
}

SA_EXPORT int32_t sa_amd_check_integrity_device(const uint8_t *dT, int32_t n, const uint32_t *dSA, void *dWork,
                                                int64_t work_bytes, void *stream)
{
    if (n < 0 || !dSA || !dWork || (n > 0 && !dT)) return SA_AMD_EINVAL;
    if (work_bytes < ((int64_t)n + 1) * 4 + 256) return SA_AMD_EINVAL;
    SA_ABI_GUARD_BEGIN
    using namespace sa;
    hipStream_t st = (hipStream_t)stream;
    uint32_t *flags = (uint32_t *)dWork;
    uint32_t *rank = (uint32_t *)((char *)dWork + 256);
    HIP_TRY(hipMemsetAsync(flags, 0, 4, st));
    int64_t blocks = ((int64_t)n + 1 + 255) / 256;
    if (blocks > 16384) blocks = 16384;
    const CiLayout L = ci_layout(n);
    if (work_bytes >= (int64_t)L.bytes && (((uintptr_t)dWork) & 255u) == 0 && (((uintptr_t)dSA) & 15u) == 0 && n >= 2) {
        hipLaunchKernelGGL(k_ci_range, dim3((unsigned)blocks), dim3(256), 0, st, dSA, (int64_t)n, flags);
        HIP_TRY(hipGetLastError());
        uint32_t f = 0;
        { const int rcw = read_words(&f, flags, 4, st); if (rcw) return rcw; }
        if (f & 1u) return SA_AMD_ERANGE;
        if (f & 2u) return 0;
        char *base = (char *)dWork;
        Workspace w;
        memset(&w, 0, sizeof(w));
        w.isa = (uint32_t *)(base + L.rank);
        w.spine = (uint32_t *)(base + L.spine);
        w.digit_tot = w.spine + (size_t)RADIX * SORT_MAX_WG;
        w.os_status = (unsigned long long *)(base + L.status);
        w.os_err = (uint32_t *)(base + L.err);
        w.ss.spine = w.spine; w.ss.digit_tot = w.digit_tot; w.ss.status = w.os_status; w.ss.err = w.os_err;
        HIP_TRY(hipMemsetAsync(w.os_err, 0, 16, st));
        uint32_t *alt = (uint32_t *)(base + L.alt);
        const Tuning tn = Tuning::from_env(N_SORT_VARIANTS, N_SORT32_VARIANTS, N_OS_SHAPES64, N_OS_SHAPES32);
        sa_amd_stats local;
        memset(&local, 0, sizeof(local));
        const int rcs = scatter_binned((uint32_t *)dSA, nullptr, alt, alt + L.alt_elems, (int64_t)n + 1, (int64_t)n, w, st, &local, tn, true,
                                       alt + 2 * L.alt_elems, alt + 3 * L.alt_elems);
        if (rcs) return rcs;
        uint32_t *starts = (uint32_t *)(base + L.starts), *bitmap = (uint32_t *)(base + L.bitmap);
        HIP_TRY(hipMemsetAsync(bitmap, 0, L.bitmap_bytes, st));
        hipLaunchKernelGGL(k_ci_starts, dim3(1), dim3(512), 0, st, dT, dSA, (int64_t)n, starts, bitmap);
        int64_t fblocks = ceil_div((int64_t)n, 256 * 16);
        if (fblocks > 16384) fblocks = 16384;
        hipLaunchKernelGGL(k_ci_first_bytes, dim3((unsigned)fblocks), dim3(256), 0, st, dT, (int64_t)n, (const uint32_t *)w.isa, (const uint32_t *)starts, flags);
        const int64_t cblocks = ceil_div((int64_t)n, (int64_t)CI_THREADS * CI_ITEMS);
        hipLaunchKernelGGL(k_ci_check_shared, dim3((unsigned)cblocks), dim3(CI_THREADS), 0, st, dSA, (int64_t)n, (const uint32_t *)w.isa,
                           (const uint32_t *)bitmap, flags);
        HIP_TRY(hipGetLastError());
        uint32_t words[2] = { 0, 0 };
        { const int rcw = read_words(&words[0], flags, 4, st); if (rcw) return rcw; }
        { const int rcw = read_words(&words[1], w.os_err, 4, st); if (rcw) return rcw; }
        if (words[1]) return SA_AMD_EINTERNAL;
        return (words[0] & 2u) ? 0 : 1;
    }
    hipLaunchKernelGGL(sa::k_ci_scatter, dim3((unsigned)blocks), dim3(256), 0, st, dSA, (int64_t)n, rank, flags);
    hipLaunchKernelGGL(sa::k_ci_check, dim3((unsigned)blocks), dim3(256), 0, st, dT, dSA, (int64_t)n, (const uint32_t *)rank, flags);
    if (hipGetLastError() != hipSuccess) return SA_AMD_EHIP;
    uint32_t f = 0;
    if (hipMemcpyAsync(&f, flags, 4, hipMemcpyDeviceToHost, st) != hipSuccess) return SA_AMD_EHIP;
    if (hipStreamSynchronize(st) != hipSuccess) return SA_AMD_EHIP;
    if (f & 1u) return SA_AMD_ERANGE;
    return (f & 2u) ? 0 : 1;
    SA_ABI_GUARD_END(0)
}

static int32_t bucket_table_host(const uint8_t *T, int32_t n, uint32_t *bkt)
{
    using namespace sa;
    if (n < 0 || !bkt || (n > 0 && !T)) return SA_AMD_EINVAL;
    if (sa_amd_device_count() <= 0) return SA_AMD_ENODEVICE;
    DeviceGuard guard(pick_device());
    if (guard.rc != SA_AMD_OK) return guard.rc;
    int cur = 0;
    HIP_TRY(hipGetDevice(&cur));
    const size_t tb = align_up((size_t)n + 16, 256);
    DevBlock blk;
    hipStream_t st = nullptr;
    int32_t rc = pool().stream(cur, &st);
    if (rc != SA_AMD_OK) return rc;
    rc = pool().acquire(cur, tb + (size_t)BKT_LEN * 4, &blk);
    if (rc != SA_AMD_OK) { pool().release_stream(cur, st); return rc; }
    uint8_t *dT = (uint8_t *)blk.p;
    uint32_t *dB = (uint32_t *)((char *)blk.p + tb);
    if (n > 0) rc = hip_status(hipMemcpyAsync(dT, T, (size_t)n, hipMemcpyHostToDevice, st));
    if (rc == SA_AMD_OK) rc = sa_amd_bucket_table_device(dT, nullptr, n, dB, st);
    if (rc == SA_AMD_OK) rc = hip_status(hipMemcpyAsync(bkt, dB, (size_t)BKT_LEN * 4, hipMemcpyDeviceToHost, st));
    const int32_t rs = hip_status(hipStreamSynchronize(st));
    if (rc == SA_AMD_OK) rc = rs;
    pool().release(blk);
    pool().release_stream(cur, st);
    return rc;
}

static int32_t extras_host(const uint8_t *T, int32_t n, uint32_t *SA, int64_t sa_len, uint32_t *bkt, int which)
{
    using namespace sa;
    if (n < 0 || !SA || (n > 0 && !T)) return SA_AMD_EINVAL;
    if (sa_amd_device_count() <= 0) return SA_AMD_ENODEVICE;
    if (which == 2 && sa_len != (int64_t)n + 1) return 0;
    DeviceGuard guard(pick_device());
    if (guard.rc != SA_AMD_OK) return guard.rc;
    DevBuf dT, dSA, dB, dW;
    int32_t rc;
    const size_t N = (size_t)n;
// ... 824 lines not shown
```

Before: 5665 MB/s.

## Add two-level gram-rank keys to pack more symbols per sort key

Adds a second gram level: ranks of (g+e)-grams are built over level-1 gram ranks extended by e plain symbols. Keys are then composed from level-2 grams, level-1 grams and a plain tail to fit more symbols into 64 bits or to need fewer radix passes. The aim is to resolve more suffixes in the initial sort and shorten later refinement. It costs an extra mark/count/scan/table pass with a host readback, extra shared memory in key building, and a second rank table in the workspace. It is on by default for n >= 2^28, which matches this input size exactly.

```diff
diff --git a/include/suffix_array_amd.h b/include/suffix_array_amd.h
--- a/include/suffix_array_amd.h
+++ b/include/suffix_array_amd.h
@@ -47,6 +47,9 @@
 
 int32_t sa_amd_saca_device(const uint8_t *dT, uint32_t *dSA, int32_t n, void *dWork,
                            int64_t work_bytes, void *stream, sa_amd_stats *stats);
+
+int32_t sa_amd_set_gram_levels(int32_t levels, int64_t min_n);
+int64_t sa_amd_gram2_min_n(void);
 
 void sa_amd_release_cache(void);
 
diff --git a/suffix_array_amd/__init__.py b/suffix_array_amd/__init__.py
--- a/suffix_array_amd/__init__.py
+++ b/suffix_array_amd/__init__.py
@@ -7,7 +7,7 @@
 import numpy as np
 
 __all__ = ["MAX_LENGTH", "saca", "SuffixArray", "SuffixArrayError", "lib", "diag_lib", "library_path", "Stats", "last_host_timing",
-           "saca_batch", "workspace_bytes", "device_pci_bus_id", "saca_device_ptr", "bucket_table", "check_integrity", "last_stats", "DeviceIndex", "pack", "unpack",
+           "saca_batch", "workspace_bytes", "set_gram_levels", "gram2_min_n", "device_pci_bus_id", "saca_device_ptr", "bucket_table", "check_integrity", "last_stats", "DeviceIndex", "pack", "unpack",
            "lcp", "saca_lcp", "last_lcp_stats", "lcp_work_bytes", "lcp_device_ptr", "LcpStats",
            "lcp_set_compare_cap", "last_search_stats", "SearchStats",
            "bwt", "unbwt", "bwt_device_ptr", "unbwt_device_ptr", "bwt_work_bytes", "unbwt_work_bytes", "last_unbwt_stats",
@@ -132,6 +132,9 @@
         L.sa_amd_workspace_bytes.restype = ctypes.c_int64
         L.sa_amd_saca_device.argtypes = [c_vp, c_vp, ctypes.c_int32, c_vp, ctypes.c_int64, c_vp, c_vp]
         L.sa_amd_saca_device.restype = ctypes.c_int32
+        L.sa_amd_set_gram_levels.argtypes = [ctypes.c_int32, ctypes.c_int64]
+        L.sa_amd_set_gram_levels.restype = ctypes.c_int32
+        L.sa_amd_gram2_min_n.restype = ctypes.c_int64
         L.sa_amd_device_count.restype = ctypes.c_int32
         L.sa_amd_device_pci_bus_id.argtypes = [ctypes.c_int32, ctypes.c_char_p, ctypes.c_int32]
         L.sa_amd_device_pci_bus_id.restype = ctypes.c_int32
@@ -308,7 +311,10 @@
         L.sa_amd_saca_device.restype = ctypes.c_int32
         L.sa_amd_workspace_bytes.argtypes = [ctypes.c_int32]
         L.sa_amd_workspace_bytes.restype = ctypes.c_int64
+        L.sa_amd_set_gram_levels.argtypes = [ctypes.c_int32, ctypes.c_int64]
+        L.sa_amd_set_gram_levels.restype = ctypes.c_int32
         L.sa_amd_version.restype = ctypes.c_char_p
+        L.sa_amd_set_gram_levels(lib().sa_amd_set_gram_levels(0, 0), lib().sa_amd_gram2_min_n())
         _diag = L
     return _diag
 
@@ -826,6 +832,16 @@
         return {"contains": c.astype(bool), "lo": lo, "hi": hi, "lcp_start": ls, "lcp_len": ll}
 
 
+def set_gram_levels(levels: int = 0, min_n: int = 0) -> int:
+    if _diag is not None:
+        _diag.sa_amd_set_gram_levels(int(levels), int(min_n))
+    return int(lib().sa_amd_set_gram_levels(int(levels), int(min_n)))
+
+
+def gram2_min_n() -> int:
+    return int(lib().sa_amd_gram2_min_n())
+
+
 def workspace_bytes(n: int) -> int:
     return int(lib().sa_amd_workspace_bytes(n))
 
diff --git a/suffix_array_amd/csrc/host/pipeline.hpp b/suffix_array_amd/csrc/host/pipeline.hpp
--- a/suffix_array_amd/csrc/host/pipeline.hpp
+++ b/suffix_array_amd/csrc/host/pipeline.hpp
@@ -67,6 +67,7 @@
     uint8_t *packed;
     uint8_t *gram_flags;
     uint4 *gram_table;
+    uint4 *gram_table2;
     uint32_t *surv_bits, *surv_cnt, *todo_bits, *ft_cnt, *ft_head;
     unsigned long long *os_status;
     uint32_t *os_err;
@@ -104,6 +105,7 @@
     w.bk_start = (uint32_t *)take(((size_t)BK_BUCKETS_MAX + 1) * 4);
     w.early_cnt = (uint32_t *)take(((N + 1 + EARLY_TILE - 1) / EARLY_TILE + 8) * 4);
     w.gram_table = (uint4 *)take((gram_entries / 64 + 1) * 16);
+    w.gram_table2 = (uint4 *)take((gram_entries / 64 + 1) * 16);
     w.has_isa = (uint32_t *)take((N + 31) / 32 * 4);
     w.surv_bits = (uint32_t *)take((N + 31) / 32 * 4);
     w.todo_bits = (uint32_t *)take((N + 31) / 32 * 4);
@@ -649,6 +651,7 @@
     *sigma_out = sigma;
     P->packed = nullptr;
     P->gram = 0; P->gram_m = 0; P->gram_tail = 0; P->gram_top = 0; P->gram_D = 0; P->gram_table = nullptr;
+    P->gram2_e = 0; P->gram2_m = 0; P->gram2_D = 0; P->gram2_table = nullptr;
     const uint64_t se = sigma > 2 ? (uint64_t)sigma : 2u;
     P->sigma = se;
     if ((se & (se - 1)) == 0) {
@@ -1033,8 +1036,34 @@
     return SA_AMD_OK;
 }
 
+struct GramComposition { int m2, m1, t, syms, bits, passes; };
+static GramComposition compose_gram_key(uint64_t D2, int g2, uint64_t D1, int g1, uint64_t se, int tail_max)
+{
+    GramComposition best = { 0, 0, 0, 0, 0, 0 };
+    const unsigned __int128 lim = (unsigned __int128)1 << 64;
+    unsigned __int128 p2 = 1;
+    for (int m2 = 1; m2 * g2 <= 64; ++m2) {
+        if (D2 < 2 || p2 * D2 > lim) break;
+        p2 *= D2;
+        unsigned __int128 p1 = p2;
+        for (int m1 = 0; m2 * g2 + m1 * g1 <= 64; ++m1) {
+            if (m1 > 0) { if (D1 < 2 || p1 * D1 > lim) break; p1 *= D1; }
+            unsigned __int128 pw = p1;
+            for (int t = 0; t <= tail_max && m2 * g2 + m1 * g1 + t <= 64; ++t) {
+                if (t > 0) { if (pw * se > lim) break; pw *= se; }
+                GramComposition c = { m2, m1, t, m2 * g2 + m1 * g1 + t, bit_length((uint64_t)(pw - 1)), 0 };
+                c.passes = (int)ceil_div(c.bits, RADIX_BITS);
+                const bool wins = c.syms > best.syms || (c.syms == best.syms && (c.passes < best.passes ||
+                                  (c.passes == best.passes && c.m2 + c.m1 + c.t < best.m2 + best.m1 + best.t)));
+                if (wins) best = c;
+            }
+        }
+    }
+    return best;
+}
+
 static int choose_gram_keys(const uint8_t *dT, int64_t n, KeyParams *Pp, int *key_bits, const Workspace &w, hipStream_t st,
-                            const Tuning &tn, bool trace)
+                            const Tuning &tn, bool trace, bool level2_ok)
 {
     KeyParams &P = *Pp;
     const uint64_t se = P.sigma;
@@ -1051,8 +1080,8 @@
     for (int t = 0; t + 1 < g; ++t) top *= se;
     const int64_t gtiles = ceil_div((int64_t)S, GT_TILE);
     HIP_TRY(hipMemsetAsync(w.gram_flags, 0, (size_t)S, st));
-    PROF(KC_MISC, n, st, hipLaunchKernelGGL((k_gram_mark), dim3((unsigned)ceil_div(ceil_div(n, KB_TILE), GM_TPW)), dim3(KB_THREADS), 0, st, dT, n, P, g,
-                                            (uint32_t)top, w.gram_flags));
+    PROF(KC_MISC, n, st, hipLaunchKernelGGL((k_gram_mark<false>), dim3((unsigned)ceil_div(ceil_div(n, KB_TILE), GM_TPW)), dim3(KB_THREADS), 0, st, dT, n, P, g,
+                                            (uint32_t)top, 0, w.gram_flags));
     PROF(KC_MISC, (int64_t)S, st, hipLaunchKernelGGL((k_gram_count), dim3((unsigned)gtiles), dim3(GT_THREADS), 0, st,
                                             (const uint8_t *)w.gram_flags, (int64_t)S, w.tcnt));
     PROF(KC_RR_SCAN, gtiles, st, hipLaunchKernelGGL((k_rr_scan), dim3(1), dim3(SPINE_THREADS), 0, st, w.tcnt, w.thead, gtiles, w.total));
@@ -1075,6 +1104,36 @@
     P.gram = g; P.gram_m = m; P.gram_tail = tail; P.gram_top = (uint32_t)top; P.gram_D = D; P.gram_table = w.gram_table;
     P.bits = 0; P.k = syms; P.mask = ~0ull;
     *key_bits = gram_bits;
+    if (tn.gram_levels < 2 || n < tn.gram2_min_n || tn.gram_tail_max == 0 || !level2_ok) return SA_AMD_OK;
+
+    int e = 0;
+    uint64_t S2 = D;
+    while (S2 * se <= cap) { S2 *= se; ++e; }
+    if (e < 1) return SA_AMD_OK;
+    {
+        const GramComposition ub = compose_gram_key(D, g + e, D, g, se, tn.gram_tail_max);
+        if (!(ub.m2 > 0 && (ub.syms > syms || (ub.syms == syms && ub.passes < gram_passes)))) return SA_AMD_OK;
+    }
+    const int64_t gtiles2 = ceil_div((int64_t)S2, GT_TILE);
+    HIP_TRY(hipMemsetAsync(w.gram_flags, 0, (size_t)S2, st));
+    PROF(KC_MISC, n, st, hipLaunchKernelGGL((k_gram_mark<true>), dim3((unsigned)ceil_div(ceil_div(n, KB_TILE), GM_TPW)), dim3(KB_THREADS), 0, st, dT, n, P, g,
+                                            (uint32_t)top, e, w.gram_flags));
+    PROF(KC_MISC, (int64_t)S2, st, hipLaunchKernelGGL((k_gram_count), dim3((unsigned)gtiles2), dim3(GT_THREADS), 0, st,
+                                            (const uint8_t *)w.gram_flags, (int64_t)S2, w.tcnt));
+    PROF(KC_RR_SCAN, gtiles2, st, hipLaunchKernelGGL((k_rr_scan), dim3(1), dim3(SPINE_THREADS), 0, st, w.tcnt, w.thead, gtiles2, w.total));
+    uint32_t D2 = 0;
+    { const int rcw = read_words(&D2, w.total, 4, st); if (rcw) return rcw; }
+    const GramComposition c2 = compose_gram_key(D2, g + e, D, g, se, tn.gram_tail_max);
+    const bool better2 = c2.m2 > 0 && (c2.syms > syms || (c2.syms == syms && c2.passes < gram_passes));
+    if (trace) fprintf(stderr, "suffix_array_amd: gram keys, level 2: %u of %llu (%d+%d)-grams occur -> %d symbols (%d level-2 + %d level-1 grams + %d plain) in %d bits (level 1: %d in %d) -> %s\n",
+                       D2, (unsigned long long)S2, g, e, c2.syms, c2.m2, c2.m1, c2.t, c2.bits, syms, gram_bits, better2 ? "level 2" : "level 1");
+    if (!better2) return SA_AMD_OK;
+    PROF(KC_MISC, (int64_t)S2, st, hipLaunchKernelGGL((k_gram_table), dim3((unsigned)gtiles2), dim3(GT_THREADS), 0, st,
+                                            (const uint8_t *)w.gram_flags, (int64_t)S2, (const uint32_t *)w.tcnt, w.gram_table2));
+    P.gram2_e = e; P.gram2_m = c2.m2; P.gram2_D = D2; P.gram2_table = w.gram_table2;
+    P.gram_m = c2.m1; P.gram_tail = c2.t;
+    P.k = c2.syms;
+    *key_bits = c2.bits;
     return SA_AMD_OK;
 }
 
@@ -1113,7 +1172,7 @@
     }
     KeyParams P, Ptext;
     int sigma = 0, key_bits = 0, g_bits = 0, top_shift = 0;
-    bool force_dense = false, text_ok = false, local_ok = false, probe_dense = false;
+    bool force_dense = false, text_ok = false, local_ok = false, probe_dense = false, probe_ran = false;
     SortResult sr;
     const uint32_t *sorted32 = nullptr;
     int bucket_top_bits = 0;
@@ -1287,8 +1346,9 @@
             if (use) top_shift = key_bits - 32;
         }
         local.top32_first = top_shift ? 1 : 0;
-        probe_dense = false;
+        probe_dense = false; probe_ran = false;
         if (text_ok && local_ok && !top_shift && !force_dense && !tn.no_repeat_probe && n >= ((int64_t)1 << 24)) {
+            probe_ran = true;
             const int64_t S = (int64_t)1 << 20;
             PROF(KC_MISC, S, st, hipLaunchKernelGGL((k_sample_repeat_keys), dim3((unsigned)ceil_div(S, GK_THREADS)), dim3(GK_THREADS), 0, st, dT, P, n, S,
                                                     w.keysA));
@@ -1307,8 +1367,9 @@
         }
 
         if (!top_shift && !tn.no_gram_keys && n >= tn.gram_min_n && n >= 2 && sigma >= 2 && tn.key_bits_max == 64) {
-            const int rcg = choose_gram_keys(dT, n, &P, &key_bits, w, st, tn, trace);
+            const int rcg = choose_gram_keys(dT, n, &P, &key_bits, w, st, tn, trace, !(probe_ran && !probe_dense));
             if (rcg) return rcg;
+            if (P.k > 64) return SA_AMD_EINTERNAL;
             local.bits_per_symbol = P.bits; local.symbols_per_key = P.k;
         }
 
@@ -1422,8 +1483,12 @@
             const bool counted = n > 1 && key_bits > 0;
             const int nb0 = key_bits < RADIX_BITS ? key_bits : RADIX_BITS;
             if (counted) HIP_TRY(hipMemsetAsync(fc.zero_ptr, 0, fc.zero_bytes, st));
-            if (P.gram > 0)
-                PROF(KC_BUILD_KEYS, n, st, hipLaunchKernelGGL((k_build_keys<false, true>), dim3((unsigned)ceil_div(ceil_div(n, KB_TILE), KB_TPW)), dim3(KB_THREADS), 0, st, dT, n, P,
+            if (P.gram2_m > 0)
+                PROF(KC_BUILD_KEYS, n, st, hipLaunchKernelGGL((k_build_keys<false, 2>), dim3((unsigned)ceil_div(ceil_div(n, KB_TILE), KB_TPW)), dim3(KB_THREADS), 0, st, dT, n, P,
+                                                              w.keysA, vals0, (uint32_t *)nullptr, 0, packed_out,
+                                                              counted ? fc.counts : (uint32_t *)nullptr, fc.chunk_elems, fc.G, (1u << nb0) - 1u));
+            else if (P.gram > 0)
+                PROF(KC_BUILD_KEYS, n, st, hipLaunchKernelGGL((k_build_keys<false, 1>), dim3((unsigned)ceil_div(ceil_div(n, KB_TILE), KB_TPW)), dim3(KB_THREADS), 0, st, dT, n, P,
                                                               w.keysA, vals0, (uint32_t *)nullptr, 0, packed_out,
                                                               counted ? fc.counts : (uint32_t *)nullptr, fc.chunk_elems, fc.G, (1u << nb0) - 1u));
             else
@@ -1441,8 +1506,11 @@
                     if (ss_done) { sr.keys = w.keysB; sr.vals = SA; sr.passes = 3; sr.skipped = 0; }
                     else {
                         HIP_TRY(hipMemsetAsync(fc.zero_ptr, 0, fc.zero_bytes, st));
-                        if (P.gram > 0)
-                            PROF(KC_BUILD_KEYS, n, st, hipLaunchKernelGGL((k_build_keys<false, true>), dim3((unsigned)ceil_div(ceil_div(n, KB_TILE), KB_TPW)), dim3(KB_THREADS), 0, st, dT, n, P,
+                        if (P.gram2_m > 0)
+                            PROF(KC_BUILD_KEYS, n, st, hipLaunchKernelGGL((k_build_keys<false, 2>), dim3((unsigned)ceil_div(ceil_div(n, KB_TILE), KB_TPW)), dim3(KB_THREADS), 0, st, dT, n, P,
+                                                                          w.keysA, vals0, (uint32_t *)nullptr, 0, packed_out, fc.counts, fc.chunk_elems, fc.G, (1u << nb0) - 1u));
+                        else if (P.gram > 0)
+                            PROF(KC_BUILD_KEYS, n, st, hipLaunchKernelGGL((k_build_keys<false, 1>), dim3((unsigned)ceil_div(ceil_div(n, KB_TILE), KB_TPW)), dim3(KB_THREADS), 0, st, dT, n, P,
                                                                           w.keysA, vals0, (uint32_t *)nullptr, 0, packed_out, fc.counts, fc.chunk_elems, fc.G, (1u << nb0) - 1u));
                         else
                             PROF(KC_BUILD_KEYS, n, st, hipLaunchKernelGGL((k_build_keys<false>), dim3((unsigned)ceil_div(ceil_div(n, KB_TILE), KB_TPW)), dim3(KB_THREADS), 0, st, dT, n, P,
diff --git a/suffix_array_amd/csrc/host/tuning.hpp b/suffix_array_amd/csrc/host/tuning.hpp
--- a/suffix_array_amd/csrc/host/tuning.hpp
+++ b/suffix_array_amd/csrc/host/tuning.hpp
@@ -32,6 +32,11 @@
 }
 
 inline int env_small_max() { return (int)env_int("SA_AMD_SMALL_MAX", 8192, 0, 8192); }
+
+constexpr int GRAM_LEVELS_DEFAULT = 2;
+constexpr int64_t GRAM2_MIN_N_DEFAULT = (int64_t)1 << 28;
+inline std::atomic<int> g_gram_levels{GRAM_LEVELS_DEFAULT};
+inline std::atomic<int64_t> g_gram2_min_n{GRAM2_MIN_N_DEFAULT};
 
 #ifdef SA_AMD_DIAG
 inline std::atomic<int> g_rerank_routes{0};
@@ -74,6 +79,8 @@
     int64_t gram_min_n = (int64_t)1 << 22;
     int gram_g = 0;
     int gram_tail_max = 8;
+    int gram_levels = GRAM_LEVELS_DEFAULT;
+    int64_t gram2_min_n = GRAM2_MIN_N_DEFAULT;
     int top32_partners_x100 = 50;
     int top32_collisions_x100 = 400;
     int64_t top32_probe_min_n = (int64_t)1 << 21;
@@ -146,6 +153,8 @@
         t.gram_min_n = env_int("SA_AMD_GRAM_MIN_N", (int64_t)1 << 22, 1, (int64_t)1 << 40);
         t.gram_g = (int)env_int("SA_AMD_GRAM_G", 0, 0, 8);
         t.gram_tail_max = (int)env_int("SA_AMD_GRAM_TAIL", 8, 0, 8);
+        t.gram_levels = g_gram_levels.load(std::memory_order_relaxed);
+        t.gram2_min_n = g_gram2_min_n.load(std::memory_order_relaxed);
         t.top32_partners_x100 = (int)env_int("SA_AMD_TOP32_PARTNERS_X100", 50, 0, 1000000);
         t.top32_collisions_x100 = (int)env_int("SA_AMD_TOP32_COLLISIONS_X100", 400, 0, 1000000);
         t.top32_probe_min_n = env_int("SA_AMD_TOP32_PROBE_MIN_N", (int64_t)1 << 21, 8192, (int64_t)1 << 40);
diff --git a/suffix_array_amd/csrc/kernels/keys.hpp b/suffix_array_amd/csrc/kernels/keys.hpp
--- a/suffix_array_amd/csrc/kernels/keys.hpp
+++ b/suffix_array_amd/csrc/kernels/keys.hpp
@@ -85,6 +85,9 @@
     uint32_t gram_top;
     uint64_t gram_D;
     const uint4 *gram_table;
+    int32_t gram2_e, gram2_m;
+    uint64_t gram2_D;
+    const uint4 *gram2_table;
 };
 
 __device__ __forceinline__ uint32_t gram_rank(const uint4 *__restrict__ table, uint32_t idx)
@@ -92,6 +95,13 @@
     const uint4 rec = table[idx >> 6];
     const uint64_t bits = ((uint64_t)rec.y << 32) | rec.x;
     return rec.z + (uint32_t)__popcll(bits & ((1ull << (idx & 63u)) - 1ull));
+}
+
+__device__ __forceinline__ uint32_t gram2_index(uint32_t rank1, const uint8_t *c, int o, int e, uint32_t sg)
+{
+    uint32_t idx = rank1;
+    for (int t = 0; t < e; ++t) idx = idx * sg + (uint32_t)c[o + t];
+    return idx;
 }
 
 __device__ __forceinline__ void kb_stage_codes(const uint8_t *__restrict__ T, int64_t n, int64_t base, const uint8_t *lcode, uint8_t *c, int tid);
@@ -102,7 +112,7 @@
 constexpr int GM_TPW = 64;
 __device__ __forceinline__ uint32_t gram_slot(uint32_t idx) { return (idx * 2654435761u) >> (32 - GM_LOG); }
 
-template <bool TOP32, bool GRAM = false>
+template <bool TOP32, int GRAM = 0>
 __global__ __launch_bounds__(KB_THREADS) void k_build_keys(const uint8_t *__restrict__ T, int64_t n,
                                                             KeyParams P, uint64_t *__restrict__ keys,
                                                             uint32_t *__restrict__ vals, uint32_t *__restrict__ keys32,
@@ -113,6 +123,7 @@
     __shared__ __attribute__((aligned(16))) uint8_t c[KB_TILE + KB_HALO];
     __shared__ uint32_t dhist[512];
     __shared__ uint32_t gc[GRAM ? KB_TILE + KB_HALO : 1];
+    __shared__ uint32_t gc2[GRAM == 2 ? KB_TILE + KB_HALO : 1];
     const int tid = threadIdx.x;
     lcode[tid] = P.code[tid];
     for (int d = tid; d < 512; d += KB_THREADS) dhist[d] = 0;
@@ -139,12 +150,29 @@
         __syncthreads();
         const uint64_t D = P.gram_D;
         const int tail = P.gram_tail;
+        if (GRAM == 2) {
+            const int e = P.gram2_e, m2 = P.gram2_m, g2 = g + e;
+            for (int o = tid; o + g2 <= KB_TILE + KB_HALO; o += KB_THREADS)
+                gc2[o] = gram_rank(P.gram2_table, gram2_index(gc[o], c, o + g, e, sg));
+            __syncthreads();
+            const uint64_t D2 = P.gram2_D;
+#pragma unroll
+            for (int r = 0; r < KB_ITEMS; ++r) {
+                uint64_t key = 0;
+                int o = p0 + r;
+                for (int j = 0; j < m2; ++j, o += g2) key = key * D2 + (uint64_t)gc2[o];
+                for (int j = 0; j < m; ++j, o += g) key = key * D + (uint64_t)gc[o];
+                for (int t = 0; t < tail; ++t) key = key * (uint64_t)sg + (uint64_t)c[o + t];
+                kk[r] = key;
+            }
+        } else {
 #pragma unroll
         for (int r = 0; r < KB_ITEMS; ++r) {
             uint64_t key = 0;
             for (int j = 0; j < m; ++j) key = key * D + (uint64_t)gc[p0 + r + g * j];
             for (int t = 0; t < tail; ++t) key = key * (uint64_t)sg + (uint64_t)c[p0 + r + g * m + t];
             kk[r] = key;
+        }
         }
     } else if (bits > 0) {
         const uint64_t mask = P.mask;
@@ -250,7 +278,8 @@
     }
 }
 
-__global__ __launch_bounds__(KB_THREADS) void k_gram_mark(const uint8_t *__restrict__ T, int64_t n, KeyParams P, int g, uint32_t top,
+template <bool LEVEL2>
+__global__ __launch_bounds__(KB_THREADS) void k_gram_mark(const uint8_t *__restrict__ T, int64_t n, KeyParams P, int g, uint32_t top, int e,
                                                            uint8_t *__restrict__ F)
 {
     __shared__ uint8_t lcode[256];
@@ -273,13 +302,24 @@
         for (int t = 0; t < g; ++t) idx = idx * sg + (uint32_t)c[p0 + t];
         uint32_t ix[KB_ITEMS];
         bool miss[KB_ITEMS];
+        if (LEVEL2) {
+#pragma unroll
+            for (int r = 0; r < KB_ITEMS; ++r) {
+                ix[r] = gram_rank(P.gram_table, idx);
+                idx = (idx - (uint32_t)c[p0 + r] * top) * sg + (uint32_t)c[p0 + r + g];
+            }
+#pragma unroll
+            for (int r = 0; r < KB_ITEMS; ++r) ix[r] = gram2_index(ix[r], c, p0 + r + g, e, sg);
+        }
 #pragma unroll
         for (int r = 0; r < KB_ITEMS; ++r) {
-            ix[r] = idx;
-            const uint32_t sl = gram_slot(idx);
-            miss[r] = base + p0 + r < n && s_tag[sl] != idx;
-            if (miss[r]) s_tag[sl] = idx;
-            idx = (idx - (uint32_t)c[p0 + r] * top) * sg + (uint32_t)c[p0 + r + g];
+            if (!LEVEL2) {
+                ix[r] = idx;
+                idx = (idx - (uint32_t)c[p0 + r] * top) * sg + (uint32_t)c[p0 + r + g];
+            }
+            const uint32_t sl = gram_slot(ix[r]);
+            miss[r] = base + p0 + r < n && s_tag[sl] != ix[r];
+            if (miss[r]) s_tag[sl] = ix[r];
         }
         uint8_t f[KB_ITEMS];
 #pragma unroll
@@ -345,12 +385,20 @@
     uint64_t tk = 0;
     if (P.gram > 0 && nsym == P.k) {
         const uint32_t sg = (uint32_t)P.sigma;
+        int64_t q = p;
+        for (int j = 0; j < P.gram2_m; ++j) {
+            uint32_t idx = 0;
+            for (int t = 0; t < P.gram; ++t) idx = idx * sg + (uint32_t)code_at(T, lcode, n, q++);
+            idx = gram_rank(P.gram_table, idx);
+            for (int t = 0; t < P.gram2_e; ++t) idx = idx * sg + (uint32_t)code_at(T, lcode, n, q++);
+            tk = tk * P.gram2_D + (uint64_t)gram_rank(P.gram2_table, idx);
+        }
         for (int j = 0; j < P.gram_m; ++j) {
             uint32_t idx = 0;
-            for (int t = 0; t < P.gram; ++t) idx = idx * sg + (uint32_t)code_at(T, lcode, n, p + (int64_t)P.gram * j + t);
+            for (int t = 0; t < P.gram; ++t) idx = idx * sg + (uint32_t)code_at(T, lcode, n, q++);
             tk = tk * P.gram_D + (uint64_t)gram_rank(P.gram_table, idx);
         }
-        for (int t = 0; t < P.gram_tail; ++t) tk = tk * P.sigma + code_at(T, lcode, n, p + (int64_t)P.gram * P.gram_m + t);
+        for (int t = 0; t < P.gram_tail; ++t) tk = tk * P.sigma + code_at(T, lcode, n, q++);
         return tk;
     }
     if (P.packed) {
diff --git a/suffix_array_amd/csrc/sa_api.hip b/suffix_array_amd/csrc/sa_api.hip
--- a/suffix_array_amd/csrc/sa_api.hip
+++ b/suffix_array_amd/csrc/sa_api.hip
@@ -112,6 +112,15 @@
     return sa::build_device(dT, dSA, n, dWork, work_bytes, (hipStream_t)stream, stats);
     SA_ABI_GUARD_END(0)
 }
+
+SA_EXPORT int32_t sa_amd_set_gram_levels(int32_t levels, int64_t min_n)
+{
+    if (min_n != 0) sa::g_gram2_min_n.store(min_n < 0 ? sa::GRAM2_MIN_N_DEFAULT : min_n, std::memory_order_relaxed);
+    if (levels == 0) return sa::g_gram_levels.load(std::memory_order_relaxed);
+    return sa::g_gram_levels.exchange(levels < 0 ? sa::GRAM_LEVELS_DEFAULT : (levels > 2 ? 2 : levels), std::memory_order_relaxed);
+}
+
+SA_EXPORT int64_t sa_amd_gram2_min_n(void) { return sa::g_gram2_min_n.load(std::memory_order_relaxed); }
 
 
 SA_EXPORT int32_t sa_amd_bucket_table_device(const uint8_t *dT, const uint32_t *dSA, int32_t n, uint32_t *dBkt, void *stream)
```

Result: no change. 5743 MB/s, median of 6 (+1.4%).
